# robdancer/SymbolicRegression.jl

Measured on AMD Instinct MI355X. Metric: tree-node x row evals/sec (whole node), 1k trees x 1M rows f32; % VALU peak, higher is better.
Workload: dtype f32; 1 GPU; C2 eval-only: 1024 random trees (size<=30) x 1M rows x 5 features Float32, fused L2 loss; ntrees_per_gpu=1024, rows=1000000, features=5, parallelism=single, trees_ok=808

## Files before the change

include/srhip.h:

```cpp
#ifndef SRHIP_H
#define SRHIP_H

#include <stdint.h>

#ifdef __cplusplus
extern "C" {
#endif

enum {
  SRHIP_OK = 0,
  SRHIP_ERR_INVALID = 1,
  SRHIP_ERR_UNSUPPORTED = 2,
  SRHIP_ERR_DEVICE = 3,
  SRHIP_ERR_NOMEM = 4
};

enum { SRHIP_F32 = 0, SRHIP_F64 = 1, SRHIP_I32 = 2 };

enum {
  SRHIP_OP_ADD = 1, SRHIP_OP_SUB = 2, SRHIP_OP_MUL = 3, SRHIP_OP_DIV = 4,
  SRHIP_OP_POW = 5,
  SRHIP_OP_GREATER = 6,
  SRHIP_OP_COND = 7,
  SRHIP_OP_LOGICAL_OR = 8,
// ... 31 lines not shown
  SRHIP_LOSS_PERCEPTRON = 10,
  SRHIP_LOSS_LOGIT_MARGIN = 11,
  SRHIP_LOSS_L1_HINGE = 12,
  SRHIP_LOSS_L2_HINGE = 13,
  SRHIP_LOSS_SMOOTHED_L1_HINGE = 14,
  SRHIP_LOSS_MODIFIED_HUBER = 15,
  SRHIP_LOSS_L2_MARGIN = 16,
  SRHIP_LOSS_EXP = 17,
  SRHIP_LOSS_SIGMOID = 18,
  SRHIP_LOSS_DWD_MARGIN = 19
};

typedef struct srhip_node {
  uint8_t degree;
  uint8_t constant;
  uint16_t op;
  uint16_t feature;
  uint16_t pad;
  int32_t l, r;
  double val;
} srhip_node;

typedef struct srhip_operators {
  int32_t nbin, nuna;
  const int32_t* binops;
  const int32_t* unaops;
} srhip_operators;

typedef struct srhip_loss {
  int32_t kind;
  int32_t pad;
  double p0, p1;
} srhip_loss;

typedef struct srhip_ctx srhip_ctx;
typedef struct srhip_dataset srhip_dataset;
typedef struct srhip_program srhip_program;

const char* srhip_last_error(void);
const char* srhip_version(void);
int srhip_device_count(void);

int srhip_ctx_create(int device_ordinal, srhip_ctx** out);
void srhip_ctx_destroy(srhip_ctx* ctx);
int srhip_ctx_synchronize(srhip_ctx* ctx);

int srhip_dataset_create(srhip_ctx* ctx, int dtype, const void* X, int64_t nfeatures, int64_t n,
                         int64_t stride_feature, int64_t stride_row, const void* y,
                         const void* weights, srhip_dataset** out);
void srhip_dataset_destroy(srhip_dataset* ds);

int srhip_program_create(srhip_ctx* ctx, int dtype, const srhip_node* nodes,
                         const int64_t* tree_offsets , int32_t ntrees,
                         const srhip_operators* ops, srhip_program** out);
void srhip_program_destroy(srhip_program* prog);
int srhip_program_num_constants(const srhip_program* prog, int32_t* out_nconst );
int srhip_program_set_constants(srhip_program* prog, const double* consts);
int srhip_program_get_constants(const srhip_program* prog, double* consts);

int srhip_eval_loss(srhip_ctx* ctx, const srhip_dataset* ds, const srhip_program* prog,
                    const srhip_loss* loss, const int64_t* idx, int64_t nidx,
                    double* out_loss, uint8_t* out_ok);

int srhip_eval_loss_rowsets(srhip_ctx* ctx, const srhip_dataset* ds, const srhip_program* prog,
                            const srhip_loss* loss, const int64_t* row_offsets ,
                            const int64_t* rows, double* out_loss, uint8_t* out_ok);

typedef struct srhip_eval_ticket srhip_eval_ticket;
int srhip_eval_loss_submit(srhip_ctx* ctx, const srhip_dataset* ds, const srhip_program* prog,
                           const srhip_loss* loss, const int64_t* idx, int64_t nidx,
                           srhip_eval_ticket** out_ticket);
int srhip_eval_loss_wait(srhip_eval_ticket* ticket, double* out_loss, uint8_t* out_ok);

int srhip_eval_predict(srhip_ctx* ctx, const srhip_dataset* ds, const srhip_program* prog,
                       const int64_t* idx, int64_t nidx, void* out_pred, uint8_t* out_ok);

int srhip_eval_loss_batch(srhip_ctx* ctx, const srhip_dataset* ds, const srhip_node* nodes,
                          const int64_t* tree_offsets, int32_t ntrees, const srhip_operators* ops,
                          const srhip_loss* loss, const int64_t* idx, int64_t nidx,
                          double* out_loss, uint8_t* out_ok);

int srhip_eval_loss_partials(srhip_ctx* ctx, const srhip_dataset* ds, const srhip_program* prog,
                             const srhip_loss* loss, const int64_t* idx, int64_t nidx,
                             double* sums, double* chk);
int srhip_partials_finalize(const srhip_program* prog, int64_t nfeatures, const double* sums,
                            const double* chk, double* out_loss, uint8_t* out_ok,
                            uint8_t* out_status);
int srhip_eval_precise_partials(srhip_ctx* ctx, const srhip_dataset* ds, const srhip_program* prog,
                                const int64_t* idx, int64_t nidx, const int32_t* trees,
                                int32_t ntrees_sel, double* opsums);
int srhip_precise_finalize(const srhip_program* prog, const int32_t* trees, int32_t ntrees_sel,
                           const double* opsums, uint8_t* out_ok);
int srhip_chk_reduce_op(int dtype);
int32_t srhip_program_max_ops(const srhip_program* prog);

typedef struct srhip_comm srhip_comm;
enum { SRHIP_COMM_ID_BYTES = 128 };
enum { SRHIP_REDUCE_SUM = 0, SRHIP_REDUCE_MAX = 1 };
int srhip_comm_unique_id(uint8_t* out_id );
int srhip_comm_create(srhip_ctx* ctx, const uint8_t* id, int32_t nranks, int32_t rank, srhip_comm** out);
void srhip_comm_destroy(srhip_comm* comm);
int srhip_comm_size(const srhip_comm* comm, int32_t* nranks, int32_t* rank);
int srhip_comm_stats(const srhip_comm* comm, double* ms_last, double* ms_total, int64_t* calls);
int srhip_comm_allreduce_f64(srhip_comm* comm, double* buf, int64_t n, int32_t op);
int srhip_comm_allgather(srhip_comm* comm, const void* send, int64_t bytes, void* recv);
int srhip_comm_migrate_start(srhip_comm* comm, const srhip_node* nodes, const int64_t* offsets,
                             int32_t ntrees, const double* losses, int32_t k, int32_t max_nodes);
int srhip_comm_migrate_wait(srhip_comm* comm, int32_t* out_counts, int64_t* out_offsets,
                            double* out_losses, srhip_node* out_nodes);
int srhip_eval_loss_sharded(srhip_ctx* ctx, srhip_comm* comm, const srhip_dataset* ds,
                            const srhip_program* prog, const srhip_loss* loss, const int64_t* idx,
                            int64_t nidx, double* out_loss, uint8_t* out_ok);

int srhip_eval_loss_grad(srhip_ctx* ctx, const srhip_dataset* ds, srhip_program* prog,
                         const srhip_loss* loss, const int64_t* idx, int64_t nidx,
                         double* out_loss, double* out_grad, uint8_t* out_ok);

enum { SRHIP_WRT_CONSTANTS = 0, SRHIP_WRT_FEATURES = 1 };
int srhip_eval_grad_predict(srhip_ctx* ctx, const srhip_dataset* ds, srhip_program* prog, int32_t wrt,
                            int32_t direction, const int64_t* idx, int64_t nidx, void* out_pred, void* out_grad,
                            uint8_t* out_ok);

typedef struct srhip_optim_options {
  int32_t iterations;
  int32_t nrestarts;
  uint64_t seed;
  double g_tol;
} srhip_optim_options;

int srhip_optimize_constants(srhip_ctx* ctx, const srhip_dataset* ds, srhip_program* prog,
                             const srhip_loss* loss, const int64_t* idx, int64_t nidx,
                             const srhip_optim_options* opt, double* out_loss,
                             uint8_t* out_improved, int64_t* out_fcalls);
int srhip_optimize_constants_starts(srhip_ctx* ctx, const srhip_dataset* ds, srhip_program* prog,
                                    const srhip_loss* loss, const int64_t* idx, int64_t nidx,
                                    const srhip_optim_options* opt, const double* starts_in,
                                    double* starts_out, double* out_loss, uint8_t* out_improved,
                                    int64_t* out_fcalls);

int srhip_eval_loss_grad_rowsets(srhip_ctx* ctx, const srhip_dataset* ds, srhip_program* prog,
                                 const srhip_loss* loss, const int64_t* row_offsets ,
                                 const int64_t* rows, double* out_loss, double* out_grad,
                                 uint8_t* out_ok);

int srhip_optimize_constants_rowsets(srhip_ctx* ctx, const srhip_dataset* ds, srhip_program* prog,
                                     const srhip_loss* loss, const int64_t* row_offsets ,
                                     const int64_t* rows, const srhip_optim_options* opt,
                                     const uint64_t* tree_seeds ,
                                     const double* starts_in , double* starts_out ,
                                     double* out_loss, uint8_t* out_improved, int64_t* out_fcalls);

double srhip_last_kernel_ms(const srhip_ctx* ctx);
int srhip_last_work(const srhip_ctx* ctx, int64_t out[4]);
int srhip_program_stats(const srhip_program* prog, int64_t* total_nodes, int64_t* total_opnodes,
                        int32_t* max_stack);
int srhip_program_derived(const srhip_program* prog, int32_t* count, uint32_t* spec, int32_t cap);
int srhip_code_cache_stats(int64_t* hits, int64_t* misses, int64_t* inserts);
int srhip_tail_share_parts(int32_t blocks, int32_t units, int32_t nshares, int32_t share, int32_t* out);

typedef struct srhip_batcher srhip_batcher;
int srhip_batcher_create(srhip_ctx* ctx, const srhip_dataset* ds, const srhip_operators* ops,
                         const srhip_loss* loss, int32_t max_batch, int32_t max_wait_us,
                         srhip_batcher** out);
int srhip_batcher_set_clients(srhip_batcher* b, int32_t nclients);
int srhip_batcher_submit(srhip_batcher* b, const srhip_node* nodes, int64_t nnodes,
                         const int64_t* idx, int64_t nidx, uint64_t* ticket);
int srhip_batcher_wait(srhip_batcher* b, uint64_t ticket, double* out_loss, uint8_t* out_ok);
int srhip_batcher_eval(srhip_batcher* b, const srhip_node* nodes, int64_t nnodes,
                       const int64_t* idx, int64_t nidx, double* out_loss, uint8_t* out_ok);
int srhip_batcher_stats(const srhip_batcher* b, int64_t* nrequests, int64_t* nlaunches,
                        int64_t* max_batch_seen);
int srhip_batcher_timing(const srhip_batcher* b, double* busy_ms, double* kernel_ms);
void srhip_batcher_destroy(srhip_batcher* b);

#ifdef __cplusplus
}
#endif
#endif
```

symbolicregression.jl_amd/csrc/srhip_eval_f32w.hip:

```cpp
#include "srhip_eval_impl.h"
#include "srhip_eval_variants.h"

namespace srhip {
hipError_t launch_eval_f32w(const EvalArgs& a, int mode, bool xlds, dim3 g, size_t lds, hipStream_t s) {
  if (mode == MODE_LOSS)
    return xlds ? launch_eval_t<float, R_F32_WIDE, 2, MODE_LOSS, true>(a, g, lds, s)
                : launch_eval_t<float, R_F32_WIDE, 2, MODE_LOSS, false>(a, g, lds, s);
  return xlds ? launch_eval_t<float, R_F32_WIDE, 2, MODE_PRED, true>(a, g, lds, s)
              : launch_eval_t<float, R_F32_WIDE, 2, MODE_PRED, false>(a, g, lds, s);
}
}
```

symbolicregression.jl_amd/csrc/srhip_eval_impl.h:

```cpp
#pragma once
#include <hip/hip_runtime.h>
#include <stdint.h>

#include <algorithm>
#include <type_traits>

#include "srhip_isa.h"
#include "srhip_kernels.h"
#include "srhip_ops.h"

#define UNR _Pragma("unroll")
#ifdef SRHIP_KDEBUG
#define KDBG(...) do { if (blockIdx.x == 0 && blockIdx.y == 0 && threadIdx.x == 0) printf(__VA_ARGS__); } while (0)
#else
#define KDBG(...) do { } while (0)
#endif
#ifdef SRHIP_KTRACE
#define KMARK(slot, val)                                                                       \
  do {                                                                                         \
    if (p.dbg && blockIdx.x == 0 && blockIdx.y == 0 && threadIdx.x == 0)                      \
      __hip_atomic_store(p.dbg + (slot), (int32_t)(val), __ATOMIC_RELAXED, __HIP_MEMORY_SCOPE_SYSTEM); \
  } while (0)
#else
#define KMARK(slot, val) do { } while (0)
#endif
#ifndef SRHIP_HEAVY_ILP
#define SRHIP_HEAVY_ILP 1
#endif
#ifndef SRHIP_TRIG_ILP
#ifndef SRHIP_JTRIG_FAST
#define SRHIP_JTRIG_FAST 1
#endif
#define SRHIP_TRIG_ILP SRHIP_HEAVY_ILP
#endif
#ifndef SRHIP_TRIG_ROWS
#define SRHIP_TRIG_ROWS 1
#endif
#ifndef SRHIP_HOT_CASES
#define SRHIP_HOT_CASES 0
#endif
#if SRHIP_HOT_CASES
#define SRHIP_LK [[likely]]
#else
#define SRHIP_LK
#endif
#define SRHIP_HOTB_ADD SRHIP_LK
#define SRHIP_HOTB_SUB SRHIP_LK
#define SRHIP_HOTB_MUL SRHIP_LK
#define SRHIP_HOTB_DIV SRHIP_LK
#define SRHIP_HOTB_GREATER
#define SRHIP_HOTB_COND
#define SRHIP_HOTB_LOGICAL_OR
#define SRHIP_HOTB_LOGICAL_AND
#define SRHIP_HOTB_MAX
#define SRHIP_HOTB_MIN
#define SRHIP_HOTU_NEG SRHIP_LK
#define SRHIP_HOTU_SQUARE SRHIP_LK
#define SRHIP_HOTU_CUBE SRHIP_LK
#define SRHIP_HOTU_ABS SRHIP_LK
#define SRHIP_HOTU_RELU
#define SRHIP_HOTU_COS SRHIP_LK
#define SRHIP_HOTU_SIN SRHIP_LK
#define SRHIP_HOTU_TAN
#define SRHIP_HOTU_EXP SRHIP_LK
#define SRHIP_HOTU_LOG SRHIP_LK
#define SRHIP_HOTU_LOG2
#define SRHIP_HOTU_LOG10
#define SRHIP_HOTU_LOG1P
#define SRHIP_HOTU_SQRT
#define SRHIP_HOTU_ACOSH
#define SRHIP_HOTU_ATANH_CLIP
#define SRHIP_HOTU_SINH
#define SRHIP_HOTU_COSH
#define SRHIP_HOTU_TANH
#define SRHIP_HOTU_ASIN
#define SRHIP_HOTU_ACOS
#define SRHIP_HOTU_ATAN
#define SRHIP_HOTU_ASINH
#define SRHIP_HOTU_ERF
#define SRHIP_HOTU_ERFC
#define SRHIP_HOTU_GAMMA
#define SRHIP_HOTU_ROUND
#define SRHIP_HOTU_FLOOR
#define SRHIP_HOTU_CEIL
#define SRHIP_HOTU_SIGN
#define SRHIP_HOTU_EXP2
#define SRHIP_HOTU_EXPM1
#define SRHIP_HOTU_CBRT
#ifndef SRHIP_ASM_DEF
#define SRHIP_ASM_DEF 1
#endif
#ifndef SRHIP_ROW_FENCE
#define SRHIP_ROW_FENCE() __builtin_amdgcn_sched_barrier(0)
#endif

namespace srhip {

template <typename T> constexpr bool kIsInt = std::is_same<T, int32_t>::value;

__device__ __attribute__((always_inline)) inline int tid_x() {
  int t = (int)__builtin_amdgcn_workitem_id_x();
  asm volatile("" : "+v"(t));
  return t;
}

template <typename T>
using OpsT = typename std::conditional<kIsInt<T>, IOps, FOps<typename std::conditional<kIsInt<T>, float, T>::type>>::type;

template <typename T> __device__ constexpr bool sb_ok(int sb) {
  return !kIsInt<T> || sb != SB_DIV;
}
template <typename T> __device__ constexpr bool hb_ok(int) { return !kIsInt<T>; }
template <typename T> __device__ constexpr bool un_ok(int u) {
  return !kIsInt<T> || u == UN_NEG || u == UN_SQUARE || u == UN_CUBE || u == UN_ABS ||
         u == UN_RELU || u == UN_SIGN;
}

template <typename T> struct Vec16;
template <> struct Vec16<float> { typedef float __attribute__((ext_vector_type(4))) type; };
template <> struct Vec16<int32_t> { typedef int32_t __attribute__((ext_vector_type(4))) type; };
template <> struct Vec16<double> { typedef double __attribute__((ext_vector_type(2))) type; };

template <typename T, int R> struct RowVec { typedef T type __attribute__((ext_vector_type(R))); };
template <typename T, int R> using RV = typename RowVec<T, R>::type;

template <typename T, int R>
__device__ __attribute__((always_inline)) inline void load_rows(const T* base, int lane, RV<T, R>& v) {
  constexpr int VEC = 16 / sizeof(T);
  using V = typename Vec16<T>::type;
  UNR for (int j = 0; j < R / VEC; ++j) {
    const V q = reinterpret_cast<const V*>(base)[j * 64 + lane];
    UNR for (int e = 0; e < VEC; ++e) v[j * VEC + e] = q[e];
  }
}

#if defined(__HIP_DEVICE_COMPILE__)
typedef const __attribute__((address_space(4))) Ins CIns;
#else
typedef const Ins CIns;
#endif

template <typename T> __device__ __attribute__((always_inline)) inline T imm_as(uint64_t bits) {
  if constexpr (sizeof(T) == 8) {
    return __builtin_bit_cast(T, bits);
  } else {
    return __builtin_bit_cast(T, (uint32_t)bits);
  }
}


__device__ __attribute__((always_inline)) inline int cvt_i32_sat(double k) {
  int m;
  asm("v_cvt_i32_f64 %0, %1" : "=v"(m) : "v"(k));
  return m;
}

template <int KIND>
__device__ __attribute__((always_inline)) inline float sincosf_dev(double x) {
  const double invpi = 0.3183098861837907, pi_hi = 3.141592653589793, pi_lo = 1.2246467991473532e-16;
  double k = __builtin_rint(__builtin_fma(x, invpi, KIND == 0 ? -0.5 : 0.0));
  const int m = cvt_i32_sat(k);
  if (KIND == 0) k += 0.5;
  const double y = __builtin_fma(-k, pi_lo, __builtin_fma(-k, pi_hi, x));
  const double p = srm_psin(y * y);
  const float r = KIND == 0 ? (float)(-y * p) : (float)(y * p);
  uint32_t o;
  asm("v_lshl_add_u32 %0, %1, 31, %2" : "=v"(o) : "v"(m), "v"(__builtin_bit_cast(uint32_t, r)));
  return __builtin_bit_cast(float, o);
}

typedef float F2 __attribute__((ext_vector_type(2)));
__device__ __attribute__((always_inline)) inline int cvt_i32_f32(float x) {
  int m;
  asm("v_cvt_i32_f32 %0, %1" : "=v"(m) : "v"(x));
  return m;
}
__device__ __attribute__((always_inline)) inline F2 expf2_dev(F2 x) {
  x = __builtin_elementwise_minimum(__builtin_elementwise_maximum(x, (F2)(-104.0f)), (F2)(89.0f));
  F2 n = x * (F2)(SRM_EXPF_LOG2E);
  n.x = __builtin_rintf(n.x);
  n.y = __builtin_rintf(n.y);
  F2 r = __builtin_elementwise_fma(n, (F2)(SRM_EXPF_NLN2_HI), x);
  r = __builtin_elementwise_fma(n, (F2)(SRM_EXPF_NLN2_LO), r);
  F2 p = __builtin_elementwise_fma(r, (F2)(SRM_EXPF_C6), (F2)(SRM_EXPF_C5));
  p = __builtin_elementwise_fma(r, p, (F2)(SRM_EXPF_C4));
  p = __builtin_elementwise_fma(r, p, (F2)(SRM_EXPF_C3));
  p = __builtin_elementwise_fma(r, p, (F2)(0.5f));
  p = __builtin_elementwise_fma(r, p, (F2)(1.0f));
  p = __builtin_elementwise_fma(r, p, (F2)(1.0f));
  F2 out;
  out.x = __builtin_ldexpf(p.x, cvt_i32_f32(n.x));
  out.y = __builtin_ldexpf(p.y, cvt_i32_f32(n.y));
  return out;
}

constexpr float EXPF_FAST_MAX = 87.0f;
__device__ __attribute__((always_inline)) inline F2 expf2_fast(F2 x) {
  const F2 t = x * (F2)(SRM_EXPF_LOG2E) + (F2)(12582912.0f);
  const F2 n = t - (F2)(12582912.0f);
  F2 r = __builtin_elementwise_fma(n, (F2)(SRM_EXPF_NLN2_HI), x);
  r = __builtin_elementwise_fma(n, (F2)(SRM_EXPF_NLN2_LO), r);
  F2 p = __builtin_elementwise_fma(r, (F2)(SRM_EXPF_C6), (F2)(SRM_EXPF_C5));
  p = __builtin_elementwise_fma(r, p, (F2)(SRM_EXPF_C4));
  p = __builtin_elementwise_fma(r, p, (F2)(SRM_EXPF_C3));
  p = __builtin_elementwise_fma(r, p, (F2)(0.5f));
  p = __builtin_elementwise_fma(r, p, (F2)(1.0f));
  p = __builtin_elementwise_fma(r, p, (F2)(1.0f));
  float s0, s1;
  asm("v_lshl_add_u32 %0, %1, 23, 1.0" : "=v"(s0) : "v"(t.x));
  asm("v_lshl_add_u32 %0, %1, 23, 1.0" : "=v"(s1) : "v"(t.y));
  return p * (F2){s0, s1};
}

#define SRM_PIO2F_BIG_F 421657440.0f
template <int R>
__device__ __attribute__((noinline)) RV<float, R> trigf_fix_tan(RV<float, R> v, RV<float, R> res) {
  UNR for (int r = 0; r < R; ++r) {
    const float x = v[r];
    if (x - x == 0.0f && srm_pio2f_is_big((double)x)) res[r] = srm_trigf(2, x);
  }
  return res;
}
template <int R, int KIND>
__device__ __attribute__((noinline)) RV<float, R> trigf_fix(RV<float, R> v, RV<float, R> res) {
  UNR for (int r = 0; r < R; ++r) {
    const float x = v[r];
    if (!(__builtin_fabsf(x) < SRM_PIO2F_BIG_F)) res[r] = srm_trigf(KIND, x);
  }
  return res;
}
template <int R, int KIND>
__device__ __attribute__((noinline)) RV<float, R> trigf_fast(RV<float, R> v) {
  UNR for (int r = 0; r < R; ++r) {
    v[r] = sincosf_dev<KIND>((double)v[r]);
    if ((r + 1) % SRHIP_HEAVY_ILP == 0) SRHIP_ROW_FENCE();
  }
  return v;
}
template <int R, int KIND>
__device__ __attribute__((noinline)) RV<float, R> trigf_slow(RV<float, R> v) {
  UNR for (int r = 0; r < R; ++r) {
    const float x = v[r];
    v[r] = __builtin_fabsf(x) < SRM_PIO2F_BIG_F ? sincosf_dev<KIND>((double)x) : srm_trigf(KIND, x);
  }
  return v;
}
#define SRHIP_M3(OP, a, b) OP " %0, %0, |%" #a "|, |%" #b "|\n\t"
template <int R, bool MAX>
__device__ __attribute__((always_inline)) inline float abs_fold(float m, const RV<float, R>& v) {
#define SRHIP_OPC (MAX ? "v_maximum3_f32" : "v_minimum3_f32")
  if constexpr (R == 16) {
    if constexpr (MAX)
      asm(SRHIP_M3("v_maximum3_f32", 1, 2) SRHIP_M3("v_maximum3_f32", 3, 4) SRHIP_M3("v_maximum3_f32", 5, 6)
          SRHIP_M3("v_maximum3_f32", 7, 8) SRHIP_M3("v_maximum3_f32", 9, 10) SRHIP_M3("v_maximum3_f32", 11, 12)
          SRHIP_M3("v_maximum3_f32", 13, 14) SRHIP_M3("v_maximum3_f32", 15, 16)
          : "+v"(m) : "v"(v[0]), "v"(v[1]), "v"(v[2]), "v"(v[3]), "v"(v[4]), "v"(v[5]), "v"(v[6]), "v"(v[7]),
            "v"(v[8]), "v"(v[9]), "v"(v[10]), "v"(v[11]), "v"(v[12]), "v"(v[13]), "v"(v[14]), "v"(v[15]));
    else
      asm(SRHIP_M3("v_minimum3_f32", 1, 2) SRHIP_M3("v_minimum3_f32", 3, 4) SRHIP_M3("v_minimum3_f32", 5, 6)
          SRHIP_M3("v_minimum3_f32", 7, 8) SRHIP_M3("v_minimum3_f32", 9, 10) SRHIP_M3("v_minimum3_f32", 11, 12)
          SRHIP_M3("v_minimum3_f32", 13, 14) SRHIP_M3("v_minimum3_f32", 15, 16)
          : "+v"(m) : "v"(v[0]), "v"(v[1]), "v"(v[2]), "v"(v[3]), "v"(v[4]), "v"(v[5]), "v"(v[6]), "v"(v[7]),
            "v"(v[8]), "v"(v[9]), "v"(v[10]), "v"(v[11]), "v"(v[12]), "v"(v[13]), "v"(v[14]), "v"(v[15]));
  } else if constexpr (R == 32) {
    RV<float, 16> lo, hi;
    UNR for (int r = 0; r < 16; ++r) { lo[r] = v[r]; hi[r] = v[16 + r]; }
    m = abs_fold<16, MAX>(m, lo);
    m = abs_fold<16, MAX>(m, hi);
  } else if constexpr (R == 8) {
    if constexpr (MAX)
      asm(SRHIP_M3("v_maximum3_f32", 1, 2) SRHIP_M3("v_maximum3_f32", 3, 4) SRHIP_M3("v_maximum3_f32", 5, 6)
          SRHIP_M3("v_maximum3_f32", 7, 8)
          : "+v"(m) : "v"(v[0]), "v"(v[1]), "v"(v[2]), "v"(v[3]), "v"(v[4]), "v"(v[5]), "v"(v[6]), "v"(v[7]));
    else
      asm(SRHIP_M3("v_minimum3_f32", 1, 2) SRHIP_M3("v_minimum3_f32", 3, 4) SRHIP_M3("v_minimum3_f32", 5, 6)
          SRHIP_M3("v_minimum3_f32", 7, 8)
          : "+v"(m) : "v"(v[0]), "v"(v[1]), "v"(v[2]), "v"(v[3]), "v"(v[4]), "v"(v[5]), "v"(v[6]), "v"(v[7]));
  } else {
    static_assert(R % 2 == 0, "row pairs");
    UNR for (int r = 0; r < R; r += 2) {
      if constexpr (MAX) asm("v_maximum3_f32 %0, %1, |%2|, |%3|" : "=v"(m) : "v"(m), "v"(v[r]), "v"(v[r + 1]));
      else asm("v_minimum3_f32 %0, %1, |%2|, |%3|" : "=v"(m) : "v"(m), "v"(v[r]), "v"(v[r + 1]));
    }
  }
#undef SRHIP_OPC
  return m;
}

template <int R> __device__ __attribute__((always_inline)) inline bool trigf_rows_fast(const RV<float, R>& A) {
  const float mx = abs_fold<R, true>(0.0f, A);
  return __builtin_amdgcn_ballot_w64(!(mx < SRM_PIO2F_BIG_F)) == 0;
}
// ... 516 lines not shown
      bin_rows<T, R, SB_SUB, false>(lv, yv);
      RV<T, R> dv;
      UNR for (int r = 0; r < R; ++r) dv[r] = lv[r];
      bin_rows<T, R, SB_MUL, false>(lv, dv);
    } else if (p.loss_kind == SRHIP_LOSS_L1) {
      UNR for (int r = 0; r < R; ++r) lv[r] = m_abs(A[r] - yv[r]);
    } else {
      lv = loss_rows_generic<T, R>(A, yv, p.loss_kind, p0);
    }
    if (p.weighted) {
      UNR for (int r = 0; r < R; ++r) lacc[r / RPC] += (double)(wv[r] * lv[r]);
    } else {
      if (!full) {
        UNR for (int r = 0; r < R; ++r) {
          const int64_t row = row0 + (r / VEC) * 64 * VEC + lane * VEC + (r % VEC);
          lv[r] = row < p.nvalid ? lv[r] : T(0);
        }
      }
      if constexpr (sizeof(T) == 4 && R % 4 == 0 && VEC == 4) {
        UNR for (int r = 0; r < R; r += 4) {
          const F2 a = {lv[r], lv[r + 1]}, b = {lv[r + 2], lv[r + 3]};
          const F2 q = a + b;
          lacc[r / RPC] += (double)(q.x + q.y);
        }
      } else {
        UNR for (int r = 0; r < R; ++r) lacc[r / RPC] += (double)lv[r];
      }
    }
  }
}

template <typename T, int R>
__device__ __attribute__((always_inline)) inline void store_pred(const EvalArgs& p, const RV<T, R>& A, int tree, int lane,
                                                                 int64_t row0) {
  constexpr int VEC = 16 / sizeof(T);
  using V = typename Vec16<T>::type;
  T* out = reinterpret_cast<T*>(p.out_pred) + (int64_t)tree * p.nvalid;
  UNR for (int j = 0; j < R / VEC; ++j) {
    const int64_t row = row0 + j * 64 * VEC + lane * VEC;
    if (row + VEC <= p.nvalid && ((p.nvalid % VEC) == 0)) {
      V q;
      UNR for (int e = 0; e < VEC; ++e) q[e] = A[j * VEC + e];
      *reinterpret_cast<V*>(out + row) = q;
    } else {
      UNR for (int e = 0; e < VEC; ++e)
        if (row + e < p.nvalid) out[row + e] = A[j * VEC + e];
    }
  }
}

template <typename T, int R>
__device__ __attribute__((noinline)) RV<T, R> derive_un(int u, RV<T, R> v) {
  switch (u) {
#define X_(NAME, FN)                                                                     \
  case UN_##NAME:                                                                        \
    if constexpr (un_ok<T>(UN_##NAME) && un_derivable(UN_##NAME)) return heavy_un<T, R, UN_##NAME>(v); \
    break;
    SRHIP_UNOPS(X_)
#undef X_
    default: break;
  }
  return v;
}

template <typename T>
__device__ __attribute__((always_inline)) inline void derive_columns(const EvalArgs& p, T* lx, int rbb,
                                                                     typename Chk<T>::type* dchk) {
  using CT = typename Chk<T>::type;
  constexpr int DV = 16 / sizeof(T);
  __shared__ CT part[EVAL_WAVES_MAX][DERIVE_MAX];
  const int tid = tid_x();
  const int lane = tid & 63, wave = tid >> 6;
  for (int d = 0; d < p.nd; ++d) {
    const uint32_t spec = __builtin_amdgcn_readfirstlane(p.dspec[d]);
    const int u = (int)(spec >> 16), f = (int)(spec & 0xffff);
    const T* src = lx + (int64_t)f * rbb;
    T* dst = lx + (int64_t)(p.nfeat + d) * rbb;
    CT m = 0;
    for (int c = tid; c < rbb / DV; c += blockDim.x) {
      RV<T, DV> v = reinterpret_cast<const RV<T, DV>*>(src)[c];
      v = derive_un<T, DV>(u, v);
      reinterpret_cast<RV<T, DV>*>(dst)[c] = v;
      UNR for (int e = 0; e < DV; ++e) {
        if constexpr (sizeof(T) == 4) m = __builtin_elementwise_maximum(m, __builtin_fabsf(v[e]));
        else m = __builtin_fma(__builtin_fabs(v[e]), 0x1p-512, m);
      }
    }
    m = wave_chk(m);
    if (lane == WAVE_LAST) part[wave][d] = m;
  }
  __syncthreads();
  const int tf = tid_x();
  if (tf < p.nd) {
    const int d = tf;
    CT t = part[0][d];
    for (int w = 1; w < (int)(blockDim.x >> 6); ++w) {
      if constexpr (sizeof(T) == 4) t = __builtin_elementwise_maximum(t, part[w][d]);
      else t += part[w][d];
    }
    dchk[d] = t;
  }
  __syncthreads();
}

template <typename T, int R>
__device__ __attribute__((always_inline)) inline void derive_columns_tiles(const EvalArgs& p, T* lx, int rbb,
                                                                           typename Chk<T>::type* dchk) {
  using CT = typename Chk<T>::type;
  constexpr int TILE = 64 * R, VEC = 16 / sizeof(T);
  constexpr int MAX_TILES = ROW_ALIGN / TILE > 0 ? ROW_ALIGN / TILE : 1;
  __shared__ CT part[DERIVE_MAX][MAX_TILES];
  const int tid = tid_x();
  const int lane = tid & 63;
  const int wave = __builtin_amdgcn_readfirstlane(tid >> 6), nwaves = blockDim.x >> 6;
  const int ntiles = rbb / TILE;
  for (int item = wave; item < p.nd * ntiles; item += nwaves) {
    const int d = item / ntiles, j = item - d * ntiles;
    const uint32_t spec = __builtin_amdgcn_readfirstlane(p.dspec[d]);
    const int u = (int)(spec >> 16), f = (int)(spec & 0xffff);
    RV<T, R> v;
    load_rows<T, R>(lx + (int64_t)f * rbb + (int64_t)j * TILE, lane, v);
    RV<T, R> rv;
    UNR for (int r = 0; r < R; ++r) rv[r] = v[r];
    rv = derive_un<T, R>(u, rv);
    CT m = 0;
    using V = typename Vec16<T>::type;
    T* dst = lx + (int64_t)(p.nfeat + d) * rbb + (int64_t)j * TILE;
    UNR for (int q = 0; q < R / VEC; ++q) {
      V o;
      UNR for (int e = 0; e < VEC; ++e) {
        o[e] = rv[q * VEC + e];
        if constexpr (sizeof(T) == 4) m = __builtin_elementwise_maximum(m, __builtin_fabsf(o[e]));
        else m = __builtin_fma(__builtin_fabs(o[e]), 0x1p-512, m);
      }
      reinterpret_cast<V*>(dst)[q * 64 + lane] = o;
    }
    m = wave_chk(m);
    if (lane == WAVE_LAST) part[d][j] = m;
  }
  __syncthreads();
  const int tf = tid_x();
  if (tf < p.nd) {
    const int d = tf;
    CT t = part[d][0];
    for (int j = 1; j < ntiles; ++j) {
      if constexpr (sizeof(T) == 4) t = __builtin_elementwise_maximum(t, part[d][j]);
      else t += part[d][j];
    }
    dchk[d] = t;
  }
  __syncthreads();
}

template <typename T, int R, int K, int MODE, bool XLDS>
__device__ __attribute__((always_inline)) inline void eval_block(const EvalArgs& p, unsigned char* smem, const int rb,
                                                                 const int gy, const int gslice = 0,
                                                                 const int gstride = 1, const int gw = 1) {
  constexpr int WAVES = eval_waves(R, K);
  using O = OpsT<T>;
  using CT = typename Chk<T>::type;
  constexpr int TILE = 64 * R;
  const int lane = tid_x() & 63;
  const int64_t row_base = (int64_t)rb * p.rb_rows;
  const int ntiles = p.rb_rows / TILE;
  const int nrel = __builtin_amdgcn_readfirstlane((int)min<int64_t>(max<int64_t>(p.nvalid - row_base, 0), (int64_t)p.rb_rows));

  const T* xsrc;
  const T* ysrc;
  const T* wsrc;
  int64_t xstride;
  if constexpr (XLDS) {
    T* lx = reinterpret_cast<T*>(smem);
    const int rbb = p.rb_rows;
    const int ncols = p.nfeat + (p.has_y ? 1 : 0) + (p.weighted ? 1 : 0);
    using V = typename Vec16<T>::type;
    constexpr int VEC = 16 / sizeof(T);
    const int vec_per_col = rbb / VEC;
    const T* gX = reinterpret_cast<const T*>(p.X);
    const T* gy = reinterpret_cast<const T*>(p.y);
    const T* gw = reinterpret_cast<const T*>(p.w);
    for (int i = tid_x(); i < ncols * vec_per_col; i += blockDim.x) {
      const int c = i / vec_per_col;
      const int v = i - c * vec_per_col;
      const T* src = c < p.nfeat ? gX + (int64_t)c * p.ld : (c == p.nfeat ? gy : gw);
      const int lc = c < p.nfeat ? c : c + p.nd;
      reinterpret_cast<V*>(lx + (int64_t)lc * rbb)[v] = reinterpret_cast<const V*>(src + row_base)[v];
    }
    xsrc = lx;
    ysrc = lx + (int64_t)(p.nfeat + p.nd) * rbb;
    wsrc = lx + (int64_t)(p.nfeat + p.nd + 1) * rbb;
    xstride = rbb;
  } else {
    xsrc = reinterpret_cast<const T*>(p.X) + row_base;
    ysrc = reinterpret_cast<const T*>(p.y) + row_base;
    wsrc = reinterpret_cast<const T*>(p.w) + row_base;
    xstride = p.ld;
  }
  KDBG("[k] staged, ntiles=%d rb_rows=%d nvalid=%ld max_steps=%d\n", ntiles, p.rb_rows, (long)p.nvalid, p.max_steps);
  __shared__ int next_tree;
  if (threadIdx.x == 0) next_tree = blockDim.x >> 6;
  constexpr int FLAG_SNAP = 2048;
  constexpr bool SNAP = MODE == MODE_LOSS && !kIsInt<T>;
  __shared__ uint8_t failed_snap[SNAP ? FLAG_SNAP : 1];
  const int gb0 = p.group_off ? p.group_off[gy] : gy * p.trees_per_group;
  const int snap_base = gb0 + gslice;
  const int snap_n = gstride > 1 ? tail_units_count(p.ntrees, gstride, gslice, gw)
                                 : (p.group_off ? p.group_off[gy + 1] - gb0 : min(p.trees_per_group, p.ntrees - gb0));
  if constexpr (SNAP) {
    if (p.early_exit)
      for (int i = tid_x(); i < min(snap_n, FLAG_SNAP); i += blockDim.x)
        failed_snap[i] = __hip_atomic_load(p.fail_flag + snap_base + (gw > 1 ? i / gw * gstride + i % gw : i * gstride),
                                           __ATOMIC_RELAXED, __HIP_MEMORY_SCOPE_AGENT) == p.epoch;
  }
  __syncthreads();
  constexpr bool DERIVED = XLDS && !kIsInt<T> && MODE != MODE_PRECISE;
  __shared__ CT dchk[DERIVED ? DERIVE_MAX : 1];
  if constexpr (DERIVED) {
    if (p.nd > 0) {
      if (p.persistent) derive_columns_tiles<T, R>(p, reinterpret_cast<T*>(smem), p.rb_rows, dchk);
      else derive_columns<T>(p, reinterpret_cast<T*>(smem), p.rb_rows, dchk);
    }
  }
  KMARK(0, 2);
  if (p.debug_stop == 2) return;

  const int group_base = __builtin_amdgcn_readfirstlane(snap_base);
  int group_n = __builtin_amdgcn_readfirstlane(snap_n);
  if constexpr (MODE == MODE_PRECISE) {
    if (p.dev_count) {
      const int cnt = __builtin_amdgcn_readfirstlane(*p.dev_count);
      group_n = max(0, min(group_n, (cnt - group_base + gstride - 1) / gstride));
    }
  }

  const int wave = __builtin_amdgcn_readfirstlane(threadIdx.x >> 6);
  const CIns* code = (const CIns*)(uintptr_t)p.code;
  KMARK(8 + wave, 10);
  const bool tile_claims = p.tile_claims != 0 && TILE == (sizeof(T) == 8 ? LOSS_CHUNK_8B : LOSS_CHUNK_4B);
  const int nclaims = tile_claims ? group_n * ntiles : group_n;
  for (int cl = wave; cl < nclaims;) {
    const int ti = tile_claims ? cl / ntiles : cl;
    const int tile0 = tile_claims ? cl - ti * ntiles : 0, tile_end = tile_claims ? tile0 + 1 : ntiles;
    KMARK(8 + wave, 11);
    const int slot = group_base + (gw > 1 ? ti / gw * gstride + ti % gw : ti * gstride);
    const int tree = __builtin_amdgcn_readfirstlane(p.order[slot]);
    const int pc0 = __builtin_amdgcn_readfirstlane(p.prog_off[tree]);
    const int max_steps = __builtin_amdgcn_readfirstlane(p.max_steps);
    KDBG("[k] ti=%d tree=%d pc0=%d group_n=%d\n", ti, tree, pc0, group_n);
    KMARK(0, 3);
    KMARK(1, tree);
    if (p.debug_stop == 3) break;

    if constexpr (MODE == MODE_PRECISE) {
      if (p.dev_count && lane == WAVE_LAST)
        for (int k = 0; k < p.prec_stride; ++k)
          reinterpret_cast<double*>(p.slab_prec)[((int64_t)slot * p.prec_stride + k) * p.nrb + rb] = 0.0;
    }
    constexpr int CHS = sizeof(T) == 8 ? LOSS_CHUNK_8B : LOSS_CHUNK_4B;
    constexpr int CPT = TILE > CHS ? TILE / CHS : 1, TPC = TILE > CHS ? 1 : CHS / TILE;
    static_assert(TILE > CHS ? TILE % CHS == 0 : CHS % TILE == 0, "tiles and loss chunks nest");
    LAccT<T> lacc[CPT];
    UNR for (int c = 0; c < CPT; ++c) lacc[c] = 0;
    CT M = 0;
    bool failed = false;
    if constexpr (SNAP) {
      if (p.early_exit && ti < FLAG_SNAP) failed = __builtin_amdgcn_readfirstlane(failed_snap[ti]) != 0;
    }
    if constexpr (DERIVED) {
      if (p.nd > 0) {
        uint64_t msk = p.dmask[tree];
        msk = ((uint64_t)__builtin_amdgcn_readfirstlane((uint32_t)(msk >> 32)) << 32) |
              (uint32_t)__builtin_amdgcn_readfirstlane((uint32_t)msk);
        while (msk) {
          const int d = __builtin_ctzll(msk);
          msk &= msk - 1;
          if constexpr (sizeof(T) == 4) M = __builtin_elementwise_maximum(M, dchk[d]);
          else if (lane == WAVE_LAST) M += dchk[d];
        }
      }
    }
    LAccT<T>* lslab = reinterpret_cast<LAccT<T>*>(p.slab_loss) +
                      ((int64_t)rb * p.ntrees + slot) * __builtin_amdgcn_readfirstlane(p.cpb);
    LAccT<T> csum = 0;
    int rows_done = 0;
    if (failed) {
      if (lane == WAVE_LAST)
        for (int c = tile_claims ? tile0 : 0; c < (tile_claims ? tile_end : p.cpb); ++c) lslab[c] = (LAccT<T>)NAN;
      M = (CT)NAN;
      csum = (LAccT<T>)NAN;
    }
    for (int tile = tile0; tile < (failed ? tile0 : tile_end); ++tile) {
      const int64_t row0 = row_base + (int64_t)tile * TILE;
      const int trel = tile * TILE;
      if (trel >= nrel) break;
      rows_done += min(TILE, nrel - trel);
      const T* xt = xsrc + (int64_t)tile * TILE;
      RV<T, R> A, S[K];
#if SRHIP_ASM_DEF
      asm volatile("" : "=v"(A));
      UNR for (int k = 0; k < K; ++k) asm volatile("" : "=v"(S[k]));
#else
      UNR for (int r = 0; r < R; ++r) A[r] = T(0);
      UNR for (int k = 0; k < K; ++k) UNR for (int r = 0; r < R; ++r) S[k][r] = T(0);
#endif
      const CIns* prog = code + pc0;
      Ins nxt = prog[0];
      [[maybe_unused]] uint32_t pord = 0;
      for (int step = 0; step < max_steps; ++step) {
        const Ins ins = nxt;
        nxt = prog[step + 1];
        KDBG("[k]   tile=%d step=%d h=%u a=%u\n", tile, step, ins.h, ins.a);
        if (ins.h == H_END) break;
        switch (ins.h) {
          SRHIP_LK case H_LOADF:
            load_rows<T, R>(xt + (int64_t)(ins.a & 0xffff) * xstride, lane, A);
            if constexpr (MODE == MODE_PRECISE)
              if ((ins.a >> 16) != 0) precise_hook<T, R>(p, ++pord, A, slot, rb, lane, row0);
            break;
          SRHIP_LK case H_LOADC: { const T c = imm_as<T>(ins.imm); UNR for (int r = 0; r < R; ++r) A[r] = c; break; }
#define SRHIP_K_CASES(BASE, ...)                                                            \
  case BASE + 0: if constexpr (0 < K) { constexpr int k = 0; __VA_ARGS__ } break;                 \
  case BASE + 1: if constexpr (1 < K) { constexpr int k = 1; __VA_ARGS__ } break;                 \
  case BASE + 2: if constexpr (2 < K) { constexpr int k = 2; __VA_ARGS__ } break;                 \
  case BASE + 3: if constexpr (3 < K) { constexpr int k = 3; __VA_ARGS__ } break;                 \
  case BASE + 4: if constexpr (4 < K) { constexpr int k = 4; __VA_ARGS__ } break;                 \
  case BASE + 5: if constexpr (5 < K) { constexpr int k = 5; __VA_ARGS__ } break;                 \
  case BASE + 6: if constexpr (6 < K) { constexpr int k = 6; __VA_ARGS__ } break;                 \
  case BASE + 7: if constexpr (7 < K) { constexpr int k = 7; __VA_ARGS__ } break;
#define SRHIP_K_CASES_H(HOT, BASE, ...)                                                     \
  HOT case BASE + 0: if constexpr (0 < K) { constexpr int k = 0; __VA_ARGS__ } break;             \
  HOT case BASE + 1: if constexpr (1 < K) { constexpr int k = 1; __VA_ARGS__ } break;             \
  case BASE + 2: if constexpr (2 < K) { constexpr int k = 2; __VA_ARGS__ } break;                 \
  case BASE + 3: if constexpr (3 < K) { constexpr int k = 3; __VA_ARGS__ } break;                 \
  case BASE + 4: if constexpr (4 < K) { constexpr int k = 4; __VA_ARGS__ } break;                 \
  case BASE + 5: if constexpr (5 < K) { constexpr int k = 5; __VA_ARGS__ } break;                 \
  case BASE + 6: if constexpr (6 < K) { constexpr int k = 6; __VA_ARGS__ } break;                 \
  case BASE + 7: if constexpr (7 < K) { constexpr int k = 7; __VA_ARGS__ } break;
          SRHIP_K_CASES_H(SRHIP_LK, H_PUSH0, { UNR for (int r = 0; r < R; ++r) S[k][r] = A[r]; })
          SRHIP_K_CASES_H(SRHIP_LK, H_PUSHLF0, {
            UNR for (int r = 0; r < R; ++r) S[k][r] = A[r];
            load_rows<T, R>(xt + (int64_t)(ins.a & 0xffff) * xstride, lane, A);
          })
          SRHIP_K_CASES_H(SRHIP_LK, H_PUSHLC0, {
            UNR for (int r = 0; r < R; ++r) S[k][r] = A[r];
            const T c = imm_as<T>(ins.imm);
            UNR for (int r = 0; r < R; ++r) A[r] = c;
          })
          SRHIP_K_CASES(H_SLOADF0, { load_rows<T, R>(xt + (int64_t)(ins.a & 0xffff) * xstride, lane, S[k]); })
          SRHIP_K_CASES(H_SLOADC0, { const T c = imm_as<T>(ins.imm); UNR for (int r = 0; r < R; ++r) S[k][r] = c; })

#define SRHIP_SPEC_CASE(NAME, FN)                                                                  \
  SRHIP_HOTB_##NAME case h_spec(SB_##NAME, SPEC_AF):                                                \
    if constexpr (sb_ok<T>(SB_##NAME)) {                                                           \
      RV<T, R> xv;                                                                                     \
      load_rows<T, R>(xt + (int64_t)(ins.a & 0xffff) * xstride, lane, xv);                                    \
      bin_rows_chk<T, R, SB_##NAME, false>(A, xv, M);                                              \
      if constexpr (MODE == MODE_PRECISE) precise_hook<T, R>(p, ++pord, A, slot, rb, lane, row0);         \
    }                                                                                              \
    break;                                                                                         \
  SRHIP_HOTB_##NAME case h_spec(SB_##NAME, SPEC_FA):                                                \
    if constexpr (sb_ok<T>(SB_##NAME)) {                                                           \
      RV<T, R> xv;                                                                                     \
      load_rows<T, R>(xt + (int64_t)(ins.a & 0xffff) * xstride, lane, xv);                                    \
      bin_rows_chk<T, R, SB_##NAME, true>(A, xv, M);                                               \
      if constexpr (MODE == MODE_PRECISE) precise_hook<T, R>(p, ++pord, A, slot, rb, lane, row0);         \
    }                                                                                              \
    break;                                                                                         \
  SRHIP_HOTB_##NAME case h_spec(SB_##NAME, SPEC_AC):                                                \
    if constexpr (sb_ok<T>(SB_##NAME)) {                                                           \
      bin_rows_c_chk<T, R, SB_##NAME, false>(A, imm_as<T>(ins.imm), M);                            \
      if constexpr (MODE == MODE_PRECISE) precise_hook<T, R>(p, ++pord, A, slot, rb, lane, row0);         \
    }                                                                                              \
    break;                                                                                         \
  SRHIP_HOTB_##NAME case h_spec(SB_##NAME, SPEC_CA):                                                \
    if constexpr (sb_ok<T>(SB_##NAME)) {                                                           \
      bin_rows_c_chk<T, R, SB_##NAME, true>(A, imm_as<T>(ins.imm), M);                             \
      if constexpr (MODE == MODE_PRECISE) precise_hook<T, R>(p, ++pord, A, slot, rb, lane, row0);         \
    }                                                                                              \
    break;                                                                                         \
  SRHIP_HOTB_##NAME case h_spec(SB_##NAME, SPEC_FF):                                              \
    if constexpr (sb_ok<T>(SB_##NAME)) {                                                           \
      RV<T, R> xv;                                                                                 \
      load_rows<T, R>(xt + (int64_t)(ins.a & 0xffff) * xstride, lane, A);                          \
      load_rows<T, R>(xt + (int64_t)(ins.imm & 0xffff) * xstride, lane, xv);                       \
      bin_rows_chk<T, R, SB_##NAME, false>(A, xv, M);                                              \
      if constexpr (MODE == MODE_PRECISE) precise_hook<T, R>(p, ++pord, A, slot, rb, lane, row0);     \
    }                                                                                              \
    break;                                                                                         \
  SRHIP_HOTB_##NAME case h_spec(SB_##NAME, SPEC_FC):                                              \
    if constexpr (sb_ok<T>(SB_##NAME)) {                                                           \
      load_rows<T, R>(xt + (int64_t)(ins.a & 0xffff) * xstride, lane, A);                          \
      bin_rows_c_chk<T, R, SB_##NAME, false>(A, imm_as<T>(ins.imm), M);                            \
      if constexpr (MODE == MODE_PRECISE) precise_hook<T, R>(p, ++pord, A, slot, rb, lane, row0);     \
    }                                                                                              \
    break;                                                                                         \
  SRHIP_HOTB_##NAME case h_spec(SB_##NAME, SPEC_CF):                                              \
    if constexpr (sb_ok<T>(SB_##NAME)) {                                                           \
      load_rows<T, R>(xt + (int64_t)(ins.a & 0xffff) * xstride, lane, A);                          \
      bin_rows_c_chk<T, R, SB_##NAME, true>(A, imm_as<T>(ins.imm), M);                             \
      if constexpr (MODE == MODE_PRECISE) precise_hook<T, R>(p, ++pord, A, slot, rb, lane, row0);     \
    }                                                                                              \
    break;                                                                                         \
    SRHIP_K_CASES_H(SRHIP_HOTB_##NAME, h_spec(SB_##NAME, SPEC_SA0), if constexpr (sb_ok<T>(SB_##NAME)) {                \
      bin_rows_chk<T, R, SB_##NAME, true>(A, S[k], M);                                             \
      if constexpr (MODE == MODE_PRECISE) precise_hook<T, R>(p, ++pord, A, slot, rb, lane, row0);         \
    })                                                                                             \
    SRHIP_K_CASES_H(SRHIP_HOTB_##NAME, h_spec(SB_##NAME, SPEC_AS0), if constexpr (sb_ok<T>(SB_##NAME)) {                \
      bin_rows_chk<T, R, SB_##NAME, false>(A, S[k], M);                                            \
      if constexpr (MODE == MODE_PRECISE) precise_hook<T, R>(p, ++pord, A, slot, rb, lane, row0);         \
    })
          SRHIP_SPEC_BINOPS(SRHIP_SPEC_CASE)
#undef SRHIP_SPEC_CASE

#define SRHIP_HEAVY_CASE(NAME, FN)                                                              \
    SRHIP_K_CASES(h_heavy(HB_##NAME, HEAVY_SA0), if constexpr (hb_ok<T>(HB_##NAME)) {           \
      apply_heavy<T, R, HB_##NAME>(A, S[k], A);                                                 \
      chk_update<R>(M, A);                                                                      \
      if constexpr (MODE == MODE_PRECISE) precise_hook<T, R>(p, ++pord, A, slot, rb, lane, row0);  \
    })                                                                                          \
    SRHIP_K_CASES(h_heavy(HB_##NAME, HEAVY_AS0), if constexpr (hb_ok<T>(HB_##NAME)) {           \
      apply_heavy<T, R, HB_##NAME>(A, A, S[k]);                                                 \
      chk_update<R>(M, A);                                                                      \
      if constexpr (MODE == MODE_PRECISE) precise_hook<T, R>(p, ++pord, A, slot, rb, lane, row0);  \
    })
          SRHIP_HEAVY_BINOPS(SRHIP_HEAVY_CASE)
#undef SRHIP_HEAVY_CASE

#define SRHIP_UN_CASE(NAME, FN)                                                  \
  SRHIP_HOTU_##NAME case h_un(UN_##NAME):                                        \
    if constexpr (un_ok<T>(UN_##NAME) && (K == K_MAX || !un_wide(UN_##NAME))) {  \
      apply_un<T, R, UN_##NAME>(A);                                              \
      if constexpr (UN_##NAME == UN_COS || UN_##NAME == UN_SIN) {                \
        if (!(ins.a & UN_NC_FLAG)) chk_update<R>(M, A);                          \
      } else {                                                                   \
        chk_update<R>(M, A);                                                     \
      }                                                                          \
      if constexpr (MODE == MODE_PRECISE) precise_hook<T, R>(p, ++pord, A, slot, rb, lane, row0); \
    }                                                                            \
    break;
          SRHIP_UNOPS(SRHIP_UN_CASE)
#undef SRHIP_UN_CASE
#undef SRHIP_K_CASES
          default: break;
        }
      }
      KDBG("[k]   tile %d done\n", tile);
      KMARK(0, 4);
      if constexpr (MODE == MODE_LOSS) {
        loss_tile<T, R>(p, A, ysrc + (int64_t)tile * TILE, wsrc + (int64_t)tile * TILE, lane, row0, trel + TILE <= nrel,
                        lacc);
        const bool flushed = (tile + 1) % TPC == 0 || trel + TILE >= nrel;
        const int ci0 = tile * CPT / TPC;
        if (flushed) {
          UNR for (int c = 0; c < CPT; ++c) {
            const LAccT<T> s = wave_sum(lacc[c]);
            if (lane == WAVE_LAST) lslab[ci0 + c] = s;
            if (p.fused) {
              const LAccT<T> sb = __shfl(s, WAVE_LAST);
              if (lane == (ci0 + c) % 64) csum += sb;
            }
            lacc[c] = 0;
          }
        }
        if constexpr (!kIsInt<T>) {
          if (p.early_exit && __builtin_amdgcn_ballot_w64(!(M < (CT)INFINITY)) != 0) {
            csum = (LAccT<T>)NAN;
            if (lane == WAVE_LAST) {
              for (int c = ci0 + (flushed ? CPT : 0); c < (tile_claims ? tile_end : p.cpb); ++c)
                lslab[c] = (LAccT<T>)NAN;
              __hip_atomic_store(p.fail_flag + slot, p.epoch, __ATOMIC_RELAXED, __HIP_MEMORY_SCOPE_AGENT);
            }
            break;
          }
        }
      } else if constexpr (MODE == MODE_PRED) {
        store_pred<T, R>(p, A, tree, lane, row0);
      }
    }
    KDBG("[k] tree %d tiles done\n", tree);
    KMARK(0, 5);
    KMARK(8 + wave, 12);
    if constexpr (!kIsInt<T> && MODE != MODE_PRECISE) {
      M = wave_chk(M);
      CT* chk_at = reinterpret_cast<CT*>(p.slab_chk) + (int64_t)rb * p.ntrees + slot;
      if (lane == WAVE_LAST) {
        if constexpr (sizeof(CT) == 4) {
          if (tile_claims) atomicMax(reinterpret_cast<unsigned*>(chk_at), __builtin_bit_cast(unsigned, __builtin_fabsf(M) == __builtin_fabsf(M) ? __builtin_fabsf(M) : M));
          else *chk_at = M;
        } else {
          *chk_at = M;
        }
      }
    }
    if (p.slab_rows && lane == WAVE_LAST) {
      if (tile_claims) atomicAdd(p.slab_rows + (int64_t)rb * p.ntrees + slot, rows_done);
      else p.slab_rows[(int64_t)rb * p.ntrees + slot] = rows_done;
    }
    if constexpr (MODE != MODE_PRECISE) {
      if (p.fused) {
        LAccT<T> s = csum;
        CT m = 0;
        if constexpr (!kIsInt<T>) {
          const CT mb = __shfl(M, WAVE_LAST);
          if (lane == 0) {
            if constexpr (sizeof(T) == 4) m = __builtin_elementwise_maximum(m, mb);
            else m += mb;
          }
        }
        UNR for (int o = 32; o > 0; o >>= 1) {
          if (MODE == MODE_LOSS) s += __shfl_xor(s, o);
          if constexpr (!kIsInt<T>) {
            if constexpr (sizeof(T) == 4) m = __builtin_elementwise_maximum(m, __shfl_xor(m, o));
            else m += __shfl_xor(m, o);
          }
        }
        if (lane == 0) {
          if (MODE == MODE_LOSS && p.fused_loss) reinterpret_cast<LAccT<T>*>(p.fused_loss)[tree] = s;
          if (p.fused_chk) reinterpret_cast<CT*>(p.fused_chk)[tree] = m;
          if (p.fused_rows) p.fused_rows[tree] = rows_done;
        }
      }
    }
    KMARK(8 + wave, 13);
    int claim = 0;
    if (lane == 0) claim = atomicAdd(&next_tree, 1);
    cl = __builtin_amdgcn_readfirstlane(claim);
  }
  KMARK(8 + wave, 14);
}

template <typename T, int R, int K, int MODE, bool XLDS>
__global__ __launch_bounds__(64 * eval_waves(R, K)) void eval_kernel(EvalArgs p) {
  extern __shared__ __attribute__((aligned(16))) unsigned char smem[];
  KMARK(0, 1);
  if (p.debug_stop == 1) return;
  __shared__ int claimed;
  if constexpr (MODE == MODE_PRECISE) {
    if (p.dev_count && p.grid_interleave && __builtin_amdgcn_readfirstlane(*p.dev_count) <= (int)blockIdx.y) return;
  }
  if (p.tile_claims && !p.persistent) {
    if (p.zero_ctr && blockIdx.x == 0 && blockIdx.y == 0 && threadIdx.x == 0)
      __hip_atomic_store(p.zero_ctr, 0, __ATOMIC_RELAXED, __HIP_MEMORY_SCOPE_AGENT);
    const int gs = p.grid_interleave ? (int)blockIdx.y : 0, gst = p.grid_interleave ? (int)gridDim.y : 1;
    const int nz = p.grid_interleave ? (p.ntrees - gs + gst - 1) / gst : 0;
    for (int i = threadIdx.x; i < nz; i += blockDim.x) {
      const int64_t at = (int64_t)blockIdx.x * p.ntrees + gs + (int64_t)i * gst;
      if (p.slab_chk) __hip_atomic_store(reinterpret_cast<uint32_t*>(p.slab_chk) + at, 0u, __ATOMIC_RELAXED, __HIP_MEMORY_SCOPE_AGENT);
      if (p.slab_rows) __hip_atomic_store(p.slab_rows + at, 0, __ATOMIC_RELAXED, __HIP_MEMORY_SCOPE_AGENT);
    }
    __builtin_amdgcn_fence(__ATOMIC_RELEASE, "workgroup");
  }
  const int nfull = p.nrb - p.block0 - p.tail_blocks;
  const int nitems = nfull + (p.tail_blocks > 0 ? p.tail_shares : 0);
  int items = 0;
  int next_block = 0, next_units = 0;
  for (int it = 0;; ++it) {
    int rb, gy = 0, gslice = 0, gstride = 1, gw = 1;
    if (p.persistent && next_units > 0) {
      rb = next_block;
      gstride = p.tail_slices;
      gw = next_units;
      next_units = 0;
    } else if (p.persistent) {
      if (threadIdx.x == 0) claimed = atomicAdd(p.block_ctr, 1);
      __syncthreads();
      const int item = __builtin_amdgcn_readfirstlane(claimed);
      if (item >= nitems) {
        if (threadIdx.x == 0 && items > 0) atomicAdd(p.block_ctr + 1, items);
        if (threadIdx.x == 0 && item == nitems + (int)gridDim.x - 1)
          __hip_atomic_store(p.block_ctr, 0, __ATOMIC_RELAXED, __HIP_MEMORY_SCOPE_AGENT);
        break;
      }
      ++items;
      rb = p.block0 + item;
      if (item >= nfull) {
        TailPart part[2];
        const int nparts = tail_share_parts(p.tail_blocks, p.tail_slices, p.tail_shares, item - nfull, part);
        if (nparts == 0) {
          __syncthreads();
          continue;
        }
        rb = p.block0 + nfull + part[0].block;
        gslice = part[0].u0;
        gstride = p.tail_slices;
        gw = part[0].u1 - part[0].u0;
        if (nparts == 2) {
          next_block = rb + 1;
          next_units = part[1].u1;
        }
      }
    } else {
      rb = blockIdx.x + it * (int)gridDim.x;
      if (it > 0 && (!p.block_stride || rb >= p.nrb)) break;
      if (p.grid_interleave) {
        gslice = blockIdx.y;
        gstride = gridDim.y;
      } else {
        gy = blockIdx.y;
      }
    }
    eval_block<T, R, K, MODE, XLDS>(p, smem, rb, gy, gslice, gstride, gw);
    if (!p.persistent && !p.block_stride) break;
    __syncthreads();
  }
}

template <typename T, int R, int K, int MODE, bool XLDS>
inline hipError_t launch_eval_t(const EvalArgs& a, dim3 grid, size_t lds, hipStream_t s) {
  auto kern = eval_kernel<T, R, K, MODE, XLDS>;
  if (lds > 65536) {
    hipError_t e = hipFuncSetAttribute((const void*)kern, hipFuncAttributeMaxDynamicSharedMemorySize, (int)lds);
    if (e != hipSuccess) return e;
  }
  const int waves = a.wg_waves > 0 ? std::min(a.wg_waves, eval_waves(R, K)) : eval_waves(R, K);
  hipLaunchKernelGGL(kern, grid, dim3(64 * waves), lds, s, a);
  return hipGetLastError();
}

template <typename T, int R, int MODE, bool XLDS>
inline hipError_t launch_eval_k(const EvalArgs& a, int K, dim3 grid, size_t lds, hipStream_t s) {
  if (K <= 2) return launch_eval_t<T, R, 2, MODE, XLDS>(a, grid, lds, s);
  if (K <= 4) return launch_eval_t<T, R, 4, MODE, XLDS>(a, grid, lds, s);
  return launch_eval_t<T, R, 8, MODE, XLDS>(a, grid, lds, s);
}

template <typename T, int R, int MODE>
inline hipError_t launch_eval_mode(const EvalArgs& a, int K, bool xlds, dim3 grid, size_t lds, hipStream_t s) {
  if constexpr (MODE == MODE_PRECISE) {
    (void)K;
    (void)xlds;
    return launch_eval_t<T, R, K_MAX, MODE_PRECISE, false>(a, grid, lds, s);
  } else {
    return xlds ? launch_eval_k<T, R, MODE, true>(a, K, grid, lds, s) : launch_eval_k<T, R, MODE, false>(a, K, grid, lds, s);
  }
}

}
```

symbolicregression.jl_amd/csrc/srhip_host.cpp:

```cpp
#include <hip/hip_runtime.h>
#include <math.h>
#include <stdarg.h>
#include <stdint.h>
#include <stdio.h>
#include <stdlib.h>
#include <string.h>
#include <unistd.h>
#include <sys/resource.h>
#include <sys/syscall.h>

#include <algorithm>
#include <atomic>
#include <chrono>
#include <condition_variable>
#include <functional>
#include <memory>
#include <map>
#include <mutex>
#include <numeric>
#include <string>
#include <thread>
#include <type_traits>
#include <unordered_map>
#include <vector>
// ... 1375 lines not shown
  if (n_dspec) memcpy(h + o_dspec, P.dspec.data(), n_dspec);
  if (n_dmask) memcpy(h + o_dmask, P.dmask.data(), n_dmask);
  if (n_sb) memcpy(h + o_sb, P.sbound.data(), n_sb);
  const size_t offs[7] = {o_off, o_dcode, o_doff, o_dspec, o_dmask, o_sb, total};
  memcpy(P.blob_off, offs, sizeof(offs));
  if (defer) {
    P.upload_pending = true;
    return SRHIP_OK;
  }
  P.upload_pending = false;
  const bool with_order = !P.ord_host.empty() && P.ord_key[0] > 0;
  const size_t nbytes = with_order ? total + P.ord_host.size() * sizeof(int32_t) : total;
  if (with_order) {
    P.blob.resize(nbytes);
    memcpy(P.blob.data() + total, P.ord_host.data(), P.ord_host.size() * sizeof(int32_t));
    h = P.blob.data();
  }
  HIP_TRY(P.d_prog.ensure(nbytes));
  hipStream_t st = stream ? stream : P.ctx->stream;
  HIP_TRY(hipMemcpyAsync(P.d_prog.p, h, nbytes, hipMemcpyHostToDevice, st));
  set_prog_pointers(P);
  if (with_order) P.ord_dev = (const uint8_t*)P.d_prog.p + total;
  if (sync) HIP_TRY(hipStreamSynchronize(st));
  return SRHIP_OK;
}


namespace {

}

int srhip::make_view(srhip_ctx* ctx, const srhip_dataset* ds, const int64_t* idx, int64_t nidx, bool need_y, View& v) {
  if (need_y && !ds->has_y) return fail(SRHIP_ERR_INVALID, "dataset has no y");
  if (!idx) {
    v.X = ds->X.p;
    v.y = ds->y.p;
    v.w = ds->weighted ? ds->w.p : nullptr;
    v.ld = ds->ld;
    v.m = ds->n;
    v.stats = ds->hstats.data();
    v.sum_w = ds->sum_w;
    return SRHIP_OK;
  }
  if (nidx <= 0) return fail(SRHIP_ERR_INVALID, "empty idx");
  for (int64_t i = 0; i < nidx; ++i)
    if (idx[i] < 0 || idx[i] >= ds->n) return fail(SRHIP_ERR_INVALID, "idx[%lld] = %lld out of range", (long long)i, (long long)idx[i]);
  const size_t es = dtype_size(ds->dtype);
  const int64_t ld = (nidx + ROW_ALIGN - 1) / ROW_ALIGN * ROW_ALIGN;
  HIP_TRY(ctx->vX.ensure((size_t)std::max<int64_t>(1, ds->nfeat) * ld * es));
  HIP_TRY(ctx->vy.ensure((size_t)ld * es));
  HIP_TRY(ctx->vw.ensure((size_t)ld * es));
  HIP_TRY(ctx->vidx.ensure((size_t)nidx * sizeof(int64_t)));
  HIP_TRY(ctx->vstats.ensure(feature_stats_scratch(ds->nfeat) * sizeof(FeatStat)));
  HIP_TRY(ctx->h_stats.ensure((size_t)std::max<int64_t>(1, ds->nfeat) * sizeof(FeatStat)));
  HIP_TRY(hipMemcpyAsync(ctx->vidx.p, idx, (size_t)nidx * sizeof(int64_t), hipMemcpyHostToDevice, ctx->stream));
  HIP_TRY(launch_gather(ds->dtype, ds->X.p, ds->has_y ? ds->y.p : nullptr, ds->weighted ? ds->w.p : nullptr, ds->ld,
                        (int)ds->nfeat, (const int64_t*)ctx->vidx.p, nidx, ld, ctx->vX.p,
                        ds->has_y ? ctx->vy.p : nullptr, ds->weighted ? ctx->vw.p : nullptr, ctx->stream));
  HIP_TRY(launch_feature_stats(ds->dtype, ctx->vX.p, ld, nidx, (int)ds->nfeat, (FeatStat*)ctx->vstats.p, ctx->stream));
  if (ds->dtype != SRHIP_I32 && ds->nfeat > 0)
    HIP_TRY(hipMemcpyAsync(ctx->h_stats.p, ctx->vstats.p, (size_t)ds->nfeat * sizeof(FeatStat), hipMemcpyDeviceToHost,
                           ctx->stream));
  double sw = 0.0;
  if (ds->weighted) {
  }
  HIP_TRY(hipStreamSynchronize(ctx->stream));
  v.X = ctx->vX.p;
  v.y = ds->has_y ? ctx->vy.p : nullptr;
  v.w = ds->weighted ? ctx->vw.p : nullptr;
  v.ld = ld;
  v.m = nidx;
  v.stats = (const FeatStat*)ctx->h_stats.p;
  v.sum_w = sw;
  return SRHIP_OK;
}

LaunchPlan srhip::plan_launch(const srhip_ctx* ctx, int dtype, int64_t nxcols, bool weighted, bool with_y, int64_t m,
                              int32_t ntrees, int tile, size_t budget, int waves) {
  LaunchPlan L;
  ntrees = std::max<int32_t>(1, ntrees);
  m = std::max<int64_t>(1, m);
  const size_t es = dtype_size(dtype);
  const int ncols = (int)nxcols + (with_y ? 1 : 0) + (weighted ? 1 : 0);
  const int lo = std::max(tile, loss_chunk(dtype));
  int rb = ROW_ALIGN;
  while (rb > lo && (size_t)ncols * rb * es > budget) rb /= 2;
  while (rb > lo && rb / 2 >= m) rb /= 2;
  static const int rb_env = [] { const char* e = getenv("SRHIP_RB_ROWS"); return e ? atoi(e) : 0; }();
  if (rb_env >= lo && rb_env <= ROW_ALIGN && (rb_env & (rb_env - 1)) == 0 && rb_env < rb) rb = rb_env;
  L.rb_rows = rb;
  L.xlds = (size_t)ncols * rb * es <= budget;
  L.lds = (L.xlds ? (size_t)ncols * rb * es : 0) + 16;
  L.nrb = (int)((m + rb - 1) / rb);
  const int target_blocks = 4 * ctx->num_cu;
  int g = (target_blocks + L.nrb - 1) / L.nrb;
  const int max_g = std::max(1, ntrees / (2 * waves));
  g = std::max(1, std::min(g, max_g));
  L.groups = g;
  L.tpg = (ntrees + g - 1) / g;
  L.groups = (ntrees + L.tpg - 1) / L.tpg;
  return L;
}

namespace {

std::vector<int32_t> shape_groups(const LaunchPlan& L, int32_t ntrees, int num_cu) {
  static const bool no_tail = [] { const char* e = getenv("SRHIP_NO_TAIL"); return e && *e && *e != '0'; }();
  std::vector<int32_t> off(1, 0);
  const bool tail = !no_tail && ntrees >= 128 && (int64_t)L.groups * L.nrb > 2 * (int64_t)num_cu;
  if (!tail) {
    for (int g = 0; g < L.groups; ++g) off.push_back(std::min(ntrees, off.back() + L.tpg));
    return off;
  }
  static const int tail_div = [] { const char* e = getenv("SRHIP_TAIL_DIV"); return e && atoi(e) >= 2 ? atoi(e) : 32; }();
  static const int bulk_g = [] { const char* e = getenv("SRHIP_BULK_GROUPS"); return e ? atoi(e) : 0; }();
  const int32_t tl = std::max<int32_t>(16, ntrees / tail_div), bulk = ntrees - tl;
  const int groups = bulk_g > 0 ? std::min<int>(bulk_g, std::max(1, bulk / 16)) : L.groups;
  const int32_t tpg = (bulk + groups - 1) / groups;
  while (off.back() < bulk) off.push_back(std::min(bulk, off.back() + tpg));
  static const int tail_min = [] { const char* e = getenv("SRHIP_TAIL_MIN"); return e && atoi(e) > 0 ? atoi(e) : 16; }();
  int32_t t = tl;
  while (t > tail_min) {
    const int32_t h = t / 2;
    off.push_back(off.back() + h);
    t -= h;
  }
  if (t > 0) off.push_back(off.back() + t);
  return off;
}

std::vector<int32_t> make_order(const srhip_program& P, const std::vector<int32_t>& trees,
                                const std::vector<int32_t>& goff, bool derived) {
  std::vector<int32_t> s(trees);
  auto cost = [&](int32_t t) { return derived ? P.dcost[t] : P.info[t].cost; };
  std::stable_sort(s.begin(), s.end(), [&](int32_t a, int32_t b) { return cost(a) > cost(b); });
  const int groups = (int)goff.size() - 1;
  std::vector<int32_t> order(s.size());
  std::vector<int> fill(groups, 0);
  for (int32_t t : s) {
    int best = -1;
    double bf = -1.0;
    for (int g = 0; g < groups; ++g) {
      const int cap = goff[g + 1] - goff[g];
      if (fill[g] >= cap) continue;
      const double f = (double)(cap - fill[g]) / cap;
      if (f > bf) {
        bf = f;
        best = g;
      }
    }
    order[(size_t)goff[best] + fill[best]++] = t;
  }
  return order;
}


static int decide_info(const TreeInfo& I, int dtype, int32_t T, int64_t nfeat, const double* sums, double chk) {
  if (I.static_fail) return 1;
  if (dtype == SRHIP_I32) return 0;
  const long double m = (long double)sums[2 * (size_t)T + 2 * (size_t)nfeat];
  const long double ovf = ovf_threshold(dtype);
  for (double c : I.fill_consts)
    if ((long double)fabs(c) * m >= ovf) return 1;
  for (int f : I.feat_checks) {
    const double fsum = sums[2 * (size_t)T + 2 * (size_t)f], fbad = sums[2 * (size_t)T + 2 * (size_t)f + 1];
    if (fbad > 0) return 1;
    const long double sum = dtype == SRHIP_F64 ? (long double)fsum * 0x1p64L : (long double)fsum;
    if (!isfinite(fsum) || fabsl(sum) >= ovf) return 1;
  }
  if (I.op_sumcheck.empty()) return 0;
  if (!isfinite(chk)) return 1;
  long double bound;
  if (dtype == SRHIP_F64) bound = (long double)chk * 0x1p512L;
  else bound = (long double)chk * m;
  if (bound * 2.0L >= ovf) return 2;
  return 0;
}

static int decide_fast(const srhip_program& P, int32_t t, int64_t nfeat, const double* sums, double chk) {
  const TreeDecide& d = P.dec[t];
  if (d.slow) return decide_info(P.info[t], P.dtype, P.ntrees, nfeat, sums, chk);
  if (d.static_fail) return 1;
  const int dtype = P.dtype;
  if (dtype == SRHIP_I32) return 0;
  const int32_t T = P.ntrees;
  const long double m = (long double)sums[2 * (size_t)T + 2 * (size_t)nfeat];
  const long double ovf = ovf_threshold(dtype);
  if (d.maxc >= 0.0 && (long double)d.maxc * m >= ovf) return 1;
  for (uint64_t fm = d.feat_mask; fm; fm &= fm - 1) {
    const int f = __builtin_ctzll(fm);
    const double fsum = sums[2 * (size_t)T + 2 * (size_t)f], fbad = sums[2 * (size_t)T + 2 * (size_t)f + 1];
    if (fbad > 0) return 1;
    const long double sum = dtype == SRHIP_F64 ? (long double)fsum * 0x1p64L : (long double)fsum;
    if (!isfinite(fsum) || fabsl(sum) >= ovf) return 1;
  }
  if (!d.has_op) return 0;
  if (!isfinite(chk)) return 1;
  long double bound;
  if (dtype == SRHIP_F64) bound = (long double)chk * 0x1p512L;
  else bound = (long double)chk * m;
  if (bound * 2.0L >= ovf) return 2;
  return 0;
}

static void finalize(const srhip_program& P, int64_t nfeat, const double* sums, const double* chk, double* out_loss,
                     uint8_t* out_ok, uint8_t* out_status) {
  const bool fast = P.dec.size() == (size_t)P.ntrees && !env_flag("SRHIP_DECIDE_SLOW");
  for (int32_t t = 0; t < P.ntrees; ++t) {
    const double c = chk ? chk[t] : 0.0;
    const int st = fast ? decide_fast(P, t, nfeat, sums, c) : decide_info(P.info[t], P.dtype, P.ntrees, nfeat, sums, c);
    if (out_status) out_status[t] = (uint8_t)st;
    if (out_ok) out_ok[t] = st == 0 ? 1 : 0;
    if (out_loss) out_loss[t] = st == 0 ? sums[2 * (size_t)t] / sums[2 * (size_t)t + 1] : INFINITY;
  }
}

static void finalize_precise(const srhip_program& P, const int32_t* trees, int32_t nsel, const double* opsums,
                             uint8_t* out_ok, bool grad = false) {
  const int stride = std::max(1, grad ? P.gmax_ops : P.max_ops);
  const long double ovf = ovf_threshold(P.dtype);
  for (int u = 0; u < nsel; ++u) {
    const TreeInfo& I = grad ? P.ginfo[trees[u]] : P.info[trees[u]];
    int st = I.static_fail ? 1 : 0;
    for (size_t k = 0; k < I.op_sumcheck.size() && !st; ++k) {
      const double s = opsums[(size_t)u * stride + k];
      if (!isfinite(s)) st = 1;
      else if (I.op_sumcheck[k]) {
        const long double S = P.dtype == SRHIP_F64 ? (long double)s * 0x1p64L : (long double)s;
        if (fabsl(S) >= ovf) st = 1;
      }
    }
    out_ok[u] = st == 0 ? 1 : 0;
  }
}

}

namespace {
struct DevPool {
  std::mutex mu;
  std::map<std::pair<int, size_t>, std::vector<void*>> free;
  size_t cached = 0;
};
DevPool& devpool() {
  static DevPool* P = new DevPool();
  return *P;
}
constexpr size_t DEVPOOL_MAX_CACHED = (size_t)512 << 20;
size_t devpool_class(size_t n) {
  size_t c = 4096;
  while (c < n) c <<= 1;
  return c;
}
}

void* srhip::devpool_get(size_t bytes, size_t* cap) {
  const size_t c = devpool_class(bytes);
  int dev = 0;
  if (hipGetDevice(&dev) != hipSuccess) return nullptr;
  {
    DevPool& P = devpool();
    std::lock_guard<std::mutex> g(P.mu);
    auto it = P.free.find({dev, c});
    if (it != P.free.end() && !it->second.empty()) {
      void* q = it->second.back();
      it->second.pop_back();
      P.cached -= c;
      *cap = c;
      return q;
    }
  }
  void* q = nullptr;
  if (hipMalloc(&q, c) != hipSuccess) return nullptr;
  *cap = c;
  return q;
}

void srhip::devpool_put(void* p, size_t cap, int device) {
  if (!p) return;
  DevPool& P = devpool();
  {
    std::lock_guard<std::mutex> g(P.mu);
    if (device >= 0 && P.cached + cap <= DEVPOOL_MAX_CACHED) {
      P.free[{device, cap}].push_back(p);
      P.cached += cap;
      return;
    }
  }
  (void)hipFree(p);
}

int srhip::next_fail_epoch(srhip_ctx* ctx, int64_t n, int32_t** flags, int32_t* epoch) {
  const size_t need = (size_t)std::max<int64_t>(n, 1) * sizeof(int32_t);
  const bool fresh = !ctx->fail_flag.p || ctx->fail_flag.bytes < need;
  HIP_TRY(ctx->fail_flag.ensure(need));
  if (fresh || ctx->epoch == INT32_MAX) {
    HIP_TRY(hipMemsetAsync(ctx->fail_flag.p, 0, ctx->fail_flag.bytes, ctx->stream));
    ctx->epoch = 0;
  }
  *flags = (int32_t*)ctx->fail_flag.p;
  *epoch = ++ctx->epoch;
  return SRHIP_OK;
}

int srhip::decide_tree(const TreeInfo& I, const srhip_program& P, int64_t nfeat, const double* sums, double chk) {
  return decide_info(I, P.dtype, P.ntrees, nfeat, sums, chk);
// ... 89 lines not shown
  q.rb_rows = Lp.rb_rows;
  q.nrb = Lp.nrb;
  q.trees_per_group = 1;
  q.slab_prec = ctx->slab_prec.p;
  q.prec_stride = stride;
  q.max_steps = P->max_len;
  q.dev_count = ulist;
  q.wg_waves = 1;
  q.prec_assign = 1;
  q.block_stride = 1;
  HIP_TRY(launch_eval(dtype, q, Rp, K_MAX, MODE_PRECISE, false, dim3(std::min(Lp.nrb, PRECISE_GRID_X), G), 16,
                      ctx->stream));
  int32_t* hl = (int32_t*)rs->h_pout.p;
  double* hs = (double*)((uint8_t*)rs->h_pout.p + PREC_SUMS_OFF);
  HIP_TRY(launch_precise_reduce((const double*)ctx->slab_prec.p, Lp.nrb, stride, ulist, cap, G, DEV_PRECISE_MAX, hl,
                                hs, ctx->stream));
  *out_stride = stride;
  return SRHIP_OK;
}

struct EvalJob {
  ResultSet* rs = nullptr;
  bool launched = false, persistent = false, devp = false;
  int mode = 0, dtype = 0;
  int32_t nt = 0;
  int32_t expect_items = 0;
  std::vector<int32_t> live;
  UndecidedList ul;
  DevBuf pred;
  bool fused = false;
  float fbound = 0.0f;
};
static float feature_bound(const View& v, int64_t nfeat) {
  double F = 0.0;
  for (int64_t f = 0; v.stats && f < nfeat; ++f) {
    if (v.stats[f].nonfinite > 0 || !(v.stats[f].maxabs < INFINITY)) return INFINITY;
    F = std::max(F, v.stats[f].maxabs);
  }
  if (!v.stats && nfeat > 0) return INFINITY;
  const float r = (float)F;
  return (double)r >= F ? r : std::nextafter(r, INFINITY);
}

static int eval_issue(srhip_ctx* ctx, const srhip_dataset* ds, const srhip_program* P, int mode, const srhip_loss* loss,
                      const View& v, void* out_pred, double* sums, double* chk, DevPrecise* dp, ShardDev* sd,
                      EvalJob& J) {
  const int dtype = P->dtype;
  const int32_t nt = P->ntrees;
  ResultSet* const rs = J.rs;
  J.mode = mode;
  J.dtype = dtype;
  J.nt = nt;
  const int64_t nf = ds->nfeat;
  const bool weighted = ds->weighted && mode == MODE_LOSS;
  for (size_t i = 0; i < sums_len(nt, nf); ++i) sums[i] = 0.0;
  for (int32_t t = 0; t < nt; ++t) {
    chk[t] = 0.0;
    sums[2 * (size_t)t + 1] = weighted ? v.sum_w : (double)v.m;
  }
  for (int64_t f = 0; f < nf; ++f) {
    sums[2 * (size_t)nt + 2 * f] = v.stats[f].sum;
    sums[2 * (size_t)nt + 2 * f + 1] = (double)v.stats[f].nonfinite;
  }
  sums[2 * (size_t)nt + 2 * nf] = (double)v.m;
  std::vector<int32_t>& live = J.live;
  live.clear();
  live.reserve(nt);
  for (int32_t t = 0; t < nt; ++t)
    if (!(P->dec.size() == (size_t)nt ? P->dec[t].static_fail : P->info[t].static_fail)) live.push_back(t);
  if (live.empty()) return SRHIP_OK;
  const size_t es = dtype_size(dtype);
  bool wide = false;
  for (int32_t u : P->unaops) wide |= u == SRHIP_OP_ASIN || u == SRHIP_OP_ACOS || u == SRHIP_OP_ATANH_CLIP;
  auto kvariant = [&](int32_t kmax) { return wide ? K_MAX : (kmax <= 2 ? 2 : (kmax <= 4 ? 4 : 8)); };
  const int nd = (int)P->dspec.size();
  bool use_d = false;
  int K = 0, R = 0;
  LaunchPlan L{};
  const size_t lds_dev = (size_t)ctx->lds_max;
  auto lds_budget = [lds_dev](int r, int k, bool derived) -> size_t {
    if (eval_waves(r, k) >= 16) return lds_dev - 8 * 1024;
    return std::min<size_t>(lds_dev / 2, derived ? 64 * 1024 - 512 : 64 * 1024 - 64);
  };
  const bool no_persistent = env_flag("SRHIP_NO_PERSISTENT");
  const int prb_env = env_int("SRHIP_PRB_ROWS", 0);
  const int probe_env = env_int("SRHIP_PROBE_BLOCKS", -1);
  bool persistent = false;
  int probe_blocks = 0;
  const int small_max = env_int("SRHIP_SMALL_POP", 16);
  const bool small = (mode == MODE_LOSS || mode == MODE_PRED) && debug_stop() == 0 && (int)live.size() <= small_max &&
                     v.m >= (int64_t)64 * ROW_ALIGN;
  if (small) {
    K = kvariant(P->kmax);
    R = pick_rows_per_lane(dtype, K, mode, v.m);
    L.rb_rows = std::max(64 * R, loss_chunk(dtype));
    L.xlds = false;
    L.lds = 16;
    L.nrb = (int)((v.m + L.rb_rows - 1) / L.rb_rows);
    L.groups = 1;
    L.tpg = (int)live.size();
  }
  if (!small) {
    const int Kp = kvariant(P->kmax);
    persistent = !no_persistent && mode == MODE_LOSS && debug_stop() == 0 && dtype == SRHIP_F32 &&
                 pick_rows_per_lane(dtype, Kp, mode, v.m) == R_F32_WIDE && R_F32_WIDE != R_F32 &&
                 (nd == 0 || kvariant(P->dkmax) == Kp);
    if (persistent) {
      K = Kp;
      R = R_F32_WIDE;
      const int tile = 64 * R;
      int rb = prb_env >= tile && prb_env <= ROW_ALIGN && (prb_env & (prb_env - 1)) == 0 ? prb_env : 2048;
      rb = std::max(rb, std::max(tile, loss_chunk(dtype)));
      const size_t es = dtype_size(dtype);
      const int base_cols = P->maxfeat + 1 + (weighted ? 1 : 0);
      use_d = nd > 0 && (size_t)(base_cols + nd) * rb * es <= lds_budget(R, K, true);
      const int ncols = base_cols + (use_d ? nd : 0);
      if ((size_t)ncols * rb * es > lds_budget(R, K, false)) {
        persistent = false;
        use_d = false;
      } else {
        L.rb_rows = rb;
        L.xlds = true;
        L.lds = (size_t)ncols * rb * es + 16;
        L.nrb = (int)((v.m + rb - 1) / rb);
        L.groups = 1;
        L.tpg = (int)live.size();
        probe_blocks = probe_env >= 0 ? probe_env : 4;
        probe_blocks = L.nrb >= 16 * std::max(1, probe_blocks) ? probe_blocks : 0;
      }
    }
  }
  if (!small && !persistent && nd > 0 && mode != MODE_PRECISE) {
    K = kvariant(P->dkmax);
    R = pick_rows_per_lane(dtype, K, mode, v.m);
    L = plan_launch(ctx, dtype, P->maxfeat + nd, weighted, mode == MODE_LOSS, v.m, (int32_t)live.size(), 64 * R,
                    lds_budget(R, K, true), eval_waves(R, K));
    use_d = L.xlds;
    const char* always = env_get("SRHIP_DERIVE_ALWAYS");
    if (use_d && !(always && *always && *always != '0')) {
      const int Kp = kvariant(P->kmax), Rp = pick_rows_per_lane(dtype, Kp, mode, v.m);
      const LaunchPlan Lp = plan_launch(ctx, dtype, P->maxfeat, weighted, mode == MODE_LOSS, v.m, (int32_t)live.size(),
                                        64 * Rp, lds_budget(Rp, Kp, false), eval_waves(Rp, Kp));
      if (Lp.xlds && Lp.rb_rows > L.rb_rows) use_d = false;
    }
  }
  if (!small && !persistent && !use_d) {
    K = kvariant(P->kmax);
    R = pick_rows_per_lane(dtype, K, mode, v.m);
    L = plan_launch(ctx, dtype, P->maxfeat, weighted, mode == MODE_LOSS, v.m, (int32_t)live.size(), 64 * R,
                    lds_budget(R, K, false), eval_waves(R, K));
  }
  const int nl = (int)live.size();
  const void* d_order;
  const std::vector<int32_t> goff = persistent ? std::vector<int32_t>{0, nl} : shape_groups(L, nl, ctx->num_cu);
  {
    std::lock_guard<std::mutex> g(P->ord_mu);
    if (P->upload_pending || P->ord_key[0] != L.groups || P->ord_key[1] != L.tpg || P->ord_key[2] != (int)use_d ||
        P->ord_goff != goff) {
      std::vector<int32_t>& order = P->ord_host;
      order = make_order(*P, live, goff, use_d);
      order.insert(order.end(), goff.begin(), goff.end());
      if (P->upload_pending) {
        const size_t base = P->blob_off[6], bytes = order.size() * sizeof(int32_t);
        P->blob.resize(base + bytes);
        memcpy(P->blob.data() + base, order.data(), bytes);
        HIP_TRY(P->d_prog.ensure(base + bytes));
        HIP_TRY(hipMemcpyAsync(P->d_prog.p, P->blob.data(), base + bytes, hipMemcpyHostToDevice, ctx->stream));
        set_prog_pointers(*P);
        P->upload_pending = false;
        P->ord_dev = (const uint8_t*)P->d_prog.p + base;
      } else {
        HIP_TRY(P->d_order.ensure(order.size() * sizeof(int32_t)));
        HIP_TRY(hipMemcpyAsync(P->d_order.p, order.data(), order.size() * sizeof(int32_t), hipMemcpyHostToDevice,
                               ctx->stream));
        P->ord_dev = P->d_order.p;
      }
      P->ord_key[0] = L.groups;
      P->ord_key[1] = L.tpg;
      P->ord_key[2] = (int)use_d;
      P->ord_goff = goff;
    }
    d_order = P->ord_dev;
  }
  const int nch = (int)((v.m + loss_chunk(dtype) - 1) / loss_chunk(dtype));
  const int cpb = L.rb_rows / loss_chunk(dtype);
  HIP_TRY(ctx->slab_loss.ensure((size_t)nl * L.nrb * cpb * 8));
  HIP_TRY(ctx->slab_chk.ensure((size_t)nl * L.nrb * 8));
  HIP_TRY(rs->h_loss.ensure((size_t)nt * 8, hipHostMallocCoherent));
  HIP_TRY(rs->h_chk.ensure((size_t)nt * 8, hipHostMallocCoherent));
  HIP_TRY(rs->h_rows.ensure((size_t)(nt + 1) * 8, hipHostMallocCoherent));
  EvalArgs a{};
  a.code = use_d ? P->dcode_dev : P->code_dev;
  a.prog_off = use_d ? P->doff_dev : P->off_dev;
  a.order = (const int32_t*)d_order;
  a.nd = use_d ? nd : 0;
  a.dspec = use_d ? P->dspec_dev : nullptr;
  a.dmask = use_d ? P->dmask_dev : nullptr;
  if (dtype == SRHIP_F32) {
    if (!P->sbound_dev || P->sbound.size() != 4 * (size_t)P->ntrees)
      return fail(SRHIP_ERR_INVALID, "Float32 program without its +/- bounds");
    J.fbound = feature_bound(v, ds->nfeat);
  }
  a.X = v.X;
  a.y = v.y;
  a.w = weighted ? v.w : nullptr;
  a.slab_loss = ctx->slab_loss.p;
  a.slab_chk = ctx->slab_chk.p;
  a.ld = v.ld;
  a.nvalid = v.m;
  a.ntrees = nl;
  a.nfeat = P->maxfeat;
  a.rb_rows = L.rb_rows;
  a.nrb = L.nrb;
  a.nch = nch;
  a.cpb = cpb;
  a.trees_per_group = L.tpg;
  a.group_off = (const int32_t*)d_order + nl;
  a.loss_kind = loss ? loss->kind : 0;
  a.loss_p0 = loss ? loss->p0 : 0.0;
  a.weighted = weighted ? 1 : 0;
  a.has_y = mode == MODE_LOSS ? 1 : 0;
  a.max_steps = use_d ? P->dmax_len : P->max_len;
  a.debug_stop = debug_stop();
  if (small) a.wg_waves = (int)live.size();
  const char* nofuse = env_get("SRHIP_NO_FUSED_REDUCE");
  if (L.nrb == 1 && !sd && !(nofuse && *nofuse && *nofuse != '0')) {
    a.fused = 1;
    a.fused_loss = mode == MODE_LOSS ? rs->h_loss.p : nullptr;
    a.fused_chk = dtype == SRHIP_I32 ? nullptr : rs->h_chk.p;
    a.fused_rows = (int64_t*)rs->h_rows.p;
  } else {
    HIP_TRY(ctx->slab_rows.ensure((size_t)nl * L.nrb * sizeof(int32_t)));
    a.slab_rows = (int32_t*)ctx->slab_rows.p;
  }
  const bool devp = dp && !a.fused && dtype != SRHIP_I32 && !env_flag("SRHIP_NO_DEVICE_PRECISE");
  int ucap = std::max(1, std::min(DEV_PRECISE_MAX, env_int("SRHIP_PRECISE_LIST", DEV_PRECISE_MAX)));
  if (devp) {
    const int rc = ensure_dev_precise(ctx, P, v, &ucap, rs);
    if (rc) return rc;
  }
  a.early_exit = mode == MODE_LOSS && early_exit_on() ? 1 : 0;
  if (a.early_exit) {
    const int rc = next_fail_epoch(ctx, nl, &a.fail_flag, &a.epoch);
    if (rc) return rc;
  }
  if (trace_on()) {
    HIP_TRY(ctx->h_dbg.ensure(64 * sizeof(int32_t), hipHostMallocCoherent));
    memset(ctx->h_dbg.p, 0xff, 64 * sizeof(int32_t));
    a.dbg = (int32_t*)ctx->h_dbg.p;
  }
  DevBuf& pred = J.pred;
  if (mode == MODE_PRED) {
    HIP_TRY(pred.ensure((size_t)nt * v.m * es));
    a.out_pred = pred.p;
  }
  dim3 grid(L.nrb, (unsigned)goff.size() - 1);
  const bool probe_zeroes = probe_blocks > 0 && !env_flag("SRHIP_PROBE_TREE_CLAIMS");
  if (persistent && (!ctx->block_ctr.p || (ctx->block_ctr_dirty && !probe_zeroes))) {
    HIP_TRY(ctx->block_ctr.ensure(2 * sizeof(int32_t)));
    HIP_TRY(hipMemsetAsync(ctx->block_ctr.p, 0, 2 * sizeof(int32_t), ctx->stream));
    ctx->block_ctr_dirty = false;
  }
  if (persistent) ctx->block_ctr_dirty = true;
  if (sd) HIP_TRY(hipMemsetAsync(sd->d_loss, 0, sd->zero_bytes, ctx->stream));
  HIP_TRY(hipEventRecord(rs->ev0, ctx->stream));
  if (persistent) {
    if (probe_blocks > 0) {
      EvalArgs q = a;
      q.group_off = nullptr;
      q.trees_per_group = eval_waves(R, K);
      q.grid_interleave = 1;
      if (probe_zeroes) {
        q.tile_claims = 1;
        q.zero_ctr = (int32_t*)ctx->block_ctr.p;
      }
      q.code = P->code_dev;
      q.prog_off = P->off_dev;
      q.max_steps = P->max_len;
      q.nd = 0;
      q.dspec = nullptr;
      q.dmask = nullptr;
      const size_t qlds = (size_t)(P->maxfeat + 1 + (weighted ? 1 : 0)) * L.rb_rows * es + 16;
      const dim3 pgrid(probe_blocks, (unsigned)((nl + q.trees_per_group - 1) / q.trees_per_group));
      HIP_TRY(launch_eval(dtype, q, R, K, mode, true, pgrid, qlds, ctx->stream));
    }
    a.persistent = 1;
    a.block0 = probe_blocks;
    a.block_ctr = (int32_t*)ctx->block_ctr.p;
    if (const int seed = env_int("SRHIP_DEBUG_BLOCK_CTR", 0)) {
      const int32_t h = (int32_t)seed;
      HIP_TRY(hipMemcpyAsync(ctx->block_ctr.p, &h, sizeof(h), hipMemcpyHostToDevice, ctx->stream));
      HIP_TRY(hipStreamSynchronize(ctx->stream));
    }
    const int nmain = L.nrb - probe_blocks;
    constexpr int TAIL_UNITS = 128;
    const int wgs_cap = std::max(1, std::min(env_int("SRHIP_PERSISTENT_WGS", ctx->num_cu), ctx->num_cu));
    const int units_env = env_int("SRHIP_TAIL_SLICES", 0);
    const int units = units_env > 1 ? std::min(units_env, 128) : TAIL_UNITS;
    int wgs = std::max(1, std::min(nmain, wgs_cap));
    a.tail_slices = 1;
    a.tail_blocks = 0;
    a.tail_shares = 0;
    if (env_int("SRHIP_TAIL_BALANCE", 1) != 0 && nmain % wgs_cap != 0) {
      const int lb = nmain % wgs_cap;
      const int nshares = wgs_cap * (env_int("SRHIP_TAIL_SHARE_ROUNDS", 1) == 2 ? 2 : 1);
      if ((int64_t)nl * lb >= (int64_t)eval_waves(R, K) * nshares &&
          (int64_t)lb * units * nshares < ((int64_t)1 << 31)) {
        wgs = wgs_cap;
        a.tail_slices = units;
        a.tail_blocks = lb;
        a.tail_shares = nshares;
      }
    }
    J.expect_items = nmain - a.tail_blocks + a.tail_shares;
    HIP_TRY(launch_eval(dtype, a, R, K, mode, true, dim3(wgs, 1), L.lds, ctx->stream));
  } else {
    HIP_TRY(launch_eval(dtype, a, R, K, mode, L.xlds, grid, L.lds, ctx->stream));
  }
  HIP_TRY(hipEventRecord(rs->ev1, ctx->stream));
  J.launched = true;
  J.persistent = persistent;
  J.devp = devp;
  if (trace_on()) {
    const volatile int32_t* d = (const volatile int32_t*)ctx->h_dbg.p;
    int32_t last[16];
    for (int i = 0; i < 16; ++i) last[i] = -2;
    for (int it = 0; it < 10000; ++it) {
      hipError_t q = hipStreamQuery(ctx->stream);
      bool changed = false;
      for (int i = 0; i < 16; ++i) changed |= d[i] != last[i];
      if (changed) {
        for (int i = 0; i < 16; ++i) last[i] = d[i];
        fprintf(stderr, "[srhip] kernel progress: stage=%d tree=%d waves=%d,%d,%d,%d,%d,%d,%d,%d\n", last[0], last[1],
                last[8], last[9], last[10], last[11], last[12], last[13], last[14], last[15]);
        fflush(stderr);
      }
      if (q == hipSuccess) break;
      if (q != hipErrorNotReady) HIP_TRY(q);
      usleep(1000);
      if (it == 9999) {
        fprintf(stderr, "[srhip] kernel did not finish in 10 s; aborting\n");
        fflush(stderr);
        abort();
      }
    }
  }
  UndecidedList& ul = J.ul;
  int ul_groups = 4;
  if (devp) {
    if (!ctx->d_ulist.p) {
      HIP_TRY(ctx->d_ulist.ensure((2 + DEV_PRECISE_MAX) * sizeof(int32_t)));
      HIP_TRY(hipMemsetAsync(ctx->d_ulist.p, 0, ctx->d_ulist.bytes, ctx->stream));
    }
    ul.ulist = (int32_t*)ctx->d_ulist.p;
    ul.umax = ucap;
    ul.rows = (double)v.m;
    ul_groups = std::min(ul.umax, std::max(4, P->und_hint + 2));
  }
  J.fused = a.fused != 0;
  if (dtype == SRHIP_F32) {
    ul.sbound = P->sbound_dev;
    ul.fbound = J.fbound;
  }
  if (!a.fused)
    HIP_TRY(launch_reduce(dtype, mode == MODE_LOSS ? ctx->slab_loss.p : nullptr, nch, cpb,
                          dtype == SRHIP_I32 ? nullptr : ctx->slab_chk.p, L.nrb, nl, (const int32_t*)d_order,
                          mode == MODE_LOSS ? (sd ? sd->d_loss : rs->h_loss.p) : nullptr,
                          dtype == SRHIP_I32 ? nullptr : (sd ? sd->d_chk : rs->h_chk.p), ctx->stream, a.slab_rows,
                          (int64_t*)rs->h_rows.p, ul, sd != nullptr,
                          persistent ? (int32_t*)ctx->block_ctr.p + 1 : nullptr,
                          persistent ? (int64_t*)rs->h_rows.p + nt : nullptr));
  if (devp) {
    int stride = 1;
    const int rc = enqueue_dev_precise(ctx, ds, P, v, ul.ulist, ul.umax, ul_groups, &stride, rs);
    if (rc) return rc;
    dp->used = true;
    dp->stride = stride;
  }
  if (mode == MODE_PRED)
    HIP_TRY(hipMemcpyAsync(out_pred, pred.p, (size_t)nt * v.m * es, hipMemcpyDeviceToHost, ctx->stream));
  HIP_TRY(hipEventRecord(rs->done, ctx->stream));
  return SRHIP_OK;
}

static int eval_collect(srhip_ctx* ctx, const srhip_program* P, const View& v, double* sums, double* chk,
                        DevPrecise* dp, ShardDev* sd, EvalJob& J) {
  ResultSet* const rs = J.rs;
  const int dtype = J.dtype, mode = J.mode;
  const int32_t nt = J.nt;
  const std::vector<int32_t>& live = J.live;
  const bool persistent = J.persistent, devp = J.devp;
  const UndecidedList& ul = J.ul;
  ctx->last_ev0 = rs->ev0;
  ctx->last_ev1 = rs->ev1;
  ctx->timed = true;
  if (devp) {
    const int32_t* hl = (const int32_t*)rs->h_pout.p;
    const double* hs = (const double*)((const uint8_t*)rs->h_pout.p + PREC_SUMS_OFF);
    dp->count = hl[0];
    P->und_hint = dp->count;
    const int nu = std::min(dp->count, ul.umax);
    dp->list.assign(hl + 1, hl + 1 + nu);
    dp->opsums.assign(hs, hs + (size_t)nu * dp->stride);
  }
  static thread_local std::vector<uint64_t> r_loss, r_chk, r_rows;
  r_loss.resize(nt);
  r_chk.resize(nt);
  r_rows.resize(nt);
  if (mode == MODE_LOSS) memcpy(r_loss.data(), rs->h_loss.p, (size_t)nt * 8);
  if (dtype != SRHIP_I32) memcpy(r_chk.data(), rs->h_chk.p, (size_t)nt * (dtype == SRHIP_F32 ? 4 : 8));
  memcpy(r_rows.data(), rs->h_rows.p, (size_t)nt * 8);
  for (int32_t t : live) {
    if (sd) break;
    if (mode == MODE_LOSS)
      sums[2 * (size_t)t] = dtype == SRHIP_I32 ? (double)((const long long*)r_loss.data())[t] : ((const double*)r_loss.data())[t];
    if (dtype == SRHIP_F32) {
      const float m = ((const float*)r_chk.data())[t];
      chk[t] = J.fused ? skip_bound_apply(m, P->sbound.data() + 4 * (size_t)t, J.fbound) : m;
    } else if (dtype == SRHIP_F64) {
      chk[t] = ((const double*)r_chk.data())[t];
    }
  }
  if (persistent) {
    const int64_t done = ((const int64_t*)rs->h_rows.p)[nt];
    if (done != J.expect_items)
      return fail(SRHIP_ERR_DEVICE, "persistent launch evaluated %lld of %d row-block items (row-block counter "
                  "not at zero); the counter is reset for the next launch", (long long)done, (int)J.expect_items);
    ctx->block_ctr_dirty = false;
  }
  for (int i = 0; i < 4; ++i) ctx->work[i] = 0;
  const bool pdec = P->dec.size() == (size_t)nt;
  for (int32_t t : live) {
    const int64_t rows = ((const int64_t*)r_rows.data())[t];
    const int64_t nn = pdec ? P->dec[t].nnodes : P->info[t].nnodes, no = pdec ? P->dec[t].nops : P->info[t].nops;
    ctx->work[0] += rows * nn;
    ctx->work[1] += v.m * nn;
    ctx->work[2] += rows * no;
    ctx->work[3] += rows;
  }
  g_tail_done = std::chrono::steady_clock::now();
  return SRHIP_OK;
}

static int eval_partials(srhip_ctx* ctx, const srhip_dataset* ds, const srhip_program* P, int mode, const srhip_loss* loss,
                         const View& v, void* out_pred, double* sums, double* chk, DevPrecise* dp = nullptr,
                         ShardDev* sd = nullptr) {
  EvalJob J;
  J.rs = &ctx->rs[0];
  int rc = eval_issue(ctx, ds, P, mode, loss, v, out_pred, sums, chk, dp, sd, J);
  if (rc || !J.launched) return rc;
  rc = stream_wait(ctx);
  if (rc) return rc;
  return eval_collect(ctx, P, v, sums, chk, dp, sd, J);
}

static int eval_precise(srhip_ctx* ctx, const srhip_dataset* ds, const srhip_program* P, const View& v,
                        const int32_t* trees, int32_t nu, double* opsums, bool grad = false) {
  const int dtype = P->dtype;
  const int stride = std::max(1, grad ? P->gmax_ops : P->max_ops);
  for (size_t i = 0; i < (size_t)nu * stride; ++i) opsums[i] = 0.0;
  if (nu == 0 || dtype == SRHIP_I32) return SRHIP_OK;
  const int R = pick_rows_per_lane(dtype, K_MAX, MODE_PRECISE, v.m);
  LaunchPlan Lp = plan_launch(ctx, dtype, ds->nfeat, false, false, v.m, nu, 64 * R);
  Lp.groups = 1;
  Lp.tpg = nu;
  const size_t slab_bytes = (size_t)nu * stride * Lp.nrb * sizeof(double);
  HIP_TRY(ctx->slab_prec.ensure(slab_bytes));
  HIP_TRY(hipMemsetAsync(ctx->slab_prec.p, 0, slab_bytes, ctx->stream));
// ... 177 lines not shown
    for (size_t u = 0; u < unc.size(); ++u) {
      const int32_t t = unc[u];
      ok[t] = uok[u];
      lossv[t] = uok[u] ? sums[2 * (size_t)t] / sums[2 * (size_t)t + 1] : INFINITY;
    }
  }
  for (int32_t t = 0; t < nt; ++t) {
    if (out_ok) out_ok[t] = ok[t];
    if (out_loss) out_loss[t] = lossv[t];
  }
  return SRHIP_OK;
}

int srhip::run_eval(srhip_ctx* ctx, const srhip_dataset* ds, const srhip_program* P, int mode, const srhip_loss* loss,
                    const int64_t* idx, int64_t nidx, double* out_loss, void* out_pred, uint8_t* out_ok) {
  static const bool timing = env_flag("SRHIP_HOST_TIMING");
  const auto t_entry = std::chrono::steady_clock::now();
  struct Report {
    bool on;
    std::chrono::steady_clock::time_point t0;
    ~Report() {
      if (!on) return;
      static thread_local double acc[4];
      static thread_local int cnt;
      const auto t3 = std::chrono::steady_clock::now();
      acc[0] += std::chrono::duration<double>(g_wait_begin - t0).count();
      acc[1] += std::chrono::duration<double>(g_wait_done - g_wait_begin).count();
      acc[2] += std::chrono::duration<double>(g_tail_done - g_wait_done).count();
      acc[3] += std::chrono::duration<double>(t3 - g_tail_done).count();
      static const bool each = [] {
        const char* e = getenv("SRHIP_HOST_TIMING");
        return e && atoi(e) >= 2;
      }();
      if (++cnt % (each ? 1 : 50) == 0) {
        fprintf(stderr, "[srhip host] run_eval: before wait %.1f us, wait %.1f us, records %.1f us, decisions %.1f us "
                "(mean of %d)\n", acc[0] / cnt * 1e6, acc[1] / cnt * 1e6, acc[2] / cnt * 1e6, acc[3] / cnt * 1e6, cnt);
        acc[0] = acc[1] = acc[2] = acc[3] = 0.0;
        cnt = 0;
      }
    }
  } report{timing, t_entry};
  RunJob R;
  R.J.rs = &ctx->rs[0];
  int rc = run_issue(ctx, ds, P, mode, loss, idx, nidx, out_pred, R);
  if (rc) return rc;
  if (R.J.launched) {
    rc = stream_wait(ctx);
    if (rc) return rc;
  }
  return run_complete(ctx, R, out_loss, out_ok);
}

int srhip::run_eval_sharded(srhip_ctx* ctx, const srhip_dataset* ds, const srhip_program* P, const srhip_loss* loss,
                            const int64_t* idx, int64_t nidx, const ShardIO& io, double* out_loss, uint8_t* out_ok) {
  int rc = check_eval_args(ctx, ds, P, MODE_LOSS, loss);
  if (rc) return rc;
  HIP_TRY(hipSetDevice(ctx->device));
  View v;
  rc = make_view(ctx, ds, idx, nidx, true, v);
  if (rc) return rc;
  if (idx && ds->weighted) {
    rc = gathered_weight_sum(ctx, ds, nidx, v);
    if (rc) return rc;
  }
  const int32_t nt = P->ntrees;
  if (nt == 0) return SRHIP_OK;
  const int64_t nf = ds->nfeat;
  const size_t ns = sums_len(nt, nf);
  ShardLayout SL;
  SL.dtype = P->dtype;
  SL.nt = (size_t)nt;
  SL.naux = 2 + 2 * (size_t)nf;
  void* dbuf = nullptr;
  rc = io.buffer(SL.bytes(), &dbuf);
  if (rc) return rc;
  ShardDev sd;
  sd.d_loss = dbuf;
  sd.d_chk = (uint8_t*)dbuf + SL.chk_off();
  sd.zero_bytes = SL.chk_off() + SL.nt * SL.chk_size();
  std::vector<double> sums(ns, 0.0), chk(nt, 0.0);
  rc = eval_partials(ctx, ds, P, MODE_LOSS, loss, v, nullptr, sums.data(), chk.data(), nullptr, &sd);
  if (rc) return rc;
  std::vector<double> aux(SL.naux);
  aux[0] = sums[1];
  for (size_t i = 0; i < 2 * (size_t)nf + 1; ++i) aux[1 + i] = sums[2 * (size_t)nt + i];
  const void* red = nullptr;
  rc = io.reduce(SL, aux.data(), &red);
  if (rc) return rc;
  const uint8_t* rb = (const uint8_t*)red;
  const double* raux = (const double*)(rb + SL.aux_off());
  for (int32_t t = 0; t < nt; ++t) {
    sums[2 * (size_t)t] = P->dtype == SRHIP_I32 ? (double)((const long long*)rb)[t] : ((const double*)rb)[t];
    sums[2 * (size_t)t + 1] = raux[0];
    if (P->dtype == SRHIP_F32) chk[t] = ((const float*)(rb + SL.chk_off()))[t];
    else if (P->dtype == SRHIP_F64) chk[t] = ((const double*)(rb + SL.chk_off()))[t];
  }
  for (size_t i = 0; i < 2 * (size_t)nf + 1; ++i) sums[2 * (size_t)nt + i] = raux[1 + i];
  std::vector<uint8_t> status(nt), ok(nt);
  std::vector<double> lossv(nt);
  finalize(*P, nf, sums.data(), chk.data(), lossv.data(), ok.data(), status.data());
  std::vector<int32_t> unc;
  for (int32_t t = 0; t < nt; ++t)
    if (status[t] == 2) unc.push_back(t);
  if (!unc.empty()) {
    const int stride = std::max(1, P->max_ops);
    std::vector<double> opsums(unc.size() * stride);
    rc = eval_precise(ctx, ds, P, v, unc.data(), (int32_t)unc.size(), opsums.data());
    if (rc) return rc;
    rc = io.reduce_host(opsums.data(), opsums.size());
    if (rc) return rc;
    std::vector<uint8_t> uok(unc.size());
    finalize_precise(*P, unc.data(), (int32_t)unc.size(), opsums.data(), uok.data());
    for (size_t u = 0; u < unc.size(); ++u) {
      const int32_t t = unc[u];
      ok[t] = uok[u];
      lossv[t] = uok[u] ? sums[2 * (size_t)t] / sums[2 * (size_t)t + 1] : INFINITY;
    }
  }
  for (int32_t t = 0; t < nt; ++t) {
    if (out_ok) out_ok[t] = ok[t];
    if (out_loss) out_loss[t] = lossv[t];
  }
  return SRHIP_OK;
}

static void plan_persistent_order(const srhip_ctx* ctx, srhip_program& P) {
  if (!ctx || P.dtype != SRHIP_F32 || P.ntrees == 0) return;
  if (env_flag("SRHIP_NO_PERSISTENT") || env_flag("SRHIP_NO_PREPLAN")) return;
  bool wide = false;
  for (int32_t u : P.unaops) wide |= u == SRHIP_OP_ASIN || u == SRHIP_OP_ACOS || u == SRHIP_OP_ATANH_CLIP;
  auto kvariant = [&](int32_t kmax) { return wide ? K_MAX : (kmax <= 2 ? 2 : (kmax <= 4 ? 4 : 8)); };
  const int nd = (int)P.dspec.size();
  const int Kp = kvariant(P.kmax);
  if (pick_rows_per_lane(SRHIP_F32, Kp, MODE_LOSS, WIDE_MIN_ROWS) != R_F32_WIDE || R_F32_WIDE == R_F32) return;
  if (nd != 0 && kvariant(P.dkmax) != Kp) return;
  const int prb_env = env_int("SRHIP_PRB_ROWS", 0);
  const int tile = 64 * R_F32_WIDE;
  int rb = prb_env >= tile && prb_env <= ROW_ALIGN && (prb_env & (prb_env - 1)) == 0 ? prb_env : 2048;
  rb = std::max(rb, std::max(tile, loss_chunk(SRHIP_F32)));
  const size_t budget = (size_t)ctx->lds_max - 8 * 1024;
  const int base_cols = P.maxfeat + 1;
  const bool use_d = nd > 0 && (size_t)(base_cols + nd) * rb * 4 <= budget;
  if ((size_t)(base_cols + (use_d ? nd : 0)) * rb * 4 > budget) return;
  std::vector<int32_t> live;
  live.reserve(P.ntrees);
  for (int32_t t = 0; t < P.ntrees; ++t)
    if (!P.info[t].static_fail) live.push_back(t);
  if (live.empty()) return;
  const int nl = (int)live.size();
  const std::vector<int32_t> goff{0, nl};
  std::lock_guard<std::mutex> g(P.ord_mu);
  P.ord_host = make_order(P, live, goff, use_d);
  P.ord_host.insert(P.ord_host.end(), goff.begin(), goff.end());
  P.ord_key[0] = 1;
  P.ord_key[1] = nl;
  P.ord_key[2] = (int)use_d;
  P.ord_goff = goff;
}

namespace {
struct Reaper {
  std::mutex mu;
  std::condition_variable cv;
  std::vector<srhip_program*> q;
  bool started = false;
};
Reaper& reaper() {
  static Reaper* R = new Reaper();
  return *R;
}
}

static void reaper_push(srhip_program* P) {
  Reaper& R = reaper();
  std::lock_guard<std::mutex> g(R.mu);
  R.q.push_back(P);
  if (!R.started) {
    R.started = true;
    std::thread([&R] {
      for (;;) {
        std::vector<srhip_program*> batch;
        {
          std::unique_lock<std::mutex> lk(R.mu);
          R.cv.wait(lk, [&R] { return !R.q.empty(); });
          batch.swap(R.q);
        }
        for (srhip_program* p : batch) {
          if (p->device >= 0) (void)hipSetDevice(p->device);
          delete p;
        }
      }
    }).detach();
  }
  R.cv.notify_one();
}

template <typename T>
static void pack_column(const void* src, int64_t f, int64_t n, int64_t sf, int64_t sr, int64_t ld, T* dst) {
  const T* s = (const T*)src;
  for (int64_t j = 0; j < n; ++j) dst[j] = s[f * sf + j * sr];
  for (int64_t j = n; j < ld; ++j) dst[j] = dst[n - 1];
}

extern "C" {

const char* srhip_last_error(void) { return srhip::last_error(); }
const char* srhip_version(void) { return "srhip 0.1.0 gfx950"; }

int srhip_device_count(void) {
  int n = 0;
  if (hipGetDeviceCount(&n) != hipSuccess) return 0;
  return n;
}

int srhip_ctx_create(int device, srhip_ctx** out) {
  if (!out) return fail(SRHIP_ERR_INVALID, "null out");
  *out = nullptr;
  int n = 0;
  if (hipGetDeviceCount(&n) != hipSuccess || n <= 0) return fail(SRHIP_ERR_DEVICE, "no HIP device available");
  if (device < 0 || device >= n) return fail(SRHIP_ERR_INVALID, "device %d out of range (%d devices)", device, n);
  std::unique_ptr<srhip_ctx> c(new srhip_ctx());
  c->device = device;
  HIP_TRY(hipSetDevice(device));
  hipDeviceProp_t prop;
  HIP_TRY(hipGetDeviceProperties(&prop, device));
  c->num_cu = prop.multiProcessorCount > 0 ? prop.multiProcessorCount : 256;
  int lds_max = 0;
  if (hipDeviceGetAttribute(&lds_max, hipDeviceAttributeMaxSharedMemoryPerBlock, device) == hipSuccess && lds_max > 0)
    c->lds_max = lds_max;
  if (strncmp(prop.gcnArchName, "gfx950", 6) != 0)
    return fail(SRHIP_ERR_UNSUPPORTED, "device %d is %s; libsrhip is built for gfx950 only", device, prop.gcnArchName);
  HIP_TRY(hipStreamCreateWithFlags(&c->stream, hipStreamNonBlocking));
  HIP_TRY(hipEventCreate(&c->ev0));
  HIP_TRY(hipEventCreate(&c->ev1));
  HIP_TRY(hipEventCreateWithFlags(&c->ev_sync, hipEventDisableTiming));
  for (ResultSet& r : c->rs) {
    HIP_TRY(hipEventCreate(&r.ev0));
    HIP_TRY(hipEventCreate(&r.ev1));
    HIP_TRY(hipEventCreateWithFlags(&r.done, hipEventDisableTiming));
  }
  HIP_TRY(hipStreamCreateWithFlags(&c->up_stream, hipStreamNonBlocking));
  *out = c.release();
  return SRHIP_OK;
}

void srhip_ctx_destroy(srhip_ctx* ctx) {
  if (!ctx) return;
  for (srhip_ctx* a : ctx->aux) srhip_ctx_destroy(a);
  ctx->aux.clear();
  (void)hipSetDevice(ctx->device);
  if (ctx->stream) (void)hipStreamSynchronize(ctx->stream);
  if (ctx->ev0) (void)hipEventDestroy(ctx->ev0);
  if (ctx->ev1) (void)hipEventDestroy(ctx->ev1);
  if (ctx->ev_sync) (void)hipEventDestroy(ctx->ev_sync);
  for (ResultSet& r : ctx->rs)
    for (hipEvent_t e : {r.ev0, r.ev1, r.done})
      if (e) (void)hipEventDestroy(e);
  if (ctx->stream) (void)hipStreamDestroy(ctx->stream);
  if (ctx->up_stream) (void)hipStreamDestroy(ctx->up_stream);
  delete ctx;
  (void)hipGetLastError();
}

int srhip_ctx_synchronize(srhip_ctx* ctx) {
  if (!ctx) return fail(SRHIP_ERR_INVALID, "null ctx");
  HIP_TRY(hipStreamSynchronize(ctx->stream));
  return SRHIP_OK;
}

int srhip_dataset_create(srhip_ctx* ctx, int dtype, const void* X, int64_t nfeat, int64_t n, int64_t sf, int64_t sr,
                         const void* y, const void* w, srhip_dataset** out) {
  if (!ctx || !out) return fail(SRHIP_ERR_INVALID, "null argument");
  *out = nullptr;
  if (dtype != SRHIP_F32 && dtype != SRHIP_F64 && dtype != SRHIP_I32) return fail(SRHIP_ERR_UNSUPPORTED, "dtype %d", dtype);
  if (n <= 0) return fail(SRHIP_ERR_INVALID, "dataset needs n >= 1 rows");
  if (nfeat < 0 || nfeat > 65535) return fail(SRHIP_ERR_INVALID, "nfeatures %lld out of range", (long long)nfeat);
  if (nfeat > 0 && !X) return fail(SRHIP_ERR_INVALID, "null X");
  if (dtype == SRHIP_I32 && w) return fail(SRHIP_ERR_UNSUPPORTED, "weights on Int32 datasets");
  HIP_TRY(hipSetDevice(ctx->device));
  std::unique_ptr<srhip_dataset> d(new srhip_dataset());
  static std::atomic<uint64_t> g_ds_serial{0};
  d->serial = ++g_ds_serial;
  d->ctx = ctx;
  d->device = ctx->device;
  d->dtype = dtype;
  d->nfeat = nfeat;
  d->n = n;
  d->ld = (n + ROW_ALIGN - 1) / ROW_ALIGN * ROW_ALIGN;
  d->has_y = y != nullptr;
  d->weighted = w != nullptr;
  const size_t es = dtype_size(dtype);
  const size_t colb = (size_t)d->ld * es;
  HIP_TRY(d->X.ensure(std::max<size_t>(1, (size_t)nfeat) * colb));
  HostBuf stage;
  HIP_TRY(stage.ensure(colb));
  for (int64_t f = 0; f < nfeat; ++f) {
    if (dtype == SRHIP_F64) pack_column<uint64_t>(X, f, n, sf, sr, d->ld, (uint64_t*)stage.p);
    else pack_column<uint32_t>(X, f, n, sf, sr, d->ld, (uint32_t*)stage.p);
    HIP_TRY(hipMemcpy((char*)d->X.p + f * colb, stage.p, colb, hipMemcpyHostToDevice));
  }
  if (y) {
    HIP_TRY(d->y.ensure(colb));
    if (dtype == SRHIP_F64) pack_column<uint64_t>(y, 0, n, 0, 1, d->ld, (uint64_t*)stage.p);
    else pack_column<uint32_t>(y, 0, n, 0, 1, d->ld, (uint32_t*)stage.p);
    HIP_TRY(hipMemcpy(d->y.p, stage.p, colb, hipMemcpyHostToDevice));
  }
// ... 329 lines not shown
  std::unique_ptr<srhip_eval_ticket> t(new srhip_eval_ticket());
  t->ctx = ctx;
  if (idx) {
    t->loss.resize(prog->ntrees);
    t->ok.resize(prog->ntrees);
    const int rc = run_eval(ctx, ds, prog, MODE_LOSS, loss, idx, nidx, t->loss.data(), nullptr, t->ok.data());
    if (rc) return rc;
    t->done = true;
    *out = t.release();
    return SRHIP_OK;
  }
  int k = -1;
  for (int i = 1; i < RESULT_SETS && k < 0; ++i)
    if (!ctx->rs[i].busy) k = i;
  if (k < 0) return fail(SRHIP_ERR_INVALID, "%d evaluations already in flight on this context", RESULT_SETS - 1);
  t->R.J.rs = &ctx->rs[k];
  const int rc = run_issue(ctx, ds, prog, MODE_LOSS, loss, nullptr, 0, nullptr, t->R);
  if (rc) {
    (void)hipStreamSynchronize(ctx->stream);
    return rc;
  }
  ctx->rs[k].busy = true;
  *out = t.release();
  return SRHIP_OK;
}

int srhip_eval_loss_wait(srhip_eval_ticket* ticket, double* out_loss, uint8_t* out_ok) {
  if (!ticket) return fail(SRHIP_ERR_INVALID, "null ticket");
  std::unique_ptr<srhip_eval_ticket> t(ticket);
  if (t->done) {
    for (size_t i = 0; i < t->loss.size(); ++i) {
      if (out_loss) out_loss[i] = t->loss[i];
      if (out_ok) out_ok[i] = t->ok[i];
    }
    return SRHIP_OK;
  }
  srhip_ctx* ctx = t->ctx;
  ResultSet* rs = t->R.J.rs;
  struct Release {
    ResultSet* r;
    ~Release() { r->busy = false; }
  } release{rs};
  HIP_TRY(hipSetDevice(ctx->device));
  if (t->R.J.launched) HIP_TRY(hipEventSynchronize(rs->done));
  return run_complete(ctx, t->R, out_loss, out_ok);
}

int srhip_eval_predict(srhip_ctx* ctx, const srhip_dataset* ds, const srhip_program* prog, const int64_t* idx,
                       int64_t nidx, void* out_pred, uint8_t* out_ok) {
  if (!out_pred || !out_ok) return fail(SRHIP_ERR_INVALID, "null output");
  return run_eval(ctx, ds, prog, MODE_PRED, nullptr, idx, nidx, nullptr, out_pred, out_ok);
}

int srhip_eval_loss_batch(srhip_ctx* ctx, const srhip_dataset* ds, const srhip_node* nodes, const int64_t* offsets,
                          int32_t ntrees, const srhip_operators* ops, const srhip_loss* loss, const int64_t* idx,
                          int64_t nidx, double* out_loss, uint8_t* out_ok) {
  if (!ds) return fail(SRHIP_ERR_INVALID, "null dataset");
  srhip_program* P = nullptr;
  int rc = srhip_program_create(ctx, ds->dtype, nodes, offsets, ntrees, ops, &P);
  if (rc) return rc;
  rc = srhip_eval_loss(ctx, ds, P, loss, idx, nidx, out_loss, out_ok);
  srhip_program_destroy(P);
  return rc;
}

int srhip_eval_loss_partials(srhip_ctx* ctx, const srhip_dataset* ds, const srhip_program* P, const srhip_loss* loss,
                             const int64_t* idx, int64_t nidx, double* sums, double* chk) {
  if (!sums || !chk) return fail(SRHIP_ERR_INVALID, "null output");
  int rc = check_eval_args(ctx, ds, P, MODE_LOSS, loss);
  if (rc) return rc;
  HIP_TRY(hipSetDevice(ctx->device));
  View v;
  rc = make_view(ctx, ds, idx, nidx, true, v);
  if (rc) return rc;
  if (idx && ds->weighted) {
    rc = gathered_weight_sum(ctx, ds, nidx, v);
    if (rc) return rc;
  }
  return eval_partials(ctx, ds, P, MODE_LOSS, loss, v, nullptr, sums, chk);
}

int srhip_partials_finalize(const srhip_program* P, int64_t nfeatures, const double* sums, const double* chk,
                            double* out_loss, uint8_t* out_ok, uint8_t* out_status) {
  if (!P || !sums || (!chk && P->dtype != SRHIP_I32)) return fail(SRHIP_ERR_INVALID, "null argument");
  if (nfeatures < 0) return fail(SRHIP_ERR_INVALID, "nfeatures < 0");
  for (const TreeInfo& I : P->info)
    for (int f : I.feat_checks)
      if (f >= nfeatures) return fail(SRHIP_ERR_INVALID, "tree checks feature %d of %lld", f + 1, (long long)nfeatures);
  finalize(*P, nfeatures, sums, chk, out_loss, out_ok, out_status);
  return SRHIP_OK;
}

int srhip_eval_precise_partials(srhip_ctx* ctx, const srhip_dataset* ds, const srhip_program* P, const int64_t* idx,
                                int64_t nidx, const int32_t* trees, int32_t ntrees_sel, double* opsums) {
  if (!opsums || (!trees && ntrees_sel > 0) || ntrees_sel < 0) return fail(SRHIP_ERR_INVALID, "null argument");
  int rc = check_eval_args(ctx, ds, P, MODE_PRED, nullptr);
  if (rc) return rc;
  for (int32_t u = 0; u < ntrees_sel; ++u)
    if (trees[u] < 0 || trees[u] >= P->ntrees) return fail(SRHIP_ERR_INVALID, "tree index %d out of range", trees[u]);
  HIP_TRY(hipSetDevice(ctx->device));
  View v;
  rc = make_view(ctx, ds, idx, nidx, false, v);
  if (rc) return rc;
  return eval_precise(ctx, ds, P, v, trees, ntrees_sel, opsums);
}

int srhip_precise_finalize(const srhip_program* P, const int32_t* trees, int32_t ntrees_sel, const double* opsums,
                           uint8_t* out_ok) {
  if (!P || !opsums || !out_ok || (!trees && ntrees_sel > 0)) return fail(SRHIP_ERR_INVALID, "null argument");
  for (int32_t u = 0; u < ntrees_sel; ++u)
    if (trees[u] < 0 || trees[u] >= P->ntrees) return fail(SRHIP_ERR_INVALID, "tree index %d out of range", trees[u]);
  finalize_precise(*P, trees, ntrees_sel, opsums, out_ok);
  return SRHIP_OK;
}

int srhip_chk_reduce_op(int dtype) { return dtype == SRHIP_F32 ? 0 : 1; }

int32_t srhip_program_max_ops(const srhip_program* P) { return P ? std::max(1, P->max_ops) : 0; }

double srhip_last_kernel_ms(const srhip_ctx* ctx) {
  if (!ctx || !ctx->timed || !ctx->last_ev0 || !ctx->last_ev1) return -1.0;
  float ms = -1.0f;
  if (hipEventElapsedTime(&ms, ctx->last_ev0, ctx->last_ev1) != hipSuccess) return -1.0;
  return (double)ms;
}

int srhip_code_cache_stats(int64_t* hits, int64_t* misses, int64_t* inserts) {
  if (hits) *hits = g_cache_hits.load();
  if (misses) *misses = g_cache_misses.load();
  if (inserts) *inserts = g_cache_inserts.load();
  return SRHIP_OK;
}

int srhip_tail_share_parts(int32_t blocks, int32_t units, int32_t nshares, int32_t share, int32_t* out) {
  if (!out || blocks < 1 || units < 1 || nshares < blocks || share < 0 || share >= nshares ||
      (int64_t)blocks * units * nshares >= ((int64_t)1 << 31))
    return -1;
  TailPart part[2];
  const int n = tail_share_parts(blocks, units, nshares, share, part);
  for (int i = 0; i < n; ++i) {
    out[3 * i] = part[i].block;
    out[3 * i + 1] = part[i].u0;
    out[3 * i + 2] = part[i].u1;
  }
  return n;
}

int srhip_last_work(const srhip_ctx* ctx, int64_t* out) {
  if (!ctx || !out) return fail(SRHIP_ERR_INVALID, "null argument");
  for (int i = 0; i < 4; ++i) out[i] = ctx->work[i];
  return SRHIP_OK;
}

int srhip_program_stats(const srhip_program* P, int64_t* total_nodes, int64_t* total_opnodes, int32_t* max_stack) {
  if (!P) return fail(SRHIP_ERR_INVALID, "null program");
  if (total_nodes) *total_nodes = P->total_nodes;
  if (total_opnodes) *total_opnodes = P->total_ops;
  if (max_stack) *max_stack = P->kmax;
  return SRHIP_OK;
}

int srhip_program_derived(const srhip_program* P, int32_t* count, uint32_t* spec, int32_t cap) {
  if (!P) return fail(SRHIP_ERR_INVALID, "null program");
  if (count) *count = (int32_t)P->dspec.size();
  for (int32_t d = 0; spec && d < cap && d < (int32_t)P->dspec.size(); ++d) spec[d] = P->dspec[d];
  return SRHIP_OK;
}

}
```

symbolicregression.jl_amd/csrc/srhip_internal.h:

```cpp
#pragma once
#include <hip/hip_runtime.h>
#include <math.h>
#include <stdarg.h>
#include <stdint.h>
#include <stdio.h>
#include <stdlib.h>
#include <string.h>

#include <chrono>
#include <functional>
#include <mutex>
#include <string>
#include <vector>

#include "../../include/srhip.h"
#include "srhip_isa.h"
#include "srhip_kernels.h"

namespace srhip {

int fail(int code, const char* fmt, ...);
const char* last_error();

inline bool trace_on() {
  static const int on = [] { const char* e = getenv("SRHIP_TRACE"); return e && *e && *e != '0'; }();
  return on != 0;
}
inline int debug_stop() {
  static const int v = [] { const char* e = getenv("SRHIP_DEBUG_STOP"); return e ? atoi(e) : 0; }();
  return v;
}
inline bool early_exit_on() {
  const char* e = getenv("SRHIP_NO_EARLY_EXIT");
  return !(e && *e && *e != '0');
}
#define HIP_TRY(expr)                                                                             \
  do {                                                                                            \
    if (trace_on()) { fprintf(stderr, "[srhip] %s:%d %s\n", __FILE__, __LINE__, #expr); fflush(stderr); } \
    hipError_t e_ = (expr);                                                                       \
    if (trace_on()) { fprintf(stderr, "[srhip]   -> %d\n", (int)e_); fflush(stderr); }          \
    if (e_ != hipSuccess) return fail(SRHIP_ERR_DEVICE, "%s: %s (%s:%d)", #expr, hipGetErrorString(e_), __FILE__, __LINE__); \
  } while (0)

inline size_t dtype_size(int dtype) { return dtype == SRHIP_F64 ? 8 : 4; }

inline long double ovf_threshold(int dtype) {
  static const long double f64 = ldexpl(1.0L, 1024) - ldexpl(1.0L, 970), f32 = ldexpl(1.0L, 128) - ldexpl(1.0L, 103);
  return dtype == SRHIP_F64 ? f64 : f32;
}

inline size_t grown_size(size_t n, size_t old) {
  const size_t g = old + old / 2;
  const size_t want = (old > 0 && g > n && g <= ((size_t)256 << 20)) ? g : n;
  return want < 256 ? 256 : want;
}
struct DevBuf {
  void* p = nullptr;
  size_t bytes = 0;
  ~DevBuf() { release(); }
  void release() {
    if (p) (void)hipFree(p);
    p = nullptr;
    bytes = 0;
  }
  hipError_t ensure(size_t n) {
    if (n <= bytes && p) return hipSuccess;
    const size_t want = grown_size(n, bytes);
    release();
    hipError_t e = hipMalloc(&p, want);
    if (e == hipSuccess) bytes = want;
    return e;
  }
};
void* devpool_get(size_t bytes, size_t* cap);
void devpool_put(void* p, size_t cap, int device);
struct PoolBuf {
  void* p = nullptr;
  size_t bytes = 0;
  int device = -1;
  ~PoolBuf() { release(); }
  void release() {
    if (p) devpool_put(p, bytes, device);
    p = nullptr;
    bytes = 0;
  }
  hipError_t ensure(size_t n) {
    if (n <= bytes && p) return hipSuccess;
    release();
    size_t cap = 0;
    void* q = devpool_get(n, &cap);
    if (!q) return hipErrorOutOfMemory;
    if (hipGetDevice(&device) != hipSuccess) device = -1;
    p = q;
    bytes = cap;
    return hipSuccess;
  }
};
struct HostBuf {
  void* p = nullptr;
  size_t bytes = 0;
  ~HostBuf() { release(); }
  void release() {
    if (p) (void)hipHostFree(p);
    p = nullptr;
    bytes = 0;
  }
  hipError_t ensure(size_t n, unsigned flags = hipHostMallocDefault) {
    if (n <= bytes && p) return hipSuccess;
    const size_t want = grown_size(n, bytes);
    release();
    hipError_t e = hipHostMalloc(&p, want, flags);
    if (e == hipSuccess) bytes = want;
    return e;
  }
};

struct TreeDecide {
  double maxc = -1.0;
  uint64_t feat_mask = 0;
  int32_t nnodes = 0, nops = 0;
  uint8_t static_fail = 0, has_op = 0, slow = 0;
};
struct TreeInfo {
  bool static_fail = false;
  std::vector<double> fill_consts;
  std::vector<int> feat_checks;
  std::vector<uint8_t> op_sumcheck;
  int32_t nconst = 0, nnodes = 0, nops = 0, need = 0;
  int32_t code_begin = 0, code_len = 0;
  double cost = 0.0;
  float sb[3] = {0.0f, 0.0f, 0.0f};
};



}

namespace srhip {
struct ResultSet {
  HostBuf h_loss, h_chk, h_rows, h_pout;
  hipEvent_t ev0 = nullptr, ev1 = nullptr, done = nullptr;
  bool busy = false;
};
constexpr int RESULT_SETS = 4;
}

struct srhip_ctx {
  int device = 0;
  hipStream_t stream = nullptr;
  hipEvent_t ev0 = nullptr, ev1 = nullptr;
  hipEvent_t last_ev0 = nullptr, last_ev1 = nullptr;
  srhip::ResultSet rs[srhip::RESULT_SETS];
  hipEvent_t ev_sync = nullptr;
  hipStream_t up_stream = nullptr;
  bool timed = false;
  int num_cu = 256;
  int lds_max = 160 * 1024;
  srhip::DevBuf slab_loss, slab_chk, slab_prec, order_prec;
  srhip::DevBuf vX, vy, vw, vidx, vstats;
  srhip::DevBuf g_chunks, g_slab, g_red;
  srhip::DevBuf g_rs_packed, g_rs_meta;
  srhip::DevBuf g_xd;
  uint64_t g_xd_serial = 0;
  int64_t g_xd_ld = 0;
  int g_xd_dtype = -1, g_xd_base = -1;
  std::vector<uint32_t> g_xd_spec;
  srhip::HostBuf h_gchunks[2], h_gred[2];
  srhip::HostBuf h_gpatch, h_gspec;
  srhip::HostBuf h_stats, h_prec, h_plist, h_dbg;
  srhip::HostBuf h_rowsets;
  srhip::DevBuf fail_flag;
  int32_t epoch = 0;
  srhip::DevBuf block_ctr;
  bool block_ctr_dirty = false;
  srhip::DevBuf slab_rows;
  srhip::DevBuf d_ulist;
  int64_t work[4] = {0, 0, 0, 0};
  std::vector<srhip_ctx*> aux;
  std::mutex aux_mu;
};

struct srhip_dataset {
  srhip_ctx* ctx = nullptr;
  int device = 0;
  int dtype = SRHIP_F32;
  int64_t nfeat = 0, n = 0, ld = 0;
  bool has_y = false, weighted = false;
  double sum_w = 0.0;
  srhip::DevBuf X, y, w, stats;
  std::vector<srhip::FeatStat> hstats;
  uint64_t serial = 0;
};

struct srhip_program {
  srhip_ctx* ctx = nullptr;
  int device = -1;
  int dtype = SRHIP_F32;
  int32_t ntrees = 0;
  std::vector<srhip_node> nodes;
  std::vector<int64_t> offsets;
  std::vector<int32_t> binops, unaops;
  std::vector<srhip::TreeInfo> info;
  std::vector<srhip::TreeDecide> dec;
  std::vector<srhip::Ins> code;
  std::vector<int32_t> prog_off;
  int32_t kmax = 0, max_ops = 0, max_len = 0;
  int64_t total_nodes = 0, total_ops = 0;
  int32_t maxfeat = 0;
  mutable srhip::PoolBuf d_prog;
  mutable std::vector<uint8_t> blob;
  mutable bool upload_pending = false;
  mutable int32_t und_hint = 0;
  mutable size_t blob_off[7] = {0, 0, 0, 0, 0, 0, 0};
  mutable const srhip::Ins* code_dev = nullptr;
  mutable const int32_t* off_dev = nullptr;
  std::vector<uint32_t> dspec;
  std::vector<uint64_t> dmask;
  std::vector<srhip::Ins> dcode;
  std::vector<int32_t> dprog_off;
  std::vector<double> dcost;
  int32_t dkmax = 0, dmax_len = 0;
  mutable const srhip::Ins* dcode_dev = nullptr;
  mutable const int32_t* doff_dev = nullptr;
  mutable const uint32_t* dspec_dev = nullptr;
  mutable const uint64_t* dmask_dev = nullptr;
  std::vector<float> sbound;
  mutable const float* sbound_dev = nullptr;
  mutable std::mutex ord_mu;
  mutable int ord_key[3] = {-1, -1, -1};
  mutable std::vector<int32_t> ord_goff;
  mutable std::vector<int32_t> ord_host;
  mutable const void* ord_dev = nullptr;
  mutable srhip::PoolBuf d_order;
  bool grad_ready = false;
  std::vector<uint32_t> gdspec;
  int32_t gdbase = 0;
  bool gdspec_done = false, g_want_derived = false, g_derived = false;
  std::vector<srhip::Ins> gcode;
  std::vector<int32_t> gprog_off;
  std::vector<srhip::TreeInfo> ginfo;
  int32_t gkmax = 0, gmax_len = 0, gmax_ops = 0;
  srhip::PoolBuf d_gcode, d_goff;
  std::vector<double> gsnap;
  std::vector<int64_t> gsnap_off;
  std::vector<int32_t> ghint;
  int32_t gspec_cap = 0, gspec_alloc = 0, gspec_stride = 0;
  int64_t gspec_base = 0;
  std::vector<int32_t> gci_off, gci;
  std::vector<uint8_t> gspec_ok;
  std::vector<srhip::TreeInfo> gbase;
};

namespace srhip {

struct View {
  const void* X;
  const void* y;
  const void* w;
  int64_t ld, m;
  const FeatStat* stats;
  double sum_w;
  int32_t nfeat_x = -1;
  int32_t nd_x = 0;
};
struct LaunchPlan {
  int rb_rows, nrb, groups, tpg;
  bool xlds;
  size_t lds;
};
int compile_program(srhip_program& P);
extern thread_local double g_patch_scan_s, g_patch_copy_s;
int compile_grad_program(srhip_program& P);
void grad_derived_spec(srhip_program& P);
bool spec_instantiate(srhip_program& P, int32_t slot, int32_t t, const double* c, bool* static_fail, int64_t& lo,
                      int64_t& hi);
int upload_program(srhip_program& P, bool sync = true, bool defer = false, hipStream_t stream = nullptr);
int make_view(srhip_ctx* ctx, const srhip_dataset* ds, const int64_t* idx, int64_t nidx, bool need_y, View& v);
int gathered_weight_sum(srhip_ctx* ctx, const srhip_dataset* ds, int64_t nidx, View& v);
LaunchPlan plan_launch(const srhip_ctx* ctx, int dtype, int64_t ncols, bool weighted, bool with_y, int64_t m,
                       int32_t ntrees, int rows_per_tile, size_t lds_budget = 64 * 1024 - 64, int waves = EVAL_WAVES);
int decide_tree(const TreeInfo& I, const srhip_program& P, int64_t nfeat, const double* sums, double chk);
int next_fail_epoch(srhip_ctx* ctx, int64_t n, int32_t** flags, int32_t* epoch);
int check_eval_args(srhip_ctx* ctx, const srhip_dataset* ds, const srhip_program* P, int mode, const srhip_loss* loss);
int run_eval(srhip_ctx* ctx, const srhip_dataset* ds, const srhip_program* P, int mode, const srhip_loss* loss,
             const int64_t* idx, int64_t nidx, double* out_loss, void* out_pred, uint8_t* out_ok);
int precise_decide(srhip_ctx* ctx, const srhip_dataset* ds, const srhip_program* P, const View& v,
                   const int32_t* trees, int32_t nu, bool grad, uint8_t* out_ok);

struct ShardLayout {
  int dtype = 0;
  size_t nt = 0, naux = 0;
  size_t loss_bytes() const { return nt * 8; }
  size_t chk_size() const { return dtype == SRHIP_F64 ? 8 : (dtype == SRHIP_F32 ? 4 : 0); }
  size_t chk_off() const { return loss_bytes(); }
  size_t aux_off() const { return (chk_off() + nt * chk_size() + 7) & ~(size_t)7; }
  size_t bytes() const { return aux_off() + naux * 8; }
};
struct ShardIO {
  std::function<int(size_t bytes, void** dptr)> buffer;
  std::function<int(const ShardLayout& L, const double* aux, const void** out)> reduce;
  std::function<int(double* buf, size_t n)> reduce_host;
};
const char* env_get(const char* name);
int stream_wait(srhip_ctx* ctx);
inline int env_int(const char* name, int dflt) {
  const char* e = env_get(name);
  return e && *e ? atoi(e) : dflt;
}
inline double now_s() {
  return std::chrono::duration<double>(std::chrono::steady_clock::now().time_since_epoch()).count();
}

inline void get_consts(const srhip_node* nd, int64_t i, double*& out) {
  const srhip_node& n = nd[i];
  if (n.degree == 0) {
    if (n.constant) *out++ = n.val;
    return;
  }
  get_consts(nd, n.l, out);
  if (n.degree == 2) get_consts(nd, n.r, out);
}
inline void set_consts(srhip_node* nd, int64_t i, const double*& c) {
  srhip_node& n = nd[i];
  if (n.degree == 0) {
    if (n.constant) n.val = *c++;
    return;
  }
  set_consts(nd, n.l, c);
  if (n.degree == 2) set_consts(nd, n.r, c);
}
int subprogram(srhip_ctx* ctx, const srhip_program* P, const std::vector<int32_t>& trees, srhip_program** Q);
int check_rowsets(const srhip_dataset* ds, int32_t nt, const int64_t* row_offsets, const int64_t* rows);
inline size_t sums_len(int32_t ntrees, int64_t nfeat) { return 2 * (size_t)ntrees + 2 * (size_t)nfeat + 1; }
inline void fill_decide_inputs(double* sums, int32_t ntrees, int64_t nfeat, const FeatStat* stats, int64_t rows) {
  double* const tail = sums + 2 * (size_t)ntrees;
  for (int64_t f = 0; f < nfeat; ++f) {
    tail[2 * f] = stats ? stats[f].sum : 0.0;
    tail[2 * f + 1] = stats ? (double)stats[f].nonfinite : 0.0;
  }
  tail[2 * nfeat] = (double)rows;
}
int run_eval_sharded(srhip_ctx* ctx, const srhip_dataset* ds, const srhip_program* P, const srhip_loss* loss,
                     const int64_t* idx, int64_t nidx, const ShardIO& io, double* out_loss, uint8_t* out_ok);

}
```

symbolicregression.jl_amd/csrc/srhip_kernels.h:

```cpp
#pragma once
#include <hip/hip_runtime.h>
#include <stdint.h>

#include "srhip_isa.h"
#include "srhip_tail_shares.h"

namespace srhip {

#ifndef SRHIP_EVAL_WAVES
#define SRHIP_EVAL_WAVES 8
#endif
constexpr int EVAL_WAVES = SRHIP_EVAL_WAVES;
constexpr int EVAL_WAVES_WIDE = 16;
constexpr int eval_waves(int R, int K) { return (R == 16 && K <= 2) ? EVAL_WAVES_WIDE : EVAL_WAVES; }
constexpr int EVAL_WAVES_MAX = EVAL_WAVES_WIDE > EVAL_WAVES ? EVAL_WAVES_WIDE : EVAL_WAVES;
#ifndef SRHIP_R_F32
#define SRHIP_R_F32 8
#endif
constexpr int R_F32 = SRHIP_R_F32;
constexpr int R_F64 = 4;
constexpr int R_F32_WIDE = 16;
constexpr int64_t WIDE_MIN_ROWS = 4096;
constexpr int ROW_ALIGN = 4096;
constexpr int MODE_LOSS = 0, MODE_PRED = 1, MODE_PRECISE = 2;
constexpr int LOSS_CHUNK_4B = 1024, LOSS_CHUNK_8B = 256;
inline int loss_chunk(int dtype) { return dtype == SRHIP_F64 ? LOSS_CHUNK_8B : LOSS_CHUNK_4B; }

struct FeatStat {
  double sum;
  long long nonfinite;
  double maxabs;
};
constexpr int FEAT_STAT_BLOCKS = 64;
inline size_t feature_stats_scratch(int64_t nfeat) { return (size_t)(nfeat < 1 ? 1 : nfeat) * (1 + FEAT_STAT_BLOCKS); }

struct EvalArgs {
  const Ins* code;
  const int32_t* prog_off;
  const int32_t* order;
  const void* X;
  const void* y;
  const void* w;
  void* slab_loss;
  void* slab_chk;
  void* out_pred;
  void* slab_prec;
  int64_t ld;
  int64_t nvalid;
  int32_t ntrees;
  int32_t nfeat;
  int32_t rb_rows;
  int32_t nrb;
  int32_t nch;
  int32_t cpb;
  int32_t trees_per_group;
  const int32_t* group_off;
  int32_t loss_kind;
  double loss_p0;
  int32_t weighted;
  int32_t prec_stride;
  int32_t has_y;
  int32_t max_steps;
  int32_t debug_stop;
  int32_t nd;
  const uint32_t* dspec;
  const uint64_t* dmask;
  int32_t* dbg;
  int32_t early_exit;
  int32_t epoch;
  int32_t* fail_flag;
  int32_t fused;
  void* fused_loss;
  void* fused_chk;
  int32_t persistent;
  int32_t block0;
  int32_t tail_blocks;
  int32_t tail_slices;
  int32_t tail_shares;
  int32_t grid_interleave;
  int32_t tile_claims;
  int32_t block_stride;
  int32_t* block_ctr;
  int32_t* zero_ctr;
  const int32_t* dev_count;
  int32_t wg_waves;
  int32_t prec_assign;
  int32_t* slab_rows;
  int64_t* fused_rows;
};

int rows_per_lane(int dtype);
int pick_rows_per_lane(int dtype, int K, int mode, int64_t m);
hipError_t launch_eval(int dtype, const EvalArgs& a, int R, int K, int mode, bool xlds, dim3 grid, size_t lds,
                       hipStream_t s);
struct UndecidedList {
  int32_t* ulist = nullptr;
  int32_t umax = 0;
  double rows = 0.0;
  const float* sbound = nullptr;
  float fbound = 0.0f;
};
__host__ __device__ inline float skip_bound_apply(float M, const float* sb, float F) {
  if (!(sb[0] > 0.0f || sb[1] > 0.0f || sb[2] > 0.0f) || !(M - M == 0.0f)) return M;
  const double fb = sb[1] > 0.0f ? (double)sb[1] * (double)F : 0.0;
  const double bd = (double)sb[0] * (double)M + (fb + (double)sb[2]);
  const double mb = bd > (double)M ? bd : (double)M;
  return mb < (double)__FLT_MAX__ ? (float)mb : __FLT_MAX__;
}
hipError_t launch_reduce(int dtype, const void* slab_loss, int nch, int cpb, const void* slab_chk, int nrb, int nslots,
                         const int32_t* order, void* out_loss, void* out_chk, hipStream_t s,
                         const int32_t* slab_rows = nullptr, int64_t* out_rows = nullptr,
                         const UndecidedList& ul = UndecidedList(), bool chk_inf = false,
                         int32_t* items_done = nullptr, int64_t* out_items = nullptr);
hipError_t launch_precise_reduce(const double* slab, int nrb, int stride, int32_t* ulist, int umax, int groups, int done_slot,
                                 int32_t* out_list, double* out, hipStream_t s);
hipError_t launch_gather(int dtype, const void* X, const void* y, const void* w, int64_t ld_src, int nfeat,
                         const int64_t* idx, int64_t m, int64_t ld_dst, void* Xd, void* yd, void* wd, hipStream_t s);
hipError_t launch_feature_stats(int dtype, const void* X, int64_t ld, int64_t m, int nfeat, FeatStat* out,
                                hipStream_t s);

struct RowsetArgs {
  EvalArgs e;
  const int64_t* row_off;
  const int64_t* rows;
  int64_t src_ld;
  int32_t nstage;
  int32_t ld_lds;
  FeatStat* fstat;
  double* wsum;
};
constexpr int ROWSET_LDS_BUDGET = 40 * 1024;
int rowset_cap(int dtype, int64_t nfeat, bool weighted);
hipError_t launch_rowsets(int dtype, const RowsetArgs& a, int nlaunch, hipStream_t s);

}
```

symbolicregression.jl_amd/srhip/_lib.py:

```python
from __future__ import annotations

import ctypes
import os
import threading

import numpy as np

_PKG_DIR = os.path.dirname(os.path.abspath(__file__))
LIB_PATH = os.environ.get(
    "SRHIP_LIB", os.path.join(os.path.dirname(_PKG_DIR), "build", "libsrhip.so")
)

OK, ERR_INVALID, ERR_UNSUPPORTED, ERR_DEVICE, ERR_NOMEM = 0, 1, 2, 3, 4
COMM_ID_BYTES = 128
REDUCE_SUM, REDUCE_MAX = 0, 1
F32, F64, I32 = 0, 1, 2

OP = dict(
    ADD=1, SUB=2, MUL=3, DIV=4, POW=5, GREATER=6, COND=7, LOGICAL_OR=8, LOGICAL_AND=9,
    MAX=10, MIN=11, MOD=12, ATAN2=13,
    NEG=32, SQUARE=33, CUBE=34, ABS=35, RELU=36, COS=37, SIN=38, TAN=39, EXP=40, LOG=41,
    LOG2=42, LOG10=43, LOG1P=44, SQRT=45, ACOSH=46, ATANH_CLIP=47, SINH=48, COSH=49, TANH=50,
    ASIN=51, ACOS=52, ATAN=53, ASINH=54, ERF=55, ERFC=56, GAMMA=57, ROUND=58, FLOOR=59,
    CEIL=60, SIGN=61, EXP2=62, EXPM1=63, CBRT=64,
)
LOSS = dict(
    L2=0, L1=1, LP=2, HUBER=3, L1_EPS_INS=4, L2_EPS_INS=5, LOGIT_DIST=6, PERIODIC=7, QUANTILE=8,
    ZERO_ONE=9, PERCEPTRON=10, LOGIT_MARGIN=11, L1_HINGE=12, L2_HINGE=13, SMOOTHED_L1_HINGE=14,
    MODIFIED_HUBER=15, L2_MARGIN=16, EXP=17, SIGMOID=18, DWD_MARGIN=19,
)

NODE_DTYPE = np.dtype(
    [("degree", "u1"), ("constant", "u1"), ("op", "<u2"), ("feature", "<u2"), ("pad", "<u2"),
     ("l", "<i4"), ("r", "<i4"), ("val", "<f8")],
    align=True,
)
assert NODE_DTYPE.itemsize == 24


class Operators(ctypes.Structure):
    _fields_ = [("nbin", ctypes.c_int32), ("nuna", ctypes.c_int32),
                ("binops", ctypes.POINTER(ctypes.c_int32)), ("unaops", ctypes.POINTER(ctypes.c_int32))]


class Loss(ctypes.Structure):
    _fields_ = [("kind", ctypes.c_int32), ("pad", ctypes.c_int32),
                ("p0", ctypes.c_double), ("p1", ctypes.c_double)]


class OptimOptions(ctypes.Structure):
    _fields_ = [("iterations", ctypes.c_int32), ("nrestarts", ctypes.c_int32), ("seed", ctypes.c_uint64),
                ("g_tol", ctypes.c_double)]


class SrhipError(RuntimeError):

    def __init__(self, code: int, msg: str):
        super().__init__(f"srhip error {code}: {msg}")
        self.code = code


_vp, _i32, _i64, _dbl = ctypes.c_void_p, ctypes.c_int32, ctypes.c_int64, ctypes.c_double
SIGNATURES = {
    "srhip_last_error": (ctypes.c_char_p, []),
    "srhip_version": (ctypes.c_char_p, []),
    "srhip_device_count": (ctypes.c_int, []),
    "srhip_ctx_create": (ctypes.c_int, [ctypes.c_int, ctypes.POINTER(_vp)]),
    "srhip_ctx_destroy": (None, [_vp]),
    "srhip_ctx_synchronize": (ctypes.c_int, [_vp]),
    "srhip_dataset_create": (ctypes.c_int, [_vp, ctypes.c_int, _vp, _i64, _i64, _i64, _i64, _vp, _vp,
                                            ctypes.POINTER(_vp)]),
    "srhip_dataset_destroy": (None, [_vp]),
    "srhip_program_create": (ctypes.c_int, [_vp, ctypes.c_int, _vp, _vp, _i32, ctypes.POINTER(Operators),
                                            ctypes.POINTER(_vp)]),
    "srhip_program_destroy": (None, [_vp]),
    "srhip_program_num_constants": (ctypes.c_int, [_vp, _vp]),
    "srhip_program_set_constants": (ctypes.c_int, [_vp, _vp]),
    "srhip_program_get_constants": (ctypes.c_int, [_vp, _vp]),
    "srhip_eval_loss": (ctypes.c_int, [_vp, _vp, _vp, ctypes.POINTER(Loss), _vp, _i64, _vp, _vp]),
    "srhip_eval_loss_rowsets": (ctypes.c_int, [_vp, _vp, _vp, ctypes.POINTER(Loss), _vp, _vp, _vp, _vp]),
    "srhip_eval_predict": (ctypes.c_int, [_vp, _vp, _vp, _vp, _i64, _vp, _vp]),
    "srhip_eval_loss_submit": (ctypes.c_int, [_vp, _vp, _vp, ctypes.POINTER(Loss), _vp, _i64, ctypes.POINTER(_vp)]),
    "srhip_eval_loss_wait": (ctypes.c_int, [_vp, _vp, _vp]),
    "srhip_eval_loss_batch": (ctypes.c_int, [_vp, _vp, _vp, _vp, _i32, ctypes.POINTER(Operators),
                                             ctypes.POINTER(Loss), _vp, _i64, _vp, _vp]),
    "srhip_eval_loss_partials": (ctypes.c_int, [_vp, _vp, _vp, ctypes.POINTER(Loss), _vp, _i64, _vp, _vp]),
    "srhip_partials_finalize": (ctypes.c_int, [_vp, _i64, _vp, _vp, _vp, _vp, _vp]),
    "srhip_eval_precise_partials": (ctypes.c_int, [_vp, _vp, _vp, _vp, _i64, _vp, _i32, _vp]),
    "srhip_precise_finalize": (ctypes.c_int, [_vp, _vp, _i32, _vp, _vp]),
    "srhip_chk_reduce_op": (ctypes.c_int, [ctypes.c_int]),
    "srhip_program_max_ops": (_i32, [_vp]),
    "srhip_eval_loss_grad": (ctypes.c_int, [_vp, _vp, _vp, ctypes.POINTER(Loss), _vp, _i64, _vp, _vp, _vp]),
    "srhip_eval_grad_predict": (ctypes.c_int, [_vp, _vp, _vp, _i32, _i32, _vp, _i64, _vp, _vp, _vp]),
    "srhip_optimize_constants": (ctypes.c_int, [_vp, _vp, _vp, ctypes.POINTER(Loss), _vp, _i64,
                                                ctypes.POINTER(OptimOptions), _vp, _vp, _vp]),
    "srhip_optimize_constants_starts": (ctypes.c_int, [_vp, _vp, _vp, ctypes.POINTER(Loss), _vp, _i64,
                                                       ctypes.POINTER(OptimOptions), _vp, _vp, _vp, _vp, _vp]),
    "srhip_eval_loss_grad_rowsets": (ctypes.c_int, [_vp, _vp, _vp, ctypes.POINTER(Loss), _vp, _vp, _vp, _vp, _vp]),
    "srhip_optimize_constants_rowsets": (ctypes.c_int, [_vp, _vp, _vp, ctypes.POINTER(Loss), _vp, _vp,
                                                        ctypes.POINTER(OptimOptions), _vp, _vp, _vp, _vp, _vp, _vp]),
    "srhip_batcher_create": (ctypes.c_int, [_vp, _vp, ctypes.POINTER(Operators), ctypes.POINTER(Loss), _i32, _i32,
                                            ctypes.POINTER(_vp)]),
    "srhip_batcher_set_clients": (ctypes.c_int, [_vp, _i32]),
    "srhip_batcher_submit": (ctypes.c_int, [_vp, _vp, _i64, _vp, _i64, ctypes.POINTER(ctypes.c_uint64)]),
    "srhip_batcher_wait": (ctypes.c_int, [_vp, ctypes.c_uint64, ctypes.POINTER(_dbl), ctypes.POINTER(ctypes.c_uint8)]),
    "srhip_batcher_eval": (ctypes.c_int, [_vp, _vp, _i64, _vp, _i64, ctypes.POINTER(_dbl),
                                          ctypes.POINTER(ctypes.c_uint8)]),
    "srhip_batcher_stats": (ctypes.c_int, [_vp, ctypes.POINTER(_i64), ctypes.POINTER(_i64), ctypes.POINTER(_i64)]),
    "srhip_batcher_timing": (ctypes.c_int, [_vp, ctypes.POINTER(ctypes.c_double), ctypes.POINTER(ctypes.c_double)]),
    "srhip_batcher_destroy": (None, [_vp]),
    "srhip_comm_unique_id": (ctypes.c_int, [_vp]),
    "srhip_comm_create": (ctypes.c_int, [_vp, _vp, _i32, _i32, ctypes.POINTER(_vp)]),
    "srhip_comm_destroy": (None, [_vp]),
    "srhip_comm_size": (ctypes.c_int, [_vp, ctypes.POINTER(_i32), ctypes.POINTER(_i32)]),
    "srhip_comm_stats": (ctypes.c_int, [_vp, ctypes.POINTER(ctypes.c_double), ctypes.POINTER(ctypes.c_double),
                                        ctypes.POINTER(ctypes.c_int64)]),
    "srhip_comm_allreduce_f64": (ctypes.c_int, [_vp, _vp, _i64, _i32]),
    "srhip_comm_allgather": (ctypes.c_int, [_vp, _vp, _i64, _vp]),
    "srhip_comm_migrate_start": (ctypes.c_int, [_vp, _vp, _vp, _i32, _vp, _i32, _i32]),
    "srhip_comm_migrate_wait": (ctypes.c_int, [_vp, _vp, _vp, _vp, _vp]),
    "srhip_eval_loss_sharded": (ctypes.c_int, [_vp, _vp, _vp, _vp, ctypes.POINTER(Loss), _vp, _i64, _vp, _vp]),
    "srhip_last_kernel_ms": (_dbl, [_vp]),
    "srhip_last_work": (ctypes.c_int, [_vp, ctypes.POINTER(_i64)]),
    "srhip_program_stats": (ctypes.c_int, [_vp, ctypes.POINTER(_i64), ctypes.POINTER(_i64),
                                           ctypes.POINTER(_i32)]),
    "srhip_program_derived": (ctypes.c_int, [_vp, ctypes.POINTER(_i32), _vp, _i32]),
    "srhip_code_cache_stats": (ctypes.c_int, [ctypes.POINTER(_i64), ctypes.POINTER(_i64), ctypes.POINTER(_i64)]),
    "srhip_tail_share_parts": (ctypes.c_int, [_i32, _i32, _i32, _i32, _vp]),
}

_lib = None
_lock = threading.Lock()


def load() -> ctypes.CDLL:
    global _lib
    with _lock:
        if _lib is not None:
            return _lib
        if not os.path.exists(LIB_PATH):
            raise SrhipError(ERR_DEVICE, f"{LIB_PATH} not built: run `make -C symbolicregression.jl_amd` "
                                         "(or __graft_entry__.build()); there is no CPU fallback")
        lib = ctypes.CDLL(LIB_PATH)
        for name, (res, args) in SIGNATURES.items():
            try:
                fn = getattr(lib, name)
            except AttributeError:
                continue
            fn.restype = res
            fn.argtypes = args
        _lib = lib
        return lib


def check(code: int) -> None:
    if code != OK:
        msg = load().srhip_last_error().decode(errors="replace")
        raise SrhipError(code, msg)


def ptr(a: np.ndarray | None) -> ctypes.c_void_p | None:
    if a is None:
        return None
    return ctypes.c_void_p(a.ctypes.data)


def dtype_code(dt) -> int:
    dt = np.dtype(dt)
    if dt == np.float32:
        return F32
    if dt == np.float64:
        return F64
    if dt == np.int32:
        return I32
    raise SrhipError(ERR_UNSUPPORTED, f"element type {dt} is not supported on the device "
                                      "(Float32, Float64, Int32 only)")
```

symbolicregression.jl_amd/srhip/device.py:

```python
from __future__ import annotations

import ctypes
import threading

import numpy as np

from . import _lib
from ._lib import check, ptr


class Context:
    def __init__(self, device: int = 0):
        lib = _lib.load()
        h = ctypes.c_void_p()
        check(lib.srhip_ctx_create(int(device), ctypes.byref(h)))
        self.handle = h
        self.device = int(device)
        self._lib = lib

    def synchronize(self):
        check(self._lib.srhip_ctx_synchronize(self.handle))

    def last_kernel_ms(self) -> float:
        return float(self._lib.srhip_last_kernel_ms(self.handle))

    def last_work(self) -> dict:
        out = (ctypes.c_int64 * 4)()
        check(self._lib.srhip_last_work(self.handle, out))
        return {"node_rows": int(out[0]), "nominal_node_rows": int(out[1]), "opnode_rows": int(out[2]),
                "tree_rows": int(out[3])}

    def close(self):
        if self.handle:
            self._lib.srhip_ctx_destroy(self.handle)
            self.handle = None

    def __del__(self):
        try:
            self.close()
        except Exception:
            pass


_tls = threading.local()


def get_context(device: int = 0) -> Context:
    cache = getattr(_tls, "ctxs", None)
    if cache is None:
        cache = _tls.ctxs = {}
    ctx = cache.get(device)
    if ctx is None:
        ctx = cache[device] = Context(device)
    return ctx


def device_count() -> int:
    try:
        return int(_lib.load().srhip_device_count())
    except _lib.SrhipError:
        return 0


class DeviceDataset:

    def __init__(self, ctx: Context, X: np.ndarray, y=None, weights=None):
        X = np.asarray(X)
        if X.ndim != 2:
            raise ValueError("X must be (nfeatures, n)")
        self.dtype = X.dtype
        code = _lib.dtype_code(X.dtype)
        nfeat, n = X.shape
        es = X.itemsize
        sf, sr = X.strides[0] // es, X.strides[1] // es
        if X.strides[0] % es or X.strides[1] % es:
            X = np.ascontiguousarray(X)
            sf, sr = n, 1
        yv = None if y is None else np.ascontiguousarray(y, dtype=X.dtype)
        wv = None if weights is None else np.ascontiguousarray(weights, dtype=X.dtype)
        h = ctypes.c_void_p()
        check(_lib.load().srhip_dataset_create(ctx.handle, code, ptr(X), nfeat, n, sf, sr, ptr(yv), ptr(wv),
                                               ctypes.byref(h)))
        self.handle = h
        self.ctx = ctx
        self.nfeatures = nfeat
        self.n = n
        self.weighted = weights is not None

    def close(self):
        if self.handle:
            _lib.load().srhip_dataset_destroy(self.handle)
            self.handle = None

    def __del__(self):
        try:
            self.close()
        except Exception:
            pass


def pack_rowsets(idxs, ntrees=None):
    sets = [np.ascontiguousarray(i, dtype=np.int64).reshape(-1) for i in idxs]
    if ntrees is not None and len(sets) != ntrees:
        raise ValueError(f"{len(sets)} row subsets for {ntrees} trees")
    for t, i in enumerate(sets):
        if i.size == 0:
            raise ValueError(f"row subset of tree {t} is empty")
    offsets = np.zeros(len(sets) + 1, dtype=np.int64)
    np.cumsum([i.size for i in sets], out=offsets[1:])
    rows = np.concatenate(sets) if sets else np.zeros(0, dtype=np.int64)
    return offsets, rows


class Program:

    def __init__(self, ctx: Context | None, nodes: np.ndarray, offsets: np.ndarray, options, dtype):
        self.ctx = ctx
        self.nodes = np.ascontiguousarray(nodes)
        self.offsets = np.ascontiguousarray(offsets, dtype=np.int64)
        self.ntrees = len(self.offsets) - 1
        self.options = options
        self.dtype = np.dtype(dtype)
        h = ctypes.c_void_p()
        self._ops = options.c_operators()
        check(_lib.load().srhip_program_create(None if ctx is None else ctx.handle, _lib.dtype_code(dtype),
                                               ptr(self.nodes),
                                               ptr(self.offsets), self.ntrees, ctypes.byref(self._ops),
                                               ctypes.byref(h)))
        self.handle = h

    def num_constants(self) -> np.ndarray:
        out = np.zeros(self.ntrees, dtype=np.int32)
        check(_lib.load().srhip_program_num_constants(self.handle, ptr(out)))
        return out

    def set_constants(self, consts: np.ndarray) -> None:
        c = np.ascontiguousarray(consts, dtype=np.float64)
        check(_lib.load().srhip_program_set_constants(self.handle, ptr(c)))

    def stats(self):
        a, b, c = ctypes.c_int64(), ctypes.c_int64(), ctypes.c_int32()
        check(_lib.load().srhip_program_stats(self.handle, ctypes.byref(a), ctypes.byref(b), ctypes.byref(c)))
        return dict(total_nodes=a.value, total_opnodes=b.value, max_stack=c.value)

    def derived_columns(self) -> list:
        n = ctypes.c_int32()
        spec = np.zeros(64, dtype=np.uint32)
        check(_lib.load().srhip_program_derived(self.handle, ctypes.byref(n), ptr(spec), 64))
        return [(int(s) >> 16, int(s) & 0xffff) for s in spec[:n.value]]

    def eval_loss(self, ds: DeviceDataset, loss, idx=None):
        out = np.empty(self.ntrees, dtype=np.float64)
        ok = np.empty(self.ntrees, dtype=np.uint8)
        ls = loss.c_struct()
        idxa = None if idx is None else np.ascontiguousarray(idx, dtype=np.int64)
        check(_lib.load().srhip_eval_loss(self.ctx.handle, ds.handle, self.handle, ctypes.byref(ls), ptr(idxa),
                                          0 if idxa is None else len(idxa), ptr(out), ptr(ok)))
        return out, ok.astype(bool)

    def eval_loss_rowsets(self, ds: DeviceDataset, loss, idxs):
        offsets, rows = pack_rowsets(idxs, self.ntrees)
        out = np.empty(self.ntrees, dtype=np.float64)
        ok = np.empty(self.ntrees, dtype=np.uint8)
        ls = loss.c_struct()
        check(_lib.load().srhip_eval_loss_rowsets(self.ctx.handle, ds.handle, self.handle, ctypes.byref(ls),
                                                  ptr(offsets), ptr(rows), ptr(out), ptr(ok)))
        return out, ok.astype(bool)

    def eval_loss_submit(self, ds: DeviceDataset, loss, idx=None) -> "EvalTicket":
        ls = loss.c_struct()
        idxa = None if idx is None else np.ascontiguousarray(idx, dtype=np.int64)
        h = ctypes.c_void_p()
        check(_lib.load().srhip_eval_loss_submit(self.ctx.handle, ds.handle, self.handle, ctypes.byref(ls), ptr(idxa),
                                                 0 if idxa is None else len(idxa), ctypes.byref(h)))
        return EvalTicket(h, self, ds)

    def eval_predict(self, ds: DeviceDataset, idx=None):
        idxa = None if idx is None else np.ascontiguousarray(idx, dtype=np.int64)
        m = ds.n if idxa is None else len(idxa)
        out = np.empty((self.ntrees, m), dtype=self.dtype)
        ok = np.empty(self.ntrees, dtype=np.uint8)
        check(_lib.load().srhip_eval_predict(self.ctx.handle, ds.handle, self.handle, ptr(idxa),
                                             0 if idxa is None else len(idxa), ptr(out), ptr(ok)))
# ... 224 lines not shown
```

Measured before the change: 10500 billion node-row evals/s.

## Add specialized hot-form persistent loss kernel with packed per-slot records

Adds a FORM_HOT template specialization of the f32 wide persistent staged-loss kernel. General-path options (tile claims, fused, debug) are compiled out, and per-slot tree/pc0/derived-mask data is packed into 16-byte records read with one scalar load. Rarely used kernel arguments are reloaded from the kernarg segment, and asm barriers keep values in SGPRs, to reduce register pressure and indirect loads in the hot interpreter loop. It adds a separate kernel instantiation, a host-side record array and a launch counter, and is limited to specific launch configurations.

```diff
diff --git a/include/srhip.h b/include/srhip.h
--- a/include/srhip.h
+++ b/include/srhip.h
@@ -207,6 +207,7 @@
 
 double srhip_last_kernel_ms(const srhip_ctx* ctx);
 int srhip_last_work(const srhip_ctx* ctx, int64_t out[4]);
+int64_t srhip_hot_form_launches(const srhip_ctx* ctx);
 int srhip_program_stats(const srhip_program* prog, int64_t* total_nodes, int64_t* total_opnodes,
                         int32_t* max_stack);
 int srhip_program_derived(const srhip_program* prog, int32_t* count, uint32_t* spec, int32_t cap);
diff --git a/symbolicregression.jl_amd/csrc/srhip_eval_f32w.hip b/symbolicregression.jl_amd/csrc/srhip_eval_f32w.hip
--- a/symbolicregression.jl_amd/csrc/srhip_eval_f32w.hip
+++ b/symbolicregression.jl_amd/csrc/srhip_eval_f32w.hip
@@ -3,6 +3,12 @@
 
 namespace srhip {
 hipError_t launch_eval_f32w(const EvalArgs& a, int mode, bool xlds, dim3 g, size_t lds, hipStream_t s) {
+  if (mode == MODE_LOSS && xlds && a.recs) {
+    if (!a.persistent || a.tile_claims || a.fused || a.grid_interleave || a.block_stride || a.debug_stop || a.dbg ||
+        !a.slab_rows || a.wg_waves)
+      return hipErrorInvalidValue;
+    return launch_eval_t<float, R_F32_WIDE, 2, MODE_LOSS, true, FORM_HOT>(a, g, lds, s);
+  }
   if (mode == MODE_LOSS)
     return xlds ? launch_eval_t<float, R_F32_WIDE, 2, MODE_LOSS, true>(a, g, lds, s)
                 : launch_eval_t<float, R_F32_WIDE, 2, MODE_LOSS, false>(a, g, lds, s);
diff --git a/symbolicregression.jl_amd/csrc/srhip_eval_impl.h b/symbolicregression.jl_amd/csrc/srhip_eval_impl.h
--- a/symbolicregression.jl_amd/csrc/srhip_eval_impl.h
+++ b/symbolicregression.jl_amd/csrc/srhip_eval_impl.h
@@ -136,8 +136,10 @@
 
 #if defined(__HIP_DEVICE_COMPILE__)
 typedef const __attribute__((address_space(4))) Ins CIns;
+typedef const __attribute__((address_space(4))) SlotRec CSlotRec;
 #else
 typedef const Ins CIns;
+typedef const SlotRec CSlotRec;
 #endif
 
 template <typename T> __device__ __attribute__((always_inline)) inline T imm_as(uint64_t bits) {
@@ -960,15 +962,50 @@
   __syncthreads();
 }
 
-template <typename T, int R, int K, int MODE, bool XLDS>
+template <typename F>
+__device__ __attribute__((always_inline)) inline F karg_reload(uint32_t off) {
+  asm volatile("" : "+s"(off));
+  typedef const __attribute__((address_space(4))) unsigned char CB;
+  return *reinterpret_cast<const __attribute__((address_space(4))) F*>((CB*)__builtin_amdgcn_kernarg_segment_ptr() + off);
+}
+template <typename L>
+__device__ __attribute__((noinline)) void mark_failed(L* lslab, int c0, int c1, int32_t* flag, int32_t epoch) {
+  if (__builtin_amdgcn_inverse_ballot_w64(1ull << WAVE_LAST)) {
+    for (int c = c0; c < c1; ++c) lslab[c] = (L)NAN;
+    if (flag) __hip_atomic_store(flag, epoch, __ATOMIC_RELAXED, __HIP_MEMORY_SCOPE_AGENT);
+  }
+}
+#define SRHIP_KARG(f) (HOT ? karg_reload<decltype(EvalArgs::f)>((uint32_t)offsetof(EvalArgs, f)) : p.f)
+
+template <typename T, int R, int K, int MODE, bool XLDS, int FORM = FORM_GENERAL>
 __device__ __attribute__((always_inline)) inline void eval_block(const EvalArgs& p, unsigned char* smem, const int rb,
                                                                  const int gy, const int gslice = 0,
                                                                  const int gstride = 1, const int gw = 1) {
+  constexpr bool HOT = FORM == FORM_HOT;
+  static_assert(!HOT || (MODE == MODE_LOSS && XLDS && !kIsInt<T>), "the hot form is a staged loss launch");
   constexpr int WAVES = eval_waves(R, K);
   using O = OpsT<T>;
   using CT = typename Chk<T>::type;
   constexpr int TILE = 64 * R;
   const int lane = tid_x() & 63;
+  auto last_lane = [&]() -> bool {
+    if constexpr (HOT) return __builtin_amdgcn_inverse_ballot_w64(1ull << WAVE_LAST);
+    else return lane == WAVE_LAST;
+  };
+  [[maybe_unused]] uint32_t hot_flags = 0;
+  if constexpr (HOT) {
+    hot_flags = ((uint32_t)p.loss_kind & 0xffu) | (p.weighted ? 0x100u : 0u) | (p.early_exit ? 0x200u : 0u);
+    asm volatile("" : "+s"(hot_flags));
+  }
+  auto flags_now = [&]() -> uint32_t {
+    uint32_t f = hot_flags;
+    asm volatile("" : "+s"(f));
+    return f;
+  };
+  auto early_exit_on = [&]() -> bool {
+    if constexpr (HOT) return (flags_now() & 0x200u) != 0;
+    else return p.early_exit != 0;
+  };
   const int64_t row_base = (int64_t)rb * p.rb_rows;
   const int ntiles = p.rb_rows / TILE;
   const int nrel = __builtin_amdgcn_readfirstlane((int)min<int64_t>(max<int64_t>(p.nvalid - row_base, 0), (int64_t)p.rb_rows));
@@ -1010,9 +1047,10 @@
   constexpr int FLAG_SNAP = 2048;
   constexpr bool SNAP = MODE == MODE_LOSS && !kIsInt<T>;
   __shared__ uint8_t failed_snap[SNAP ? FLAG_SNAP : 1];
-  const int gb0 = p.group_off ? p.group_off[gy] : gy * p.trees_per_group;
+  const int gb0 = HOT ? 0 : (p.group_off ? p.group_off[gy] : gy * p.trees_per_group);
   const int snap_base = gb0 + gslice;
   const int snap_n = gstride > 1 ? tail_units_count(p.ntrees, gstride, gslice, gw)
+                     : HOT       ? p.ntrees
                                  : (p.group_off ? p.group_off[gy + 1] - gb0 : min(p.trees_per_group, p.ntrees - gb0));
   if constexpr (SNAP) {
     if (p.early_exit)
@@ -1025,12 +1063,13 @@
   __shared__ CT dchk[DERIVED ? DERIVE_MAX : 1];
   if constexpr (DERIVED) {
     if (p.nd > 0) {
-      if (p.persistent) derive_columns_tiles<T, R>(p, reinterpret_cast<T*>(smem), p.rb_rows, dchk);
+      if (HOT || p.persistent) derive_columns_tiles<T, R>(p, reinterpret_cast<T*>(smem), p.rb_rows, dchk);
       else derive_columns<T>(p, reinterpret_cast<T*>(smem), p.rb_rows, dchk);
     }
   }
   KMARK(0, 2);
-  if (p.debug_stop == 2) return;
+  if constexpr (!HOT)
+    if (p.debug_stop == 2) return;
 
   const int group_base = __builtin_amdgcn_readfirstlane(snap_base);
   int group_n = __builtin_amdgcn_readfirstlane(snap_n);
@@ -1044,20 +1083,38 @@
   const int wave = __builtin_amdgcn_readfirstlane(threadIdx.x >> 6);
   const CIns* code = (const CIns*)(uintptr_t)p.code;
   KMARK(8 + wave, 10);
-  const bool tile_claims = p.tile_claims != 0 && TILE == (sizeof(T) == 8 ? LOSS_CHUNK_8B : LOSS_CHUNK_4B);
+  const bool tile_claims = !HOT && p.tile_claims != 0 && TILE == (sizeof(T) == 8 ? LOSS_CHUNK_8B : LOSS_CHUNK_4B);
+  const bool fused = !HOT && p.fused != 0;
   const int nclaims = tile_claims ? group_n * ntiles : group_n;
   for (int cl = wave; cl < nclaims;) {
     const int ti = tile_claims ? cl / ntiles : cl;
     const int tile0 = tile_claims ? cl - ti * ntiles : 0, tile_end = tile_claims ? tile0 + 1 : ntiles;
     KMARK(8 + wave, 11);
-    const int slot = group_base + (gw > 1 ? ti / gw * gstride + ti % gw : ti * gstride);
-    const int tree = __builtin_amdgcn_readfirstlane(p.order[slot]);
-    const int pc0 = __builtin_amdgcn_readfirstlane(p.prog_off[tree]);
+    int gw_now = gw;
+    if constexpr (HOT) asm volatile("" : "+s"(gw_now));
+    const int slot = group_base + (gw_now > 1 ? ti / gw * gstride + ti % gw : ti * gstride);
+    int tree, pc0;
+    [[maybe_unused]] uint64_t rec_mask = 0;
+    [[maybe_unused]] int snap_failed = 0;
+    if constexpr (HOT) {
+      const CSlotRec* recs = (const CSlotRec*)(uintptr_t)p.recs;
+      const SlotRec rec = recs[slot];
+      snap_failed = failed_snap[min(ti, FLAG_SNAP - 1)];
+      uint32_t r0 = rec.tree, r1 = rec.pc0, r2 = rec.dmask_lo, r3 = rec.dmask_hi;
+      asm volatile("" : "+s"(r0), "+s"(r1), "+s"(r2), "+s"(r3));
+      tree = (int)r0;
+      pc0 = (int)r1;
+      rec_mask = ((uint64_t)r3 << 32) | r2;
+    } else {
+      tree = __builtin_amdgcn_readfirstlane(p.order[slot]);
+      pc0 = __builtin_amdgcn_readfirstlane(p.prog_off[tree]);
+    }
     const int max_steps = __builtin_amdgcn_readfirstlane(p.max_steps);
     KDBG("[k] ti=%d tree=%d pc0=%d group_n=%d\n", ti, tree, pc0, group_n);
     KMARK(0, 3);
     KMARK(1, tree);
-    if (p.debug_stop == 3) break;
+    if constexpr (!HOT)
+      if (p.debug_stop == 3) break;
 
     if constexpr (MODE == MODE_PRECISE) {
       if (p.dev_count && lane == WAVE_LAST)
@@ -1071,14 +1128,21 @@
     UNR for (int c = 0; c < CPT; ++c) lacc[c] = 0;
     CT M = 0;
     bool failed = false;
-    if constexpr (SNAP) {
-      if (p.early_exit && ti < FLAG_SNAP) failed = __builtin_amdgcn_readfirstlane(failed_snap[ti]) != 0;
+    if constexpr (HOT) {
+      failed = early_exit_on() && ti < FLAG_SNAP && __builtin_amdgcn_readfirstlane(snap_failed) != 0;
+    } else if constexpr (SNAP) {
+      if (early_exit_on() && ti < FLAG_SNAP) failed = __builtin_amdgcn_readfirstlane(failed_snap[ti]) != 0;
     }
     if constexpr (DERIVED) {
-      if (p.nd > 0) {
-        uint64_t msk = p.dmask[tree];
-        msk = ((uint64_t)__builtin_amdgcn_readfirstlane((uint32_t)(msk >> 32)) << 32) |
-              (uint32_t)__builtin_amdgcn_readfirstlane((uint32_t)msk);
+      if (HOT || p.nd > 0) {
+        uint64_t msk;
+        if constexpr (HOT) {
+          msk = rec_mask;
+        } else {
+          msk = p.dmask[tree];
+          msk = ((uint64_t)__builtin_amdgcn_readfirstlane((uint32_t)(msk >> 32)) << 32) |
+                (uint32_t)__builtin_amdgcn_readfirstlane((uint32_t)msk);
+        }
         while (msk) {
           const int d = __builtin_ctzll(msk);
           msk &= msk - 1;
@@ -1087,17 +1151,45 @@
         }
       }
     }
-    LAccT<T>* lslab = reinterpret_cast<LAccT<T>*>(p.slab_loss) +
-                      ((int64_t)rb * p.ntrees + slot) * __builtin_amdgcn_readfirstlane(p.cpb);
+    [[maybe_unused]] const int sidx = HOT ? rb * p.ntrees + slot : 0;
+    [[maybe_unused]] LAccT<T>* const lslab_gen =
+        HOT ? nullptr
+            : reinterpret_cast<LAccT<T>*>(p.slab_loss) +
+                  ((int64_t)rb * p.ntrees + slot) * __builtin_amdgcn_readfirstlane(p.cpb);
+    auto lslab_at = [&]() -> LAccT<T>* {
+      if constexpr (HOT) return reinterpret_cast<LAccT<T>*>(SRHIP_KARG(slab_loss)) + sidx * SRHIP_KARG(cpb);
+      else return lslab_gen;
+    };
     LAccT<T> csum = 0;
     int rows_done = 0;
     if (failed) {
-      if (lane == WAVE_LAST)
+      if constexpr (HOT) {
+        mark_failed(lslab_at(), 0, SRHIP_KARG(cpb), nullptr, 0);
+      } else if (lane == WAVE_LAST) {
+        LAccT<T>* const lslab = lslab_at();
         for (int c = tile_claims ? tile0 : 0; c < (tile_claims ? tile_end : p.cpb); ++c) lslab[c] = (LAccT<T>)NAN;
+      }
       M = (CT)NAN;
       csum = (LAccT<T>)NAN;
     }
-    for (int tile = tile0; tile < (failed ? tile0 : tile_end); ++tile) {
+    [[maybe_unused]] int tile_stop = 0;
+    [[maybe_unused]] uint64_t prog_tree = 0;
+    if constexpr (HOT) {
+      tile_stop = failed ? tile0 : tile_end;
+      asm volatile("" : "+s"(tile_stop));
+      prog_tree = (uint64_t)(uintptr_t)(code + pc0);
+      asm volatile("" : "+s"(prog_tree));
+    }
+    auto prog_of_tile = [&]() -> const CIns* {
+      if constexpr (HOT) {
+        uint64_t pt = prog_tree;
+        asm volatile("" : "+s"(pt));
+        return (const CIns*)(uintptr_t)pt;
+      } else {
+        return code + pc0;
+      }
+    };
+    for (int tile = tile0; tile < (HOT ? tile_stop : (failed ? tile0 : tile_end)); ++tile) {
       const int64_t row0 = row_base + (int64_t)tile * TILE;
       const int trel = tile * TILE;
       if (trel >= nrel) break;
@@ -1111,10 +1203,12 @@
       UNR for (int r = 0; r < R; ++r) A[r] = T(0);
       UNR for (int k = 0; k < K; ++k) UNR for (int r = 0; r < R; ++r) S[k][r] = T(0);
 #endif
-      const CIns* prog = code + pc0;
+      const CIns* prog = prog_of_tile();
       Ins nxt = prog[0];
       [[maybe_unused]] uint32_t pord = 0;
-      for (int step = 0; step < max_steps; ++step) {
+      int steps_max = max_steps;
+      if constexpr (HOT) asm volatile("" : "+s"(steps_max));
+      for (int step = 0; step < steps_max; ++step) {
         const Ins ins = nxt;
         nxt = prog[step + 1];
         KDBG("[k]   tile=%d step=%d h=%u a=%u\n", tile, step, ins.h, ins.a);
@@ -1255,15 +1349,25 @@
       KDBG("[k]   tile %d done\n", tile);
       KMARK(0, 4);
       if constexpr (MODE == MODE_LOSS) {
-        loss_tile<T, R>(p, A, ysrc + (int64_t)tile * TILE, wsrc + (int64_t)tile * TILE, lane, row0, trel + TILE <= nrel,
-                        lacc);
+        if constexpr (HOT) {
+          EvalArgs pl = p;
+          const uint32_t f = flags_now();
+          pl.loss_kind = (int32_t)(f & 0xffu);
+          pl.weighted = (int32_t)((f >> 8) & 1u);
+          loss_tile<T, R>(pl, A, ysrc + (int64_t)tile * TILE, wsrc + (int64_t)tile * TILE, lane, row0,
+                          trel + TILE <= nrel, lacc);
+        } else {
+          loss_tile<T, R>(p, A, ysrc + (int64_t)tile * TILE, wsrc + (int64_t)tile * TILE, lane, row0,
+                          trel + TILE <= nrel, lacc);
+        }
         const bool flushed = (tile + 1) % TPC == 0 || trel + TILE >= nrel;
         const int ci0 = tile * CPT / TPC;
         if (flushed) {
+          LAccT<T>* const lslab = lslab_at();
           UNR for (int c = 0; c < CPT; ++c) {
             const LAccT<T> s = wave_sum(lacc[c]);
-            if (lane == WAVE_LAST) lslab[ci0 + c] = s;
-            if (p.fused) {
+            if (last_lane()) lslab[ci0 + c] = s;
+            if (fused) {
               const LAccT<T> sb = __shfl(s, WAVE_LAST);
               if (lane == (ci0 + c) % 64) csum += sb;
             }
@@ -1271,9 +1375,13 @@
           }
         }
         if constexpr (!kIsInt<T>) {
-          if (p.early_exit && __builtin_amdgcn_ballot_w64(!(M < (CT)INFINITY)) != 0) {
+          if (early_exit_on() && __builtin_amdgcn_ballot_w64(!(M < (CT)INFINITY)) != 0) {
             csum = (LAccT<T>)NAN;
-            if (lane == WAVE_LAST) {
+            if constexpr (HOT) {
+              mark_failed(lslab_at(), ci0 + (flushed ? CPT : 0), SRHIP_KARG(cpb),
+                          SRHIP_KARG(fail_flag) + (sidx - rb * SRHIP_KARG(ntrees)), SRHIP_KARG(epoch));
+            } else if (lane == WAVE_LAST) {
+              LAccT<T>* const lslab = lslab_at();
               for (int c = ci0 + (flushed ? CPT : 0); c < (tile_claims ? tile_end : p.cpb); ++c)
                 lslab[c] = (LAccT<T>)NAN;
               __hip_atomic_store(p.fail_flag + slot, p.epoch, __ATOMIC_RELAXED, __HIP_MEMORY_SCOPE_AGENT);
@@ -1290,8 +1398,9 @@
     KMARK(8 + wave, 12);
     if constexpr (!kIsInt<T> && MODE != MODE_PRECISE) {
       M = wave_chk(M);
-      CT* chk_at = reinterpret_cast<CT*>(p.slab_chk) + (int64_t)rb * p.ntrees + slot;
-      if (lane == WAVE_LAST) {
+      CT* chk_at = HOT ? reinterpret_cast<CT*>(SRHIP_KARG(slab_chk)) + sidx
+                       : reinterpret_cast<CT*>(p.slab_chk) + (int64_t)rb * p.ntrees + slot;
+      if (last_lane()) {
         if constexpr (sizeof(CT) == 4) {
           if (tile_claims) atomicMax(reinterpret_cast<unsigned*>(chk_at), __builtin_bit_cast(unsigned, __builtin_fabsf(M) == __builtin_fabsf(M) ? __builtin_fabsf(M) : M));
           else *chk_at = M;
@@ -1300,12 +1409,14 @@
         }
       }
     }
-    if (p.slab_rows && lane == WAVE_LAST) {
+    if constexpr (HOT) {
+      if (last_lane()) SRHIP_KARG(slab_rows)[sidx] = rows_done;
+    } else if (p.slab_rows && lane == WAVE_LAST) {
       if (tile_claims) atomicAdd(p.slab_rows + (int64_t)rb * p.ntrees + slot, rows_done);
       else p.slab_rows[(int64_t)rb * p.ntrees + slot] = rows_done;
     }
     if constexpr (MODE != MODE_PRECISE) {
-      if (p.fused) {
+      if (fused) {
         LAccT<T> s = csum;
         CT m = 0;
         if constexpr (!kIsInt<T>) {
@@ -1337,16 +1448,18 @@
   KMARK(8 + wave, 14);
 }
 
-template <typename T, int R, int K, int MODE, bool XLDS>
+template <typename T, int R, int K, int MODE, bool XLDS, int FORM = FORM_GENERAL>
 __global__ __launch_bounds__(64 * eval_waves(R, K)) void eval_kernel(EvalArgs p) {
   extern __shared__ __attribute__((aligned(16))) unsigned char smem[];
+  constexpr bool HOT = FORM == FORM_HOT;
   KMARK(0, 1);
-  if (p.debug_stop == 1) return;
+  if constexpr (!HOT)
+    if (p.debug_stop == 1) return;
   __shared__ int claimed;
   if constexpr (MODE == MODE_PRECISE) {
     if (p.dev_count && p.grid_interleave && __builtin_amdgcn_readfirstlane(*p.dev_count) <= (int)blockIdx.y) return;
   }
-  if (p.tile_claims && !p.persistent) {
+  if (!HOT && p.tile_claims && !p.persistent) {
     if (p.zero_ctr && blockIdx.x == 0 && blockIdx.y == 0 && threadIdx.x == 0)
       __hip_atomic_store(p.zero_ctr, 0, __ATOMIC_RELAXED, __HIP_MEMORY_SCOPE_AGENT);
     const int gs = p.grid_interleave ? (int)blockIdx.y : 0, gst = p.grid_interleave ? (int)gridDim.y : 1;
@@ -1364,12 +1477,12 @@
   int next_block = 0, next_units = 0;
   for (int it = 0;; ++it) {
     int rb, gy = 0, gslice = 0, gstride = 1, gw = 1;
-    if (p.persistent && next_units > 0) {
+    if ((HOT || p.persistent) && next_units > 0) {
       rb = next_block;
       gstride = p.tail_slices;
       gw = next_units;
       next_units = 0;
-    } else if (p.persistent) {
+    } else if (HOT || p.persistent) {
       if (threadIdx.x == 0) claimed = atomicAdd(p.block_ctr, 1);
       __syncthreads();
       const int item = __builtin_amdgcn_readfirstlane(claimed);
@@ -1407,15 +1520,15 @@
         gy = blockIdx.y;
       }
     }
-    eval_block<T, R, K, MODE, XLDS>(p, smem, rb, gy, gslice, gstride, gw);
-    if (!p.persistent && !p.block_stride) break;
+    eval_block<T, R, K, MODE, XLDS, FORM>(p, smem, rb, gy, gslice, gstride, gw);
+    if (!HOT && !p.persistent && !p.block_stride) break;
     __syncthreads();
   }
 }
 
-template <typename T, int R, int K, int MODE, bool XLDS>
+template <typename T, int R, int K, int MODE, bool XLDS, int FORM = FORM_GENERAL>
 inline hipError_t launch_eval_t(const EvalArgs& a, dim3 grid, size_t lds, hipStream_t s) {
-  auto kern = eval_kernel<T, R, K, MODE, XLDS>;
+  auto kern = eval_kernel<T, R, K, MODE, XLDS, FORM>;
   if (lds > 65536) {
     hipError_t e = hipFuncSetAttribute((const void*)kern, hipFuncAttributeMaxDynamicSharedMemorySize, (int)lds);
     if (e != hipSuccess) return e;
diff --git a/symbolicregression.jl_amd/csrc/srhip_host.cpp b/symbolicregression.jl_amd/csrc/srhip_host.cpp
--- a/symbolicregression.jl_amd/csrc/srhip_host.cpp
+++ b/symbolicregression.jl_amd/csrc/srhip_host.cpp
@@ -1551,6 +1551,22 @@
     order[(size_t)goff[best] + fill[best]++] = t;
   }
   return order;
+}
+
+static int append_slot_records(const srhip_program& P, std::vector<int32_t>& order, int nl, bool derived) {
+  while (order.size() % 4 != 0) order.push_back(0);
+  const int at = (int)order.size();
+  order.resize((size_t)at + 4 * (size_t)nl);
+  for (int sl = 0; sl < nl; ++sl) {
+    const int32_t t = order[sl];
+    const uint64_t m = derived ? P.dmask[t] : 0;
+    int32_t* r = order.data() + at + 4 * (size_t)sl;
+    r[0] = t;
+    r[1] = derived ? P.dprog_off[t] : P.prog_off[t];
+    r[2] = (int32_t)(uint32_t)m;
+    r[3] = (int32_t)(uint32_t)(m >> 32);
+  }
+  return at;
 }
 
 
@@ -1946,14 +1962,16 @@
   }
   const int nl = (int)live.size();
   const void* d_order;
+  int rec_at = -1;
   const std::vector<int32_t> goff = persistent ? std::vector<int32_t>{0, nl} : shape_groups(L, nl, ctx->num_cu);
   {
     std::lock_guard<std::mutex> g(P->ord_mu);
     if (P->upload_pending || P->ord_key[0] != L.groups || P->ord_key[1] != L.tpg || P->ord_key[2] != (int)use_d ||
-        P->ord_goff != goff) {
+        P->ord_goff != goff || (persistent && P->ord_recs < 0)) {
       std::vector<int32_t>& order = P->ord_host;
       order = make_order(*P, live, goff, use_d);
       order.insert(order.end(), goff.begin(), goff.end());
+      P->ord_recs = persistent ? append_slot_records(*P, order, nl, use_d) : -1;
       if (P->upload_pending) {
         const size_t base = P->blob_off[6], bytes = order.size() * sizeof(int32_t);
         P->blob.resize(base + bytes);
@@ -1975,6 +1993,7 @@
       P->ord_goff = goff;
     }
     d_order = P->ord_dev;
+    rec_at = P->ord_recs;
   }
   const int nch = (int)((v.m + loss_chunk(dtype) - 1) / loss_chunk(dtype));
   const int cpb = L.rb_rows / loss_chunk(dtype);
@@ -2107,7 +2126,11 @@
       }
     }
     J.expect_items = nmain - a.tail_blocks + a.tail_shares;
+    if (R == R_F32_WIDE && K == 2 && rec_at >= 0 && !a.fused && a.slab_rows && !a.dbg && a.debug_stop == 0 &&
+        a.loss_kind >= 0 && a.loss_kind < 256 && (int64_t)nl * L.nrb * cpb < ((int64_t)1 << 31) && !env_flag("SRHIP_NO_HOT_FORM"))
+      a.recs = (const SlotRec*)((const int32_t*)d_order + rec_at);
     HIP_TRY(launch_eval(dtype, a, R, K, mode, true, dim3(wgs, 1), L.lds, ctx->stream));
+    if (a.recs) ++ctx->hot_launches;
   } else {
     HIP_TRY(launch_eval(dtype, a, R, K, mode, L.xlds, grid, L.lds, ctx->stream));
   }
@@ -2591,6 +2614,7 @@
   std::lock_guard<std::mutex> g(P.ord_mu);
   P.ord_host = make_order(P, live, goff, use_d);
   P.ord_host.insert(P.ord_host.end(), goff.begin(), goff.end());
+  P.ord_recs = append_slot_records(P, P.ord_host, nl, use_d);
   P.ord_key[0] = 1;
   P.ord_key[1] = nl;
   P.ord_key[2] = (int)use_d;
@@ -3226,6 +3250,8 @@
   return SRHIP_OK;
 }
 
+int64_t srhip_hot_form_launches(const srhip_ctx* ctx) { return ctx ? ctx->hot_launches : -1; }
+
 int srhip_program_stats(const srhip_program* P, int64_t* total_nodes, int64_t* total_opnodes, int32_t* max_stack) {
   if (!P) return fail(SRHIP_ERR_INVALID, "null program");
   if (total_nodes) *total_nodes = P->total_nodes;
diff --git a/symbolicregression.jl_amd/csrc/srhip_internal.h b/symbolicregression.jl_amd/csrc/srhip_internal.h
--- a/symbolicregression.jl_amd/csrc/srhip_internal.h
+++ b/symbolicregression.jl_amd/csrc/srhip_internal.h
@@ -176,6 +176,7 @@
   srhip::DevBuf slab_rows;
   srhip::DevBuf d_ulist;
   int64_t work[4] = {0, 0, 0, 0};
+  int64_t hot_launches = 0;
   std::vector<srhip_ctx*> aux;
   std::mutex aux_mu;
 };
@@ -231,6 +232,7 @@
   mutable std::vector<int32_t> ord_goff;
   mutable std::vector<int32_t> ord_host;
   mutable const void* ord_dev = nullptr;
+  mutable int ord_recs = -1;
   mutable srhip::PoolBuf d_order;
   bool grad_ready = false;
   std::vector<uint32_t> gdspec;
diff --git a/symbolicregression.jl_amd/csrc/srhip_kernels.h b/symbolicregression.jl_amd/csrc/srhip_kernels.h
--- a/symbolicregression.jl_amd/csrc/srhip_kernels.h
+++ b/symbolicregression.jl_amd/csrc/srhip_kernels.h
@@ -33,6 +33,15 @@
 };
 constexpr int FEAT_STAT_BLOCKS = 64;
 inline size_t feature_stats_scratch(int64_t nfeat) { return (size_t)(nfeat < 1 ? 1 : nfeat) * (1 + FEAT_STAT_BLOCKS); }
+
+constexpr int FORM_GENERAL = 0, FORM_HOT = 1;
+struct alignas(16) SlotRec {
+  int32_t tree;
+  int32_t pc0;
+  uint32_t dmask_lo;
+  uint32_t dmask_hi;
+};
+static_assert(sizeof(SlotRec) == 16, "one s_load_dwordx4");
 
 struct EvalArgs {
   const Ins* code;
@@ -87,6 +96,7 @@
   int32_t prec_assign;
   int32_t* slab_rows;
   int64_t* fused_rows;
+  const SlotRec* recs;
 };
 
 int rows_per_lane(int dtype);
diff --git a/symbolicregression.jl_amd/srhip/_lib.py b/symbolicregression.jl_amd/srhip/_lib.py
--- a/symbolicregression.jl_amd/srhip/_lib.py
+++ b/symbolicregression.jl_amd/srhip/_lib.py
@@ -122,6 +122,7 @@
     "srhip_eval_loss_sharded": (ctypes.c_int, [_vp, _vp, _vp, _vp, ctypes.POINTER(Loss), _vp, _i64, _vp, _vp]),
     "srhip_last_kernel_ms": (_dbl, [_vp]),
     "srhip_last_work": (ctypes.c_int, [_vp, ctypes.POINTER(_i64)]),
+    "srhip_hot_form_launches": (ctypes.c_int64, [_vp]),
     "srhip_program_stats": (ctypes.c_int, [_vp, ctypes.POINTER(_i64), ctypes.POINTER(_i64),
                                            ctypes.POINTER(_i32)]),
     "srhip_program_derived": (ctypes.c_int, [_vp, ctypes.POINTER(_i32), _vp, _i32]),
diff --git a/symbolicregression.jl_amd/srhip/device.py b/symbolicregression.jl_amd/srhip/device.py
--- a/symbolicregression.jl_amd/srhip/device.py
+++ b/symbolicregression.jl_amd/srhip/device.py
@@ -29,6 +29,9 @@
         check(self._lib.srhip_last_work(self.handle, out))
         return {"node_rows": int(out[0]), "nominal_node_rows": int(out[1]), "opnode_rows": int(out[2]),
                 "tree_rows": int(out[3])}
+
+    def hot_form_launches(self) -> int:
+        return int(self._lib.srhip_hot_form_launches(self.handle))
 
     def close(self):
         if self.handle:
```

Measured after the change: 11450 billion node-row evals/s, median of 6. +9.0%, better.
